# JasonQSY/Articulation3D

Hardware: AMD Instinct MI355X
Metric: frames/sec through PlaneRCNN detector at 480x640 (higher is better)
Workload: dtype f32 storage and accumulation; operands enter the matrix pipe with a 22-bit significand under ONE power-of-two block exponent per image (per ROI behind the poolers, per layer for filters): x*s = h + l in fp16, three fp16 MFMAs per k step (h.h + h.l + l.h). Elementwise law |y - y64| <= c (2^-22 sum|x|; 1 GPU; BASELINE configs[2]: full PlaneRCNN detector (ResNet50-FPN + RPN + ROIAlign + box/mask/plane/axis heads + depth head + NMS + mask paste + plane-offset LSQ + record pack), random-init weights with calibrated BN, synthetic 480x640 uint8 frames resident in HBM (arithmetic: see `dtype`)

## Files before the change

articulation3d_amd/_lib.py:

```python
from __future__ import annotations

import ctypes as C
import os

_PKG = os.path.dirname(os.path.abspath(__file__))
LIB_PATH = os.path.join(_PKG, "liba3d_hip.so")

ACT_NONE, ACT_RELU, ACT_LEAKY = 0, 1, 2

_ERR = {-1: "A3D_ERR_ARG", -2: "A3D_ERR_LAUNCH", -3: "A3D_ERR_UNSUPPORTED"}

fptr = C.c_void_p


class ConvDesc(C.Structure):
    _fields_ = [
        ("x", fptr), ("x2", fptr), ("w", fptr), ("scale", fptr), ("shift", fptr), ("res", fptr), ("y", fptr),
        ("workspace", fptr),
        ("B", C.c_int), ("H", C.c_int), ("W", C.c_int), ("Cin", C.c_int), ("Cin2", C.c_int),
        ("Ho", C.c_int), ("Wo", C.c_int), ("Cout", C.c_int),
        ("KH", C.c_int), ("KW", C.c_int), ("stride", C.c_int), ("pad", C.c_int),
        ("Kpad", C.c_int), ("ups", C.c_int), ("act", C.c_int), ("res_ups", C.c_int), ("pixshuf", C.c_int),
        ("stem", C.c_int), ("splitk", C.c_int),
        ("m_dev", fptr),
        ("tune", C.c_int), ("phase", C.c_int),
        ("w_wino", fptr),
        ("gate", fptr),
        ("precision", C.c_int),
        ("w_wino_x3", fptr),
        ("w_wino_cm", fptr),
        ("w_x3", fptr),
        ("in_amax", fptr),
        ("in_amax2", fptr),
        ("y_amax", fptr),
        ("w_scale", C.c_float),
        ("wino_m", fptr),
        ("io_bf16", C.c_int),
        ("x_h2", fptr),
        ("x2_h2", fptr),
        ("dot_w", fptr),
        ("dot_y", fptr),
        ("wino_t_off", C.c_int), ("wino_t_total", C.c_int),
        ("w_bf16", fptr),
    ]


class RpnDesc(C.Structure):
    _fields_ = [
        ("head", fptr * 5),
        ("Hf", C.c_int * 5), ("Wf", C.c_int * 5), ("stride", C.c_int * 5),
        ("cell_anchors", ((C.c_float * 4) * 3) * 5),
        ("B", C.c_int), ("L", C.c_int), ("A", C.c_int), ("CH", C.c_int),
        ("img_h", C.c_int), ("img_w", C.c_int),
        ("pre_topk", C.c_int), ("post_topk", C.c_int),
        ("nms_thresh", C.c_float), ("min_size", C.c_float),
        ("weights", C.c_float * 4),
        ("scale_clamp", C.c_float),
        ("workspace", fptr),
        ("out_boxes", fptr), ("out_scores", fptr), ("out_level", fptr), ("out_pos", fptr), ("out_count", fptr),
    ]


class BoxDetDesc(C.Structure):
    _fields_ = [
        ("pred", fptr), ("prop_boxes", fptr), ("prop_count", fptr),
        ("B", C.c_int), ("R", C.c_int), ("C", C.c_int), ("CH", C.c_int),
        ("img_h", C.c_int), ("img_w", C.c_int),
        ("score_thresh", C.c_float), ("nms_thresh", C.c_float),
        ("topk", C.c_int),
        ("weights", C.c_float * 4),
        ("scale_clamp", C.c_float),
        ("workspace", fptr),
        ("out_boxes", fptr), ("out_scores", fptr), ("out_classes", fptr), ("out_pos", fptr), ("out_count", fptr),
    ]


class RoiAlignDesc(C.Structure):
    _fields_ = [
        ("feat", fptr * 4),
        ("Hf", C.c_int * 4), ("Wf", C.c_int * 4),
        ("scale", C.c_float * 4),
        ("L", C.c_int), ("C", C.c_int),
        ("boxes", fptr), ("count", fptr), ("row_offset", fptr),
        ("B", C.c_int), ("R", C.c_int),
        ("P", C.c_int), ("sampling_ratio", C.c_int), ("aligned", C.c_int),
        ("out", fptr), ("out_level", fptr), ("order_ws", fptr),
        ("out_amax", fptr), ("level_amax", fptr * 4), ("window_count", fptr),
        ("out_h2", fptr),
        ("serial", C.c_int),
    ]


class PasteDesc(C.Structure):
    _fields_ = [
        ("boxes", fptr), ("scores", fptr), ("count", fptr), ("row_offset", fptr), ("mask_prob", fptr),
        ("normals", fptr), ("depth", fptr),
        ("B", C.c_int), ("R", C.c_int), ("MS", C.c_int), ("H", C.c_int), ("W", C.c_int),
        ("post_score_thresh", C.c_float), ("mask_thresh", C.c_float),
        ("focal", C.c_float), ("cx", C.c_float), ("cy", C.c_float), ("clip_boxes", C.c_int),
        ("masks", fptr), ("planes", fptr), ("area", fptr), ("keep", fptr), ("out_boxes", fptr),
    ]


class PackDesc(C.Structure):
    _fields_ = [
        ("boxes", fptr), ("scores", fptr), ("classes", fptr), ("count", fptr), ("row_offset", fptr), ("keep", fptr),
        ("planes", fptr), ("rot_axis", fptr), ("tran_axis", fptr), ("mask_prob", fptr),
        ("B", C.c_int), ("R", C.c_int), ("MS", C.c_int),
        ("records", fptr), ("rec_count", fptr),
    ]


class WgradDesc(C.Structure):
    _fields_ = [
        ("x", fptr), ("dy", fptr), ("scale", fptr), ("dw", fptr), ("workspace", fptr),
        ("B", C.c_int), ("H", C.c_int), ("W", C.c_int), ("Cin", C.c_int), ("Ho", C.c_int), ("Wo", C.c_int), ("Cout", C.c_int),
        ("KH", C.c_int), ("KW", C.c_int), ("stride", C.c_int), ("pad", C.c_int),
        ("splitk", C.c_int), ("accumulate", C.c_int), ("precision", C.c_int), ("io_bf16", C.c_int), ("defer_reduce", C.c_int),
        ("p_dev", fptr),
    ]
# ... 368 lines not shown
```

articulation3d_amd/csrc/conv_common.h:

```cpp
#pragma once
#include "conv_prims.h"
#include "../../include/a3d.h"

#define BK 32
#define LDK 36

template <int ACT>
__device__ __forceinline__ float a3d_act(float v) {
    if (ACT == A3D_ACT_RELU) return v <= 0.f ? 0.f : v;
    if (ACT == A3D_ACT_LEAKY) return v > 0.f ? v : 0.01f * v;
    return v;
}

__device__ __forceinline__ void a3d_stage_scale_shift(float *ss , const a3d_conv_desc &d, int n0, int BN, int tid) {
    if (tid < BN) {
        const int n = n0 + tid;
        const bool ok = n < d.Cout;
        ss[tid] = (d.scale && ok) ? d.scale[n] : 1.f;
        ss[BN + tid] = (d.shift && ok) ? d.shift[n] : 0.f;
    }
}
__device__ __forceinline__ f32x4 a3d_epilogue_math(const a3d_conv_desc &d, f32x4 v, const f32x4 s, const f32x4 sh, const bool has_res,
                                                    const f32x4 r) {
#pragma unroll
    for (int i = 0; i < 4; ++i) v[i] = __builtin_fmaf(v[i], s[i], sh[i]);
    if (has_res) v += r;
    if (d.act == A3D_ACT_RELU) {
#pragma unroll
        for (int i = 0; i < 4; ++i) v[i] = v[i] <= 0.f ? 0.f : v[i];
    } else if (d.act == A3D_ACT_LEAKY) {
#pragma unroll
        for (int i = 0; i < 4; ++i) v[i] = v[i] > 0.f ? v[i] : 0.01f * v[i];
    }
    return v;
}

__device__ __forceinline__ void out_rows(const a3d_conv_desc &d, int m, size_t &res_row, int &b, int &oh, int &ow) {
    res_row = (size_t)m;
    b = oh = ow = 0;
    if (d.res_ups || d.pixshuf || d.phase) {
        const int hw = d.Ho * d.Wo;
        b = m / hw;
        const int r = m - b * hw;
        oh = r / d.Wo;
        ow = r - oh * d.Wo;
        if (d.res_ups) res_row = ((size_t)b * (d.Ho >> 1) + (oh >> 1)) * (size_t)(d.Wo >> 1) + (ow >> 1);
    }
}

__device__ __forceinline__ void store_out(const a3d_conv_desc &d, f32x4 v, int m, int n, int b, int oh, int ow) {
    if (d.phase) {
        const int dy = (d.phase - 1) >> 1, dx = (d.phase - 1) & 1;
        const size_t row = ((size_t)b * (2 * d.Ho) + (2 * oh + dy)) * (size_t)(2 * d.Wo) + (2 * ow + dx);
        *reinterpret_cast<f32x4 *>(d.y + row * d.Cout + n) = v;
    } else if (d.pixshuf) {
        const int co_n = d.Cout >> 2;
        const int q = n / co_n, co = n - q * co_n;
        const int dy = q >> 1, dx = q & 1;
        const size_t row = ((size_t)b * (2 * d.Ho) + (2 * oh + dy)) * (size_t)(2 * d.Wo) + (2 * ow + dx);
        *reinterpret_cast<f32x4 *>(d.y + row * co_n + co) = v;
    } else {
        if (d.gate) {
            const f32x4 g = *reinterpret_cast<const f32x4 *>(d.gate + (size_t)m * d.Cout + n);
            for (int i = 0; i < 4; ++i) v[i] = g[i] > 0.f ? v[i] : 0.f;
        }
        *reinterpret_cast<f32x4 *>(d.y + (size_t)m * d.Cout + n) = v;
    }
}


__device__ __forceinline__ float a3d_pow2_scale(const float amax) {
    if (!(amax > 0.f) || !(amax < 3.0e38f)) return 1.f;
    return ldexpf(1.f, min(14 - ilogbf(amax), 126));
}
__device__ __forceinline__ float a3d_in_scale(const a3d_conv_desc &d, const int b) {
    float a = d.in_amax[b];
    if (d.in_amax2) a = fmaxf(a, d.in_amax2[b]);
    return a3d_pow2_scale(a);
}
void a3d_note_variant(const char *fmt, ...) __attribute__((format(printf, 1, 2)));

int a3d_conv_launch_v2(const a3d_conv_desc *d, hipStream_t s);
int a3d_conv_launch_xs_h2(const a3d_conv_desc *d, hipStream_t s);

#define A3D_SG_MAX_WAVES 1280
int a3d_conv_launch_sg_h2(const a3d_conv_desc *d, hipStream_t s);

int a3d_conv_launch_pw(const a3d_conv_desc *d, hipStream_t s, int force);

int a3d_conv_launch_bf16(const a3d_conv_desc *d, hipStream_t s);
int a3d_conv_launch_bf16w(const a3d_conv_desc *d, hipStream_t s);
int a3d_conv_launch_bf16xs(const a3d_conv_desc *d, hipStream_t s);
int a3d_conv_launch_bf16x3(const a3d_conv_desc *d, hipStream_t s);
int a3d_conv_launch_bf16x3_wide(const a3d_conv_desc *d, hipStream_t s);
int a3d_conv_launch_ph4p(const a3d_conv_desc *d, hipStream_t s);
int a3d_conv_launch_c3p(const a3d_conv_desc *d, hipStream_t s);
void a3d_launch_splitk_reduce(const a3d_conv_desc *d, int M, hipStream_t s);

int a3d_wino_eligible(const a3d_conv_desc *d);
size_t a3d_wino_workspace_bytes(const a3d_conv_desc *d);
int a3d_conv_launch_wino(const a3d_conv_desc *d, hipStream_t s);
int a3d_wino_fused_eligible(const a3d_conv_desc *d);
int a3d_conv_launch_wino_fused(const a3d_conv_desc *d, hipStream_t s);
```

articulation3d_amd/csrc/conv_gemm.hip:

```cpp
#include "conv_common.h"
#include <stdarg.h>
#include <stdio.h>

static int conv_check(const a3d_conv_desc *d) {
    if (!d || (!d->x && !d->x_h2) || !d->w || (!d->y && !d->dot_y)) return A3D_ERR_ARG;
    if ((d->dot_w || d->dot_y) && d->phase != 5) return A3D_ERR_ARG;
    if (d->x_h2 && d->precision != 3) return A3D_ERR_ARG;
    if (d->B <= 0 || d->Ho <= 0 || d->Wo <= 0 || d->Cout <= 0) return A3D_ERR_ARG;
    if ((d->Cout & 3) || (d->Kpad & 31) || d->splitk < 1) return A3D_ERR_ARG;
    if (d->stem) {
        if (d->KH != 7 || d->KW != 7 || d->stride != 2 || d->pad != 3 || d->Kpad != 224 || d->Cin2 || d->ups) return A3D_ERR_ARG;
    } else {
        if ((d->Cin & 31) || (d->Cin2 & 31) || (d->Cin2 && !d->x2 && !d->x2_h2)) return A3D_ERR_ARG;
        if (d->Kpad < d->KH * d->KW * (d->Cin + d->Cin2)) return A3D_ERR_ARG;
    }
    if (d->pixshuf && (d->Cout & 15)) return A3D_ERR_ARG;
    if (d->phase < 0 || d->phase > 5 || (d->phase == 5 && d->precision != 3 && d->precision != 2)) return A3D_ERR_ARG;
    if (d->gate && (d->pixshuf || d->phase)) return A3D_ERR_ARG;
    if (d->io_bf16 && d->precision != 1) return A3D_ERR_ARG;
    if (d->splitk > 1 && !d->workspace) return A3D_ERR_ARG;
    if ((size_t)d->B * d->H * d->W >= ((size_t)1 << 31)) return A3D_ERR_UNSUPPORTED;
    return A3D_OK;
}

static thread_local char g_last_variant[160] = "";
void a3d_note_variant(const char *fmt, ...) {
    va_list ap;
    va_start(ap, fmt);
    vsnprintf(g_last_variant, sizeof(g_last_variant), fmt, ap);
    va_end(ap);
}
extern "C" const char *a3d_last_conv_variant(void) { return g_last_variant; }

extern "C" size_t a3d_conv_workspace_bytes(const a3d_conv_desc *d) {
    if (!d) return 0;
    if (d->tune == 0 && a3d_wino_fused_eligible(d)) return 0;
    if ((d->tune == 0 || d->tune == 7 || d->tune == 8 || (d->tune >= 23 && d->tune <= 25) || d->tune >= 200) && a3d_wino_eligible(d)) return a3d_wino_workspace_bytes(d);
    if (d->splitk <= 1) return 0;
    return (size_t)d->splitk * d->B * d->Ho * d->Wo * d->Cout * sizeof(float);
}

extern "C" int a3d_conv2d_nhwc_f32(const a3d_conv_desc *d, void *stream) {
    const int rc = conv_check(d);
    if (rc != A3D_OK) return rc;
    hipStream_t s = (hipStream_t)stream;
    a3d_begin();
    if (d->precision == 1) return a3d_conv_launch_bf16(d, s);
    if (d->precision == 2) {
        if ((d->tune == 0 || d->tune == 8 || d->tune == 24 || d->tune == 25) && d->workspace && d->w_wino && d->w_wino_x3 && ((d->Cin + d->Cin2) & 31) == 0 && a3d_wino_eligible(d)) return a3d_conv_launch_wino(d, s);
        return a3d_conv_launch_bf16x3(d, s);
    }
    if (d->precision == 3 && d->x_h2) return a3d_conv_launch_bf16x3_wide(d, s);
    if (d->precision == 3) {
        if ((d->tune == 0 || d->tune == 23 || d->tune == 24) && d->workspace && d->w_wino && d->w_wino_x3 && ((d->Cin + d->Cin2) & 31) == 0 && a3d_wino_eligible(d))
            return a3d_conv_launch_wino(d, s);
        return a3d_conv_launch_bf16x3(d, s);
    }
    if (d->precision != 0) return A3D_ERR_ARG;
    if (d->tune == 0 && a3d_wino_fused_eligible(d)) return a3d_conv_launch_wino_fused(d, s);
    if ((d->tune == 0 || d->tune == 7 || d->tune >= 200) && d->workspace && a3d_wino_eligible(d)) return a3d_conv_launch_wino(d, s);
    if (d->tune == 0 || d->tune == 6) {
        const int r1 = a3d_conv_launch_pw(d, s, d->tune == 6);
        if (r1 != A3D_ERR_UNSUPPORTED) return r1;
    }
    if (d->tune == 1) return A3D_ERR_UNSUPPORTED;
    return a3d_conv_launch_v2(d, s);
}

extern "C" int a3d_version(void) { return 1; }
```

articulation3d_amd/csrc/conv_prims.h:

```cpp
#pragma once
#include "a3d_common.h"

typedef float f32x8 __attribute__((ext_vector_type(8)));
typedef __bf16 bf16x4 __attribute__((ext_vector_type(4)));
typedef __bf16 bf16x8 __attribute__((ext_vector_type(8)));
typedef _Float16 h16x4 __attribute__((ext_vector_type(4)));
typedef _Float16 h16x8 __attribute__((ext_vector_type(8)));

__device__ __forceinline__ __amdgpu_buffer_rsrc_t a3d_rsrc(const void *p, unsigned bytes) {
    return __builtin_amdgcn_make_buffer_rsrc(const_cast<void *>(p), 0, (int)bytes, 0x00020000);
}
__device__ __forceinline__ __amdgpu_buffer_rsrc_t a3d_rsrc_uniform(const void *p, unsigned bytes) {
    const unsigned long long v = reinterpret_cast<unsigned long long>(p);
    const unsigned lo = __builtin_amdgcn_readfirstlane((unsigned)v), hi = __builtin_amdgcn_readfirstlane((unsigned)(v >> 32));
    void *q = reinterpret_cast<void *>(((unsigned long long)hi << 32) | lo);
    return __builtin_amdgcn_make_buffer_rsrc(q, 0, (int)__builtin_amdgcn_readfirstlane(bytes), 0x00020000);
}
__device__ __forceinline__ f32x4 a3d_load4(__amdgpu_buffer_rsrc_t r, int voff, int soff) {
    return __builtin_bit_cast(f32x4, __builtin_amdgcn_raw_buffer_load_b128(r, voff, soff, 0));
}
__device__ __forceinline__ void a3d_dma16(__amdgpu_buffer_rsrc_t r, void *lds_dst, int voff, int soff) {
    __builtin_amdgcn_raw_ptr_buffer_load_lds(r, (__attribute__((address_space(3))) void *)lds_dst, 16, voff, soff, 0, 0);
}
template <int N>
__device__ __forceinline__ void a3d_wait_vm() {
    __asm__ volatile("s_waitcnt vmcnt(%0)" ::"n"(N) : "memory");
}

template <typename F, typename B>
__device__ __forceinline__ void a3d_split3(const F v, B &h, B &m, B &l) {
    h = __builtin_convertvector(v, B);
    const F r1 = v - __builtin_convertvector(h, F);
    m = __builtin_convertvector(r1, B);
    const F r2 = r1 - __builtin_convertvector(m, F);
    l = __builtin_convertvector(r2, B);
}
template <typename F, typename H>
__device__ __forceinline__ void a3d_split2h(const F v, const float s, H &h, H &l) {
    const F xs = v * s;
    h = __builtin_convertvector(xs, H);
    const F r = xs - __builtin_convertvector(h, F);
    l = __builtin_convertvector(r, H);
}

__device__ __forceinline__ void a3d_turn_put(float *T, const int row, const int quad, const f32x4 v) {
    *reinterpret_cast<f32x4 *>(T + row * 32 + ((quad ^ (row & 7)) << 2)) = v;
}
__device__ __forceinline__ f32x4 a3d_turn_get(const float *T, const int row, const int quad) {
    return *reinterpret_cast<const f32x4 *>(T + row * 32 + ((quad ^ (row & 7)) << 2));
}

__device__ __forceinline__ void a3d_note_amax(float *y_amax, const int b, float v, const bool valid) {
    if (!valid) v = 0.f;
    const unsigned long long live = __ballot(valid);
    if (!live) return;
    const int b0 = __shfl(b, __ffsll((long long)live) - 1, 64);
    const bool uniform = __all(!valid || b == b0);
    if (uniform) {
#pragma unroll
        for (int off = 32; off > 0; off >>= 1) v = fmaxf(v, __shfl_xor(v, off, 64));
        if ((threadIdx.x & 63) == 0 && v > y_amax[b0]) atomicMax(reinterpret_cast<int *>(y_amax + b0), __float_as_int(v));
    } else if (valid && v > y_amax[b]) {
        atomicMax(reinterpret_cast<int *>(y_amax + b), __float_as_int(v));
    }
}
__device__ __forceinline__ float a3d_max8(float v) {
    v = fmaxf(v, __shfl_xor(v, 1, 64));
    v = fmaxf(v, __shfl_xor(v, 2, 64));
    v = fmaxf(v, __shfl_xor(v, 4, 64));
    return v;
}
__device__ __forceinline__ void a3d_note_rows(float *y_amax, const float (&vm)[4], const bool one_image, const int mb, const int M, const int hwo,
                                              const int qr, const int qc) {
    if (!y_amax) return;
    if (one_image) {
        a3d_note_amax(y_amax, mb / hwo, fmaxf(fmaxf(vm[0], vm[1]), fmaxf(vm[2], vm[3])), true);
    } else {
#pragma unroll
        for (int j = 0; j < 4; ++j) {
            const int m = mb + qr + 8 * j;
            const float v = a3d_max8(vm[j]);
            a3d_note_amax(y_amax, m < M ? m / hwo : 0, v, m < M && qc == 0);
        }
    }
}
```

articulation3d_amd/csrc/conv_stem_pool.hip:

```cpp
#include "conv_common.h"
#include <limits.h>
#include <stdlib.h>

namespace {
typedef int i32x4 __attribute__((ext_vector_type(4)));

constexpr int SP_NKC = 14;
constexpr int SP_SP = 68;
template <int PH, int PW, int NW>
struct SpCfg {
    static constexpr int NT = 64 * NW;
    static constexpr int CH = 2 * PH + 1, CW = 2 * PW + 1, NQ = CH * CW;
    static constexpr int NBLK = NW;
    static constexpr int IH = 2 * CH + 5, IW = 2 * CW + 6, NPIX = IH * IW;
    static constexpr int PLANE = NPIX * 8;
    static constexpr int LI = (NPIX + NT - 1) / NT;
    static constexpr int PI = (PH * PW * 16 + NT - 1) / NT;
    static constexpr int LDS = 2 * PLANE + 32 * NBLK * SP_SP * 4 + 128 * 4;
    static_assert(NQ <= 32 * NBLK, "the blocks cover the conv pixels");
};

template <int PH, int PW, int NW>
__global__ __launch_bounds__(64 * NW, NW == 8 ? 1 : 2) void stem_pool_kernel(const a3d_conv_desc d, const int Hp, const int Wp, const int tiles_x, const int tiles_y, const int total) {
    using K = SpCfg<PH, PW, NW>;
// ... 136 lines not shown
                    f32x4 v = {acc[j][rg * 4 + 0], acc[j][rg * 4 + 1], acc[j][rg * 4 + 2], acc[j][rg * 4 + 3]};
                    v = (v * unx) * unw;
                    const f32x4 zero = {0.f, 0.f, 0.f, 0.f};
                    v = a3d_epilogue_math(d, v, *reinterpret_cast<const f32x4 *>(ss + n), *reinterpret_cast<const f32x4 *>(ss + 64 + n), false, zero);
                    *reinterpret_cast<f32x4 *>(stg + qq[j] * SP_SP + n) = v;
                }
        }
        __asm__ volatile("s_waitcnt lgkmcnt(0)" ::: "memory");
        __builtin_amdgcn_s_barrier();
        if (t + 1 < t_end) {
            const int bn = (t + 1) / tpi;
            if (bn != b_sx) {
                b_sx = bn;
                sx_p = a3d_in_scale(d, bn);
            }
            store_patch(sx_p);
        }
#ifdef A3D_ABLATIONS
        if (!(d.tune & 2))
#endif
#pragma unroll
        for (int it = 0; it < SP_PI; ++it) {
            if (pl_stg[it] < 0) continue;
            const int ppy = pl_pyx[it] >> 8, ppx = pl_pyx[it] & 255;
            const int py = py0 + ppy, px = px0 + ppx;
            if (py >= Hp || px >= Wp) continue;
            const float *sp = stg + pl_stg[it];
            f32x4 m = {-INFINITY, -INFINITY, -INFINITY, -INFINITY};
            if (relu) {
                i32x4 mi = {INT_MIN, INT_MIN, INT_MIN, INT_MIN};
#pragma unroll
                for (int dy = 0; dy < 3; ++dy) {
                    if ((unsigned)(cy0 + 2 * ppy + dy) >= (unsigned)d.Ho) continue;
#pragma unroll
                    for (int dx = 0; dx < 3; ++dx) {
                        if ((unsigned)(cx0 + 2 * ppx + dx) >= (unsigned)d.Wo) continue;
                        const i32x4 v = *reinterpret_cast<const i32x4 *>(sp + (dy * SP_CW + dx) * SP_SP) & 0x7FFFFFFF;
#pragma unroll
                        for (int k = 0; k < 4; ++k) mi[k] = max(mi[k], v[k]);
                    }
                }
                m = __builtin_bit_cast(f32x4, mi);
            } else {
#pragma unroll
                for (int dy = 0; dy < 3; ++dy) {
                    if ((unsigned)(cy0 + 2 * ppy + dy) >= (unsigned)d.Ho) continue;
#pragma unroll
                    for (int dx = 0; dx < 3; ++dx) {
                        if ((unsigned)(cx0 + 2 * ppx + dx) >= (unsigned)d.Wo) continue;
                        const f32x4 v = *reinterpret_cast<const f32x4 *>(sp + (dy * SP_CW + dx) * SP_SP);
#pragma unroll
                        for (int k = 0; k < 4; ++k) m[k] = (v[k] > m[k] || v[k] != v[k]) ? v[k] : m[k];
                    }
                }
            }
#ifdef A3D_ABLATIONS
            if (!(d.tune & 4))
#endif
            *reinterpret_cast<f32x4 *>(d.y + (((size_t)b * Hp + py) * Wp + px) * 64 + pl_c4[it]) = m;
            vmax = fmaxf(vmax, a3d_absmax4(m));
        }
        load_patch(t + 2 < t_end ? t + 2 : total);
    }
    if (b_cur >= 0 && d.y_amax) a3d_note_amax(d.y_amax, b_cur, vmax, true);
}
template <int PH, int PW, int NW>
int sp_launch(const a3d_conv_desc *d, hipStream_t s, const int Hp, const int Wp, const int slots) {
    using K = SpCfg<PH, PW, NW>;
    const int tiles_y = (Hp + PH - 1) / PH, tiles_x = (Wp + PW - 1) / PW;
    const long total = (long)d->B * tiles_x * tiles_y;
    if (total >= (1l << 30)) return A3D_ERR_UNSUPPORTED;
    static a3d_attr_once attr;
    if (attr.needed()) {
        if (hipFuncSetAttribute((const void *)stem_pool_kernel<PH, PW, NW>, hipFuncAttributeMaxDynamicSharedMemorySize, K::LDS) != hipSuccess) return A3D_ERR_LAUNCH;
        attr.mark();
    }
    const int grid = (int)(total < slots ? total : slots);
    hipLaunchKernelGGL((stem_pool_kernel<PH, PW, NW>), dim3(grid), dim3(K::NT), K::LDS, s, *d, Hp, Wp, tiles_x, tiles_y, (int)total);
    return a3d_check_launch();
}
}

extern "C" int a3d_stem_conv_pool(const a3d_conv_desc *d, void *stream) {
    if (!d || !d->x || !d->w_x3 || !d->y || !d->in_amax || !(d->w_scale > 0.f)) return A3D_ERR_ARG;
    if (!d->stem || d->precision != 3 || d->Cout != 64 || d->KH != 7 || d->KW != 7 || d->stride != 2 || d->pad != 3 || d->Kpad != 224) return A3D_ERR_UNSUPPORTED;
    if (d->Ho != (d->H + 6 - 7) / 2 + 1 || d->Wo != (d->W + 6 - 7) / 2 + 1 || d->x2 || d->res || d->gate || d->ups || d->phase || d->pixshuf || d->splitk != 1 || d->m_dev)
        return A3D_ERR_UNSUPPORTED;
    if ((size_t)d->B * d->H * d->W * 16 >= ((size_t)1 << 31)) return A3D_ERR_UNSUPPORTED;
    const int Hp = (d->Ho - 1) / 2 + 1, Wp = (d->Wo - 1) / 2 + 1;
    a3d_begin();
    int cus = 0, dev = 0;
    if (hipGetDevice(&dev) != hipSuccess || hipDeviceGetAttribute(&cus, hipDeviceAttributeMultiprocessorCount, dev) != hipSuccess || cus <= 0) cus = 256;
    const int form = (int)a3d_dev_knob("A3D_STEM_TILE", 0);
    a3d_note_variant("stem_pool_kernel");
    if (form == 2) return sp_launch<3, 8, 4>(d, (hipStream_t)stream, Hp, Wp, 2 * cus);
    return sp_launch<6, 9, 8>(d, (hipStream_t)stream, Hp, Wp, cus);
}
```

articulation3d_amd/csrc/conv_wino.hip:

```cpp
#include "conv_common.h"
#include <stdlib.h>

typedef unsigned int u32x4 __attribute__((ext_vector_type(4)));

__global__ __launch_bounds__(256) void wino_input_kernel(const float *__restrict__ x, const float *__restrict__ x2,
                                                         float *__restrict__ V, int B, int H, int W, int Cin, int Cin2,
                                                         int ups, int Ty, int Tx) {
    const int C = Cin + Cin2, C4 = C >> 2;
    const int Hl = ups ? 2 * H : H, Wl = ups ? 2 * W : W;
    const size_t T = (size_t)B * Ty * Tx;
    const size_t total = T * C4;
    for (size_t i = (size_t)blockIdx.x * blockDim.x + threadIdx.x; i < total; i += (size_t)gridDim.x * blockDim.x) {
        const int c = (int)(i % C4) * 4;
        const size_t t = i / C4;
        const int tx = (int)(t % Tx);
        const size_t r = t / Tx;
        const int ty = (int)(r % Ty);
        const int b = (int)(r / Ty);
        const bool second = c >= Cin;
        const float *src = second ? x2 : x;
        const int cs = second ? Cin2 : Cin, cc = second ? c - Cin : c;
        f32x4 d[4][4];
#pragma unroll
        for (int p = 0; p < 4; ++p) {
            const int ly = 2 * ty - 1 + p;
#pragma unroll
            for (int q = 0; q < 4; ++q) {
                const int lx = 2 * tx - 1 + q;
                f32x4 v = {0.f, 0.f, 0.f, 0.f};
                if ((unsigned)ly < (unsigned)Hl && (unsigned)lx < (unsigned)Wl) {
                    const int sy = ups ? ly >> 1 : ly, sx = ups ? lx >> 1 : lx;
                    v = *reinterpret_cast<const f32x4 *>(src + (((size_t)b * H + sy) * W + sx) * cs + cc);
                }
                d[p][q] = v;
            }
        }
        f32x4 m[4][4];
#pragma unroll
        for (int q = 0; q < 4; ++q) {
            m[0][q] = d[0][q] - d[2][q];
            m[1][q] = d[1][q] + d[2][q];
            m[2][q] = d[2][q] - d[1][q];
            m[3][q] = d[1][q] - d[3][q];
        }
#pragma unroll
        for (int u = 0; u < 4; ++u) {
            const f32x4 v0 = m[u][0] - m[u][2], v1 = m[u][1] + m[u][2], v2 = m[u][2] - m[u][1], v3 = m[u][1] - m[u][3];
            float *o = V + ((size_t)(u * 4) * T + t) * C + c;
            *reinterpret_cast<f32x4 *>(o) = v0;
            *reinterpret_cast<f32x4 *>(o + T * C) = v1;
            *reinterpret_cast<f32x4 *>(o + 2 * T * C) = v2;
            *reinterpret_cast<f32x4 *>(o + 3 * T * C) = v3;
        }
    }
}

typedef unsigned int wi_u32x2 __attribute__((ext_vector_type(2)));
typedef unsigned int wi_u32x4 __attribute__((ext_vector_type(4)));
__global__ __launch_bounds__(256) void wino_input_h2_kernel(const float *__restrict__ x, const float *__restrict__ x2, unsigned char *__restrict__ Vs,
                                                            const float *__restrict__ in_amax, const float *__restrict__ in_amax2, int B, int H, int W,
                                                            int Cin, int Cin2, int ups, int Ty, int Tx, int t_off, int t_total) {
    const int C = Cin + Cin2;
    const int Hl = ups ? 2 * H : H, Wl = ups ? 2 * W : W;
    const size_t T = (size_t)B * Ty * Tx;
    const size_t tile = (size_t)t_total * 64;
    const int KC = C >> 5;
    const size_t witems = ((T + 7) / 8) * KC;
    const int lane = threadIdx.x & 63;
    for (size_t w = (size_t)blockIdx.x * (blockDim.x >> 6) + (threadIdx.x >> 6); w < witems; w += (size_t)gridDim.x * (blockDim.x >> 6)) {
        const int kcw = (int)(w % KC);
        const size_t t = (w / KC) * 8 + (lane >> 3);
        if (t >= T) continue;
        const int c = kcw * 32 + (lane & 7) * 4;
        const int tx = (int)(t % Tx);
        const size_t r = t / Tx;
        const int ty = (int)(r % Ty);
        const int b = (int)(r / Ty);
        const bool second = c >= Cin;
        const float *src = second ? x2 : x;
        const int cs = second ? Cin2 : Cin, cc = second ? c - Cin : c;
        float am = in_amax[b];
        if (in_amax2) am = fmaxf(am, in_amax2[b]);
        const float sv = 0.25f * a3d_pow2_scale(am);
        f32x4 d[4][4];
#pragma unroll
        for (int p = 0; p < 4; ++p) {
            const int ly = 2 * ty - 1 + p;
#pragma unroll
            for (int q = 0; q < 4; ++q) {
                const int lx = 2 * tx - 1 + q;
                f32x4 v = {0.f, 0.f, 0.f, 0.f};
                if ((unsigned)ly < (unsigned)Hl && (unsigned)lx < (unsigned)Wl) {
                    const int sy = ups ? ly >> 1 : ly, sx = ups ? lx >> 1 : lx;
                    v = *reinterpret_cast<const f32x4 *>(src + (((size_t)b * H + sy) * W + sx) * cs + cc);
                }
                d[p][q] = v;
            }
        }
        f32x4 m[4][4];
#pragma unroll
        for (int q = 0; q < 4; ++q) {
            m[0][q] = d[0][q] - d[2][q];
            m[1][q] = d[1][q] + d[2][q];
            m[2][q] = d[2][q] - d[1][q];
            m[3][q] = d[1][q] - d[3][q];
        }
        const int kc = c >> 5;
        unsigned char *oh = Vs + (size_t)kc * 2 * tile + ((size_t)t_off + t) * 64 + (c & 31) * 2;
        const size_t pstride = (size_t)KC * 2 * tile;
#pragma unroll
        for (int u = 0; u < 4; ++u) {
            const f32x4 vv[4] = {m[u][0] - m[u][2], m[u][1] + m[u][2], m[u][2] - m[u][1], m[u][1] - m[u][3]};
#pragma unroll
            for (int v = 0; v < 4; ++v) {
                h16x4 h, l;
                a3d_split2h(vv[v], sv, h, l);
                *reinterpret_cast<h16x4 *>(oh) = h;
                *reinterpret_cast<h16x4 *>(oh + tile) = l;
                oh += pstride;
            }
        }
    }
}

struct WinoArgs {
    const float *V;
    const float *U;
    const float *scale, *shift;
    const float *gate;
    float *y;
    int T, C, Cout, B, Hl, Wl, Ty, Tx, act;
    const __bf16 *U3;
    float *y_amax;
    const float *in_amax, *in_amax2;
    float w_scale;
    float *M;
    int abl;
    int Toff, Ttot;
    struct Levels {
        int n;
        int t0[6];
        int Ty[5], Tx[5], Hl[5], Wl[5];
        float *y[5];
        const float *in_amax[5];
        float *y_amax[5];
    } lv;
};
__device__ __forceinline__ void wino_level_of(const WinoArgs::Levels &L, const int t, int &l, int &tl) {
    l = 0;
#pragma unroll
    for (int k = 1; k < 5; ++k) l = (k < L.n && t >= L.t0[k]) ? k : l;
    int base = L.t0[0];
#pragma unroll
    for (int k = 1; k < 5; ++k) base = l == k ? L.t0[k] : base;
    tl = t - base;
}
template <typename V>
__device__ __forceinline__ V wino_level_sel(const V (&arr)[5], const int l) {
    V v = arr[0];
#pragma unroll
    for (int k = 1; k < 5; ++k) v = l == k ? arr[k] : v;
    return v;
}

__device__ __forceinline__ float wino_v_scale(const WinoArgs &a, const int b) {
    float m = a.in_amax[b];
    if (a.in_amax2) m = fmaxf(m, a.in_amax2[b]);
    return 0.25f * a3d_pow2_scale(m);
}

template <int TN, int BKT>
__global__ __launch_bounds__(256, TN == 1 ? 3 : 1) void wino_gemm_kernel(const WinoArgs a, const int ntiles, const int nblk) {
    constexpr int BM = 64, BN = 2 * TN * 32;
    constexpr int LK = BKT + 4, TPR = BKT / 4, RPP = 256 / TPR;
    constexpr int XR = (BM + RPP - 1) / RPP, WR = BN / RPP;
    constexpr int BUF = (BM + BN) * LK;
    static_assert(BN % RPP == 0 && (BM % RPP == 0 || BM < RPP), "loader pass must tile the operand rows");
    __shared__ __attribute__((aligned(16))) float lds[2 * BUF];
    __shared__ __attribute__((aligned(16))) float ss[2 * BN];

    const int tid = threadIdx.x, lane = tid & 63, wave = tid >> 6;
    const int wm = wave >> 1, wn = wave & 1;
    const int logical = a3d_xcd_remap(blockIdx.x, nblk);
    const int mt = logical / ntiles, nt = logical - mt * ntiles;
    const int t0 = mt * BM, n0 = nt * BN;
    const int lr = tid / TPR, lc = (tid % TPR) * 4;
    const size_t vplane = (size_t)a.T * a.C, uplane = (size_t)a.Cout * a.C;
    const unsigned vbytes = (unsigned)(vplane * 4), ubytes = (unsigned)(uplane * 4);
    const int KC = a.C / BKT;
    const int NIT = 16 * KC;

    int xoff[XR], woff[WR];
#pragma unroll
    for (int i = 0; i < XR; ++i) {
        const int rrow = lr + RPP * i;
        const int t = t0 + rrow;
        xoff[i] = (rrow < BM && t < a.T) ? (t * a.C + lc) * 4 : -1;
    }
#pragma unroll
    for (int i = 0; i < WR; ++i) {
        const int n = n0 + lr + RPP * i;
        woff[i] = n < a.Cout ? (n * a.C + lc) * 4 : -1;
    }
    f32x4 xsA[XR], wsA[WR], xsB[XR], wsB[WR];
    int ld_f = 0, ld_kc = 0;
    auto load_chunk = [&](f32x4 (&xs)[XR], f32x4 (&ws)[WR]) {
        const int f = min(ld_f, 15);
        const __amdgpu_buffer_rsrc_t rv = a3d_rsrc(a.V + (size_t)f * vplane, vbytes);
        const __amdgpu_buffer_rsrc_t ru = a3d_rsrc(a.U + (size_t)f * uplane, ubytes);
        const int soff = ld_kc * BKT * 4;
#pragma unroll
        for (int i = 0; i < XR; ++i) xs[i] = a3d_load4(rv, xoff[i], soff);
#pragma unroll
        for (int i = 0; i < WR; ++i) ws[i] = a3d_load4(ru, woff[i], soff);
        if (++ld_kc == KC) {
            ld_kc = 0;
            ++ld_f;
        }
    };
    auto store_chunk = [&](int buf, const f32x4 (&xs)[XR], const f32x4 (&ws)[WR]) {
        float *X = lds + buf * BUF;
        float *Wt = X + BM * LK;
#pragma unroll
        for (int i = 0; i < XR; ++i)
            if (BM >= RPP || lr < BM) *reinterpret_cast<f32x4 *>(X + (lr + RPP * i) * LK + lc) = xs[i];
#pragma unroll
        for (int i = 0; i < WR; ++i) *reinterpret_cast<f32x4 *>(Wt + (lr + RPP * i) * LK + lc) = ws[i];
    };

    f32x16 mf[TN];
    f32x16 yy[4][TN];
#pragma unroll
    for (int n = 0; n < TN; ++n) {
#pragma unroll
        for (int r = 0; r < 16; ++r) {
            mf[n][r] = 0.f;
            yy[0][n][r] = yy[1][n][r] = yy[2][n][r] = yy[3][n][r] = 0.f;
        }
    }

    if (tid < BN) {
        const int n = n0 + tid;
        ss[tid] = (a.scale && n < a.Cout) ? a.scale[n] : 1.f;
        ss[BN + tid] = (a.shift && n < a.Cout) ? a.shift[n] : 0.f;
    }
    load_chunk(xsA, wsA);
    store_chunk(0, xsA, wsA);
    load_chunk(xsB, wsB);
    load_chunk(xsA, wsA);
    __syncthreads();
// ... 753 lines not shown
        rdB(F0, 0, 0, p);
    }
    X3W_FENCE

    int cf = 0, ckc = 0;
    for (int it = 0; it < nit; it += 2) {
        step0(0, F0, F1, xsB);
        __asm__ volatile("s_waitcnt vmcnt(2)" ::: "memory");
        __syncthreads();
        step1(0, F1, F0, xsB);
        if constexpr (!PS) {
            if (++ckc == KC) {
                ckc = 0;
                fold(mf, cf++);
            }
        }
        X3W_FENCE
        step0(1, F0, F1, xsA);
        __asm__ volatile("s_waitcnt vmcnt(2)" ::: "memory");
        __syncthreads();
        step1(1, F1, F0, xsA);
        if constexpr (!PS) {
            if (++ckc == KC) {
                ckc = 0;
                fold(mf, cf++);
            }
        }
        X3W_FENCE
    }
    }
#undef X3W_MIX
#undef X3W_TERM
#undef X3W_MFMA
#undef X3W_FENCE

    static_assert(NP * PLX * 2 >= WM * 4096, "WM 4 KiB tiles per V area");
    float *Tt = reinterpret_cast<float *>(lds + (wave / WM) * BUF) + (wave % WM) * 1024;
    const int tb = t0 + wm * 32;
    const int pr = lane & 31, ph = lane >> 5, qr = lane >> 3, qc = lane & 7;
    if constexpr (PS) {
#pragma unroll
        for (int ni = 0; ni < TN; ++ni) {
#pragma unroll
            for (int rg = 0; rg < 4; ++rg) {
                const f32x4 v = {mf[ni][rg * 4 + 0], mf[ni][rg * 4 + 1], mf[ni][rg * 4 + 2], mf[ni][rg * 4 + 3]};
                *reinterpret_cast<f32x4 *>(Tt + pr * 32 + (((rg * 2 + ph) ^ (pr & 7)) << 2)) = v;
            }
            const int n = n0 + wn * 64 + ni * 32 + qc * 4;
#pragma unroll
            for (int j = 0; j < 4; ++j) {
                const int q = qr + 8 * j;
                const f32x4 v = *reinterpret_cast<const f32x4 *>(Tt + q * 32 + ((qc ^ (q & 7)) << 2));
                const int t = tb + q;
                if (t < a.T && n < a.Cout) *reinterpret_cast<f32x4 *>(a.M + ((size_t)pf * a.T + t) * a.Cout + n) = v;
            }
        }
        return;
    }
#ifdef A3D_ABLATIONS
    if (a.abl & 64) {
        float sacc = 0.f;
#pragma unroll
        for (int ij = 0; ij < 4; ++ij)
#pragma unroll
            for (int ni = 0; ni < TN; ++ni)
#pragma unroll
                for (int r = 0; r < 16; ++r) sacc += yy[ij][ni][r];
        if (sacc == 12345.678f) a.y[tid] = sacc;
        return;
    }
#endif
    const int tyx = a.Ty * a.Tx;
    float unx = 1.f;
    const float unw = F16 ? 1.f / a.w_scale : 1.f;
    int jb[4], jy[4], jx[4];
    int jH[4], jW[4];
    float *jyp[4], *jya[4];
    if constexpr (ML) {
        {
            int l, tl;
            wino_level_of(a.lv, min(tb + pr, a.T - 1), l, tl);
            const int b = tl / (wino_level_sel(a.lv.Ty, l) * wino_level_sel(a.lv.Tx, l));
            if (tb + pr < a.T) {
                float m = wino_level_sel(a.lv.in_amax, l)[b];
                if (a.in_amax2) m = fmaxf(m, a.in_amax2[b]);
                unx = 1.f / (0.25f * a3d_pow2_scale(m));
            }
        }
#pragma unroll
        for (int j = 0; j < 4; ++j) {
            const int t = tb + qr + 8 * j;
            int l, tl;
            wino_level_of(a.lv, min(t, a.T - 1), l, tl);
            const int Tx = wino_level_sel(a.lv.Tx, l), Ty = wino_level_sel(a.lv.Ty, l);
            const int r = tl / Tx;
            jx[j] = 2 * (tl - r * Tx);
            jy[j] = 2 * (r % Ty);
            jb[j] = t < a.T ? r / Ty : -1;
            jH[j] = wino_level_sel(a.lv.Hl, l);
            jW[j] = wino_level_sel(a.lv.Wl, l);
            jyp[j] = wino_level_sel(a.lv.y, l);
            jya[j] = wino_level_sel(a.lv.y_amax, l);
        }
    } else {
    if (F16 && tb + pr < a.T) unx = 1.f / wino_v_scale(a, (tb + pr) / tyx);
#pragma unroll
    for (int j = 0; j < 4; ++j) {
        const int t = tb + qr + 8 * j;
        const int r = t / a.Tx;
        jx[j] = 2 * (t - r * a.Tx);
        jy[j] = 2 * (r % a.Ty);
        jb[j] = t < a.T ? r / a.Ty : -1;
        jH[j] = a.Hl;
        jW[j] = a.Wl;
        jyp[j] = a.y;
        jya[j] = a.y_amax;
    }
    }
    float vmax[4] = {0.f, 0.f, 0.f, 0.f};
#pragma unroll
    for (int ij = 0; ij < 4; ++ij) {
#pragma unroll
        for (int ni = 0; ni < TN; ++ni) {
#pragma unroll
            for (int rg = 0; rg < 4; ++rg) {
                f32x4 v = {yy[ij][ni][rg * 4 + 0], yy[ij][ni][rg * 4 + 1], yy[ij][ni][rg * 4 + 2], yy[ij][ni][rg * 4 + 3]};
                if constexpr (F16) v = (v * unx) * unw;
                *reinterpret_cast<f32x4 *>(Tt + pr * 32 + (((rg * 2 + ph) ^ (pr & 7)) << 2)) = v;
            }
            const int nl = wn * 64 + ni * 32 + qc * 4;
            const int n = n0 + nl;
            const f32x4 sc = *reinterpret_cast<const f32x4 *>(ss + nl), sh = *reinterpret_cast<const f32x4 *>(ss + BN + nl);
            f32x4 tv[4];
#pragma unroll
            for (int j = 0; j < 4; ++j) {
                const int q = qr + 8 * j;
                tv[j] = *reinterpret_cast<const f32x4 *>(Tt + q * 32 + ((qc ^ (q & 7)) << 2));
            }
#pragma unroll
            for (int j = 0; j < 4; ++j) {
                const int oy = jy[j] + (ij >> 1), ox = jx[j] + (ij & 1);
                if (jb[j] < 0 || oy >= jH[j] || ox >= jW[j] || n >= a.Cout) continue;
                const size_t ooff = (((size_t)jb[j] * jH[j] + oy) * jW[j] + ox) * a.Cout + n;
                f32x4 v = tv[j];
#pragma unroll
                for (int k = 0; k < 4; ++k) v[k] = __builtin_fmaf(v[k], sc[k], sh[k]);
                if (a.act == A3D_ACT_RELU) {
                    for (int k = 0; k < 4; ++k) v[k] = v[k] <= 0.f ? 0.f : v[k];
                } else if (a.act == A3D_ACT_LEAKY) {
                    for (int k = 0; k < 4; ++k) v[k] = v[k] > 0.f ? v[k] : 0.01f * v[k];
                }
                if (a.gate) {
                    const f32x4 g = *reinterpret_cast<const f32x4 *>(a.gate + ooff);
                    for (int k = 0; k < 4; ++k) v[k] = g[k] > 0.f ? v[k] : 0.f;
                }
                vmax[j] = fmaxf(vmax[j], a3d_absmax4(v));
                *reinterpret_cast<f32x4 *>(jyp[j] + ooff) = v;
            }
        }
    }
    if constexpr (ML) {
        int l0, tl0, l1, tl1;
        wino_level_of(a.lv, min(tb, a.T - 1), l0, tl0);
        wino_level_of(a.lv, min(tb + 31, a.T - 1), l1, tl1);
        const int tyx0 = wino_level_sel(a.lv.Ty, l0) * wino_level_sel(a.lv.Tx, l0);
        float *ya0 = wino_level_sel(a.lv.y_amax, l0);
        if (tb < a.T && l0 == l1 && tl0 / tyx0 == tl1 / tyx0) {
            if (ya0) a3d_note_amax(ya0, tl0 / tyx0, fmaxf(fmaxf(vmax[0], vmax[1]), fmaxf(vmax[2], vmax[3])), true);
        } else {
#pragma unroll
            for (int j = 0; j < 4; ++j) {
                const float v = a3d_max8(vmax[j]);
                if (jb[j] >= 0 && qc == 0 && jya[j] && v > jya[j][jb[j]]) atomicMax(reinterpret_cast<int *>(jya[j] + jb[j]), __float_as_int(v));
            }
        }
        return;
    }
    if (a.y_amax) {
        const int tl = min(tb + 31, a.T - 1);
        if (tb < a.T && tb / tyx == tl / tyx) {
            a3d_note_amax(a.y_amax, tb / tyx, fmaxf(fmaxf(vmax[0], vmax[1]), fmaxf(vmax[2], vmax[3])), true);
        } else {
#pragma unroll
            for (int j = 0; j < 4; ++j) a3d_note_amax(a.y_amax, max(jb[j], 0), a3d_max8(vmax[j]), jb[j] >= 0 && qc == 0);
        }
    }
}
__global__ __launch_bounds__(256) void wino_fold_kernel(const WinoArgs a) {
    const int C4 = a.Cout >> 2;
    const size_t idx = (size_t)blockIdx.x * 256 + threadIdx.x;
    const bool ok = idx < (size_t)a.T * C4;
    const int t = ok ? (int)(idx / C4) : 0;
    const int n = ok ? (int)(idx - (size_t)t * C4) * 4 : 0;
    const int tyx = a.Ty * a.Tx;
    const int bimg = t / tyx;
    float vmax = 0.f;
    if (ok) {
        f32x4 yy[4];
#pragma unroll
        for (int ij = 0; ij < 4; ++ij) yy[ij] = f32x4{0.f, 0.f, 0.f, 0.f};
#pragma unroll
        for (int f = 0; f < 16; ++f) {
            const f32x4 x = *reinterpret_cast<const f32x4 *>(a.M + ((size_t)f * a.T + t) * a.Cout + n);
            const int u = f >> 2, v = f & 3;
            const float au0 = (u < 3) ? 1.f : 0.f, au1 = (u == 0) ? 0.f : ((u == 1) ? 1.f : -1.f);
            const float av0 = (v < 3) ? 1.f : 0.f, av1 = (v == 0) ? 0.f : ((v == 1) ? 1.f : -1.f);
            const float c00 = au0 * av0, c01 = au0 * av1, c10 = au1 * av0, c11 = au1 * av1;
#pragma unroll
            for (int k = 0; k < 4; ++k) {
                yy[0][k] = __builtin_fmaf(c00, x[k], yy[0][k]);
                yy[1][k] = __builtin_fmaf(c01, x[k], yy[1][k]);
                yy[2][k] = __builtin_fmaf(c10, x[k], yy[2][k]);
                yy[3][k] = __builtin_fmaf(c11, x[k], yy[3][k]);
            }
        }
        const float unx = 1.f / wino_v_scale(a, bimg), unw = 1.f / a.w_scale;
        const int r = t / a.Tx;
        const int ox0 = 2 * (t - r * a.Tx), oy0 = 2 * (r % a.Ty);
        const f32x4 sc = a.scale ? *reinterpret_cast<const f32x4 *>(a.scale + n) : f32x4{1.f, 1.f, 1.f, 1.f};
        const f32x4 sh = a.shift ? *reinterpret_cast<const f32x4 *>(a.shift + n) : f32x4{0.f, 0.f, 0.f, 0.f};
#pragma unroll
        for (int ij = 0; ij < 4; ++ij) {
            const int oy = oy0 + (ij >> 1), ox = ox0 + (ij & 1);
            if (oy >= a.Hl || ox >= a.Wl) continue;
            const size_t ooff = (((size_t)bimg * a.Hl + oy) * a.Wl + ox) * a.Cout + n;
            f32x4 v = (yy[ij] * unx) * unw;
#pragma unroll
            for (int k = 0; k < 4; ++k) v[k] = __builtin_fmaf(v[k], sc[k], sh[k]);
            if (a.act == A3D_ACT_RELU) {
                for (int k = 0; k < 4; ++k) v[k] = v[k] <= 0.f ? 0.f : v[k];
            } else if (a.act == A3D_ACT_LEAKY) {
                for (int k = 0; k < 4; ++k) v[k] = v[k] > 0.f ? v[k] : 0.01f * v[k];
            }
            if (a.gate) {
                const f32x4 g = *reinterpret_cast<const f32x4 *>(a.gate + ooff);
                for (int k = 0; k < 4; ++k) v[k] = g[k] > 0.f ? v[k] : 0.f;
            }
            vmax = fmaxf(vmax, a3d_absmax4(v));
            *reinterpret_cast<f32x4 *>(a.y + ooff) = v;
        }
    }
    if (a.y_amax) a3d_note_amax(a.y_amax, bimg, vmax, ok);
}
__global__ __launch_bounds__(256) void split_bf16x3_kernel(const float *__restrict__ src, __bf16 *__restrict__ dst, int rows, int cols, int chunk, size_t total) {
    const size_t i = ((size_t)blockIdx.x * 256 + threadIdx.x) * 4;
    if (i >= total) return;
    const size_t per = (size_t)rows * cols;
    const size_t o = i / per, r = i - o * per;
    const int n = (int)(r / cols), c = (int)(r - (size_t)n * cols);
    bf16x4 h, m, l;
    a3d_split3(*reinterpret_cast<const f32x4 *>(src + i), h, m, l);
    __bf16 *d = dst + o * 3 * per + ((size_t)(c / chunk) * 3 * rows + n) * chunk + (c % chunk);
    *reinterpret_cast<bf16x4 *>(d) = h;
    *reinterpret_cast<bf16x4 *>(d + (size_t)rows * chunk) = m;
    *reinterpret_cast<bf16x4 *>(d + (size_t)rows * chunk * 2) = l;
}

extern "C" int a3d_split_bf16x3_chunk(const float *src, void *dst, int outer, int rows, int cols, int chunk, void *stream) {
    if (!src || !dst || outer <= 0 || rows <= 0 || cols <= 0 || (chunk != 16 && chunk != 32) || cols % chunk) return A3D_ERR_ARG;
    a3d_begin();
    const size_t total = (size_t)outer * rows * cols;
    hipLaunchKernelGGL(split_bf16x3_kernel, dim3((unsigned)((total / 4 + 255) / 256)), dim3(256), 0, (hipStream_t)stream, src, (__bf16 *)dst, rows, cols, chunk,
                       total);
    return a3d_check_launch();
}

__global__ __launch_bounds__(256) void split_f16x2_kernel(const float *__restrict__ src, _Float16 *__restrict__ dst, int rows, int cols, int chunk, float scale,
                                                          size_t total) {
    const size_t i = ((size_t)blockIdx.x * 256 + threadIdx.x) * 4;
    if (i >= total) return;
    const size_t per = (size_t)rows * cols;
    const size_t o = i / per, r = i - o * per;
    const int n = (int)(r / cols), c = (int)(r - (size_t)n * cols);
    h16x4 h, l;
    a3d_split2h(*reinterpret_cast<const f32x4 *>(src + i), scale, h, l);
    _Float16 *d = dst + o * 2 * per + ((size_t)(c / chunk) * 2 * rows + n) * chunk + (c % chunk);
    *reinterpret_cast<h16x4 *>(d) = h;
    *reinterpret_cast<h16x4 *>(d + (size_t)rows * chunk) = l;
}

extern "C" int a3d_split_f16x2_chunk(const float *src, void *dst, int outer, int rows, int cols, int chunk, float scale, void *stream) {
    if (!src || !dst || outer <= 0 || rows <= 0 || cols <= 0 || (chunk != 16 && chunk != 32) || cols % chunk || !(scale > 0.f)) return A3D_ERR_ARG;
    a3d_begin();
    const size_t total = (size_t)outer * rows * cols;
    hipLaunchKernelGGL(split_f16x2_kernel, dim3((unsigned)((total / 4 + 255) / 256)), dim3(256), 0, (hipStream_t)stream, src, (_Float16 *)dst, rows, cols, chunk,
                       scale, total);
    return a3d_check_launch();
}

extern "C" int a3d_split_bf16x3(const float *src, void *dst, int outer, int rows, int cols, void *stream) {
    return a3d_split_bf16x3_chunk(src, dst, outer, rows, cols, 32, stream);
}

int a3d_wino_eligible(const a3d_conv_desc *d) {
    if (!d->w_wino) return 0;
    if (d->KH != 3 || d->KW != 3 || d->stride != 1 || d->pad != 1) return 0;
    if (d->res || d->pixshuf || d->stem || d->splitk != 1 || d->m_dev) return 0;
    if (((d->Cin + d->Cin2) & 15) || (d->Cin & 3) || (d->Cin2 & 3) || (d->Cout & 3)) return 0;
    const int Hl = d->ups ? 2 * d->H : d->H, Wl = d->ups ? 2 * d->W : d->W;
    const size_t T = (size_t)d->B * ((Hl + 1) / 2) * ((Wl + 1) / 2);
    const size_t C = (size_t)d->Cin + d->Cin2;
    if (T * C * 4 >= ((size_t)1 << 32) || (size_t)d->Cout * C * 4 >= ((size_t)1 << 32)) return 0;
    return 1;
}

size_t a3d_wino_workspace_bytes(const a3d_conv_desc *d) {
    const int Hl = d->ups ? 2 * d->H : d->H, Wl = d->ups ? 2 * d->W : d->W;
    size_t T = (size_t)d->B * ((Hl + 1) / 2) * ((Wl + 1) / 2);
    if (d->precision == 3 && d->wino_t_total > 0) T = (size_t)d->wino_t_total;
    return 16 * T * ((size_t)d->Cin + d->Cin2) * sizeof(float);
}

extern "C" size_t a3d_wino_m_bytes(const a3d_conv_desc *d) {
    const long ps_max = a3d_dev_knob("A3D_WINO_PS_BLOCKS", 48);
    if (!d || d->precision != 3 || !a3d_wino_eligible(d)) return 0;
    const int C = d->Cin + d->Cin2;
    if ((C & 63) || ((d->Cout + 63) / 64) % 2 != 0) return 0;
    const int Hl = d->ups ? 2 * d->H : d->H, Wl = d->ups ? 2 * d->W : d->W;
    const size_t T = (size_t)d->B * ((Hl + 1) / 2) * ((Wl + 1) / 2);
    const long blocks4 = (long)((T + 127) / 128) * ((d->Cout + X3W_BN - 1) / X3W_BN);
    if (blocks4 > ps_max) return 0;
    return 16 * T * (size_t)d->Cout * sizeof(float);
}

static int wino_launch_input(const a3d_conv_desc *d, hipStream_t s) {
    const int Hl = d->ups ? 2 * d->H : d->H, Wl = d->ups ? 2 * d->W : d->W;
    const int Ty = (Hl + 1) / 2, Tx = (Wl + 1) / 2;
    const int C = d->Cin + d->Cin2;
    const size_t T = (size_t)d->B * Ty * Tx;
    const size_t total = T * (C / 4);
    size_t blocks = (total + 255) / 256;
    if (blocks > 16384) blocks = 16384;
    if (d->precision == 3) {
        if ((C & 31) || !d->in_amax) return A3D_ERR_ARG;
        if (d->wino_t_total && (d->wino_t_off < 0 || (size_t)d->wino_t_off + T > (size_t)d->wino_t_total)) return A3D_ERR_ARG;
        if ((size_t)(d->wino_t_total ? d->wino_t_total : T) * C * 4 >= ((size_t)1 << 32)) return A3D_ERR_UNSUPPORTED;
        hipLaunchKernelGGL(wino_input_h2_kernel, dim3((int)blocks), dim3(256), 0, s, d->x, d->x2, reinterpret_cast<unsigned char *>(d->workspace), d->in_amax,
                           d->in_amax2, d->B, d->H, d->W, d->Cin, d->Cin2, d->ups, Ty, Tx, d->wino_t_total ? d->wino_t_off : 0, d->wino_t_total ? d->wino_t_total : (int)T);
        return A3D_OK;
    }
    hipLaunchKernelGGL(wino_input_kernel, dim3((int)blocks), dim3(256), 0, s, d->x, d->x2, d->workspace, d->B, d->H, d->W,
                       d->Cin, d->Cin2, d->ups, Ty, Tx);
    return A3D_OK;
}

static int wino_launch_gemm(const a3d_conv_desc *d, hipStream_t s) {
    const int Hl = d->ups ? 2 * d->H : d->H, Wl = d->ups ? 2 * d->W : d->W;
    const int Ty = (Hl + 1) / 2, Tx = (Wl + 1) / 2;
    const size_t T = (size_t)d->B * Ty * Tx;
    WinoArgs a;
    a.V = d->workspace;
    a.U = d->w_wino;
    a.scale = d->scale;
    a.shift = d->shift;
    a.gate = d->gate;
    a.y = d->y;
    a.T = (int)T;
    a.C = d->Cin + d->Cin2;
    a.Cout = d->Cout;
    a.B = d->B;
    a.Hl = Hl;
    a.Wl = Wl;
    a.Ty = Ty;
    a.Tx = Tx;
    a.act = d->act;
    const int mtiles = (int)((T + 63) / 64);
    a.U3 = nullptr;
    a.y_amax = d->y_amax;
    a.in_amax = d->in_amax;
    a.in_amax2 = d->in_amax2;
    a.w_scale = d->w_scale;
    a.M = nullptr;
    a.abl = (int)a3d_dev_knob("A3D_WINO_ABL", 0);
    a.Toff = 0;
    a.Ttot = (int)T;
    a.lv.n = 1;
    for (int k = 0; k < 5; ++k) {
        a.lv.t0[k] = k == 0 ? 0 : (int)T;
        a.lv.Ty[k] = Ty;
        a.lv.Tx[k] = Tx;
        a.lv.Hl[k] = Hl;
        a.lv.Wl[k] = Wl;
        a.lv.y[k] = d->y;
        a.lv.in_amax[k] = d->in_amax;
        a.lv.y_amax[k] = d->y_amax;
    }
    a.lv.t0[5] = (int)T;
    if (d->wino_t_total) {
        if (d->precision != 3 || d->wino_t_off < 0 || (size_t)d->wino_t_off + T > (size_t)d->wino_t_total) return A3D_ERR_ARG;
        a.Toff = d->wino_t_off;
        a.Ttot = d->wino_t_total;
    }
    if (d->precision == 3) {
        if (!d->w_wino_x3 || (a.C & 31) || !d->in_amax || !(d->w_scale > 0.f) || ((d->Cout + 63) / 64) % 2 != 0 ||
            (size_t)16 * d->Cout * a.C * 4 >= ((size_t)1 << 32))
            return A3D_ERR_ARG;
        a.U3 = reinterpret_cast<const __bf16 *>(d->w_wino_x3);
        const int nt = (d->Cout + X3W_BN - 1) / X3W_BN;
        const int wmx = d->tune == 24 ? 2 : 4;
        static a3d_attr_once attr3;
        if (attr3.needed()) {
            if (hipFuncSetAttribute((const void *)wino_gemm_x3w_kernel<2, true>, hipFuncAttributeMaxDynamicSharedMemorySize, x3w_lds_bytes(2, 2)) != hipSuccess ||
                hipFuncSetAttribute((const void *)wino_gemm_x3w_kernel<4, true>, hipFuncAttributeMaxDynamicSharedMemorySize, x3w_lds_bytes(4, 2)) != hipSuccess ||
                hipFuncSetAttribute((const void *)wino_gemm_x3w_kernel<4, true, false, 1>, hipFuncAttributeMaxDynamicSharedMemorySize, x3w_lds_bytes(4, 2)) != hipSuccess ||
                hipFuncSetAttribute((const void *)wino_gemm_x3w_kernel<2, true, true>, hipFuncAttributeMaxDynamicSharedMemorySize, x3w_lds_bytes(2, 2)) != hipSuccess)
                return A3D_ERR_LAUNCH;
            attr3.mark();
        }
        if (d->wino_m && a3d_wino_m_bytes(d)) {
            a.M = d->wino_m;
            a3d_note_variant("wino_gemm_h2w_kernel<2> planes + wino_fold_kernel");
            hipLaunchKernelGGL((wino_gemm_x3w_kernel<2, true, true>), dim3(mtiles * nt, 16), dim3(256), x3w_lds_bytes(2, 2), s, a, nt, mtiles * nt);
            const size_t threads = T * (size_t)(d->Cout / 4);
            hipLaunchKernelGGL(wino_fold_kernel, dim3((unsigned)((threads + 255) / 256)), dim3(256), 0, s, a);
            return A3D_OK;
        }
        a3d_note_variant("wino_gemm_h2w_kernel<%d>", wmx);
        if (wmx == 4) {
            const int m4 = (int)((T + 127) / 128);
            if (d->tune == 23) hipLaunchKernelGGL((wino_gemm_x3w_kernel<4, true>), dim3(m4 * nt), dim3(512), x3w_lds_bytes(4, 2), s, a, nt, m4 * nt);
            else hipLaunchKernelGGL((wino_gemm_x3w_kernel<4, true, false, 1>), dim3(m4 * nt), dim3(512), x3w_lds_bytes(4, 2), s, a, nt, m4 * nt);
        } else {
            hipLaunchKernelGGL((wino_gemm_x3w_kernel<2, true>), dim3(mtiles * nt), dim3(256), x3w_lds_bytes(2, 2), s, a, nt, mtiles * nt);
        }
        return A3D_OK;
    }
    if (d->precision == 2) {
        if (!d->w_wino_x3 || (a.C & 31)) return A3D_ERR_ARG;
        a.U3 = reinterpret_cast<const __bf16 *>(d->w_wino_x3);
        const int wm_force = d->tune == 24 ? 2 : (d->tune == 25 ? 4 : 0);
        const int ntw = (d->Cout + X3W_BN - 1) / X3W_BN;
        const long blocks_w = (long)((T + 127) / 128) * ntw, blocks_n = (long)mtiles * ((d->Cout + 63) / 64);
        const long rounds_w = (blocks_w + 255) / 256, rounds_n = ((blocks_n + 255) / 256 + 2) / 3;
        const bool wide = d->tune != 8 && ((d->Cout + 63) / 64) % 2 == 0 && (size_t)16 * d->Cout * a.C * 6 < ((size_t)1 << 32) &&
                          (wm_force || 100 * rounds_w <= 86 * rounds_n);
        if (wide) {
            const int nt = ntw;
            const int wmx = wm_force ? wm_force : 4;
            static a3d_attr_once attr_set;
            if (attr_set.needed()) {
                if (hipFuncSetAttribute((const void *)wino_gemm_x3w_kernel<2>, hipFuncAttributeMaxDynamicSharedMemorySize, x3w_lds_bytes(2, 3)) != hipSuccess ||
                    hipFuncSetAttribute((const void *)wino_gemm_x3w_kernel<4>, hipFuncAttributeMaxDynamicSharedMemorySize, x3w_lds_bytes(4, 3)) != hipSuccess)
                    return A3D_ERR_LAUNCH;
                attr_set.mark();
            }
            a3d_note_variant("wino_gemm_x3w_kernel<%d>", wmx);
            if (wmx == 4) {
                const int m4 = (int)((T + 127) / 128);
                hipLaunchKernelGGL((wino_gemm_x3w_kernel<4>), dim3(m4 * nt), dim3(512), x3w_lds_bytes(4, 3), s, a, nt, m4 * nt);
            } else {
                hipLaunchKernelGGL((wino_gemm_x3w_kernel<2>), dim3(mtiles * nt), dim3(256), x3w_lds_bytes(2, 3), s, a, nt, mtiles * nt);
            }
            return A3D_OK;
        }
        const int nt = (d->Cout + 63) / 64;
        a3d_note_variant("wino_gemm_x3_kernel");
        hipLaunchKernelGGL(wino_gemm_x3_kernel, dim3(mtiles * nt), dim3(256), 0, s, a, nt, mtiles * nt);
        return A3D_OK;
    }
    int tn = 1, bk32 = 1;
    if (d->tune >= 200) {
        tn = (d->tune - 200) / 10 + 1;
        bk32 = (d->tune - 200) % 10;
    }
    const int bn = tn * 64;
    const int ntiles = (d->Cout + bn - 1) / bn;
    const dim3 grid(mtiles * ntiles);
    a3d_note_variant("wino_gemm_kernel<%d,%d>", tn, bk32 ? 32 : 16);
    if (tn == 1 && !bk32) hipLaunchKernelGGL((wino_gemm_kernel<1, 16>), grid, dim3(256), 0, s, a, ntiles, mtiles * ntiles);
    else if (tn == 1) hipLaunchKernelGGL((wino_gemm_kernel<1, 32>), grid, dim3(256), 0, s, a, ntiles, mtiles * ntiles);
    else if (!bk32) hipLaunchKernelGGL((wino_gemm_kernel<2, 16>), grid, dim3(256), 0, s, a, ntiles, mtiles * ntiles);
    else hipLaunchKernelGGL((wino_gemm_kernel<2, 32>), grid, dim3(256), 0, s, a, ntiles, mtiles * ntiles);
    return A3D_OK;
}

int a3d_conv_launch_wino(const a3d_conv_desc *d, hipStream_t s) {
    if (!a3d_wino_eligible(d) || !d->workspace) return A3D_ERR_UNSUPPORTED;
    int r = wino_launch_input(d, s);
    if (r != A3D_OK) return r;
    r = wino_launch_gemm(d, s);
    if (r != A3D_OK) return r;
    return a3d_check_launch();
}

extern "C" int a3d_wino_input_transform(const a3d_conv_desc *d, void *stream) {
    if (!d || !d->x || !a3d_wino_eligible(d) || !d->workspace) return A3D_ERR_ARG;
    a3d_begin();
    const int r = wino_launch_input(d, (hipStream_t)stream);
    if (r != A3D_OK) return r;
    return a3d_check_launch();
}

extern "C" int a3d_wino_gemm_levels(const a3d_conv_desc *lv, int n, void *stream) {
    if (!lv || n < 1 || n > 5) return A3D_ERR_ARG;
    const a3d_conv_desc *d0 = lv;
    if (d0->precision != 3 || !a3d_wino_eligible(d0) || !d0->workspace || !d0->w_wino_x3 || !(d0->w_scale > 0.f) || d0->wino_t_total <= 0) return A3D_ERR_ARG;
    const int C = d0->Cin + d0->Cin2;
    if ((C & 31) || ((d0->Cout + 63) / 64) % 2 != 0 || (size_t)16 * d0->Cout * C * 4 >= ((size_t)1 << 32)) return A3D_ERR_ARG;
    WinoArgs a;
    a.V = d0->workspace;
    a.U = d0->w_wino;
    a.U3 = reinterpret_cast<const __bf16 *>(d0->w_wino_x3);
    a.scale = d0->scale;
    a.shift = d0->shift;
    a.gate = nullptr;
    a.y = nullptr;
    a.y_amax = nullptr;
    a.in_amax = nullptr;
    a.in_amax2 = nullptr;
    a.w_scale = d0->w_scale;
    a.M = nullptr;
    a.abl = 0;
    a.C = C;
    a.Cout = d0->Cout;
    a.act = d0->act;
    a.B = d0->B;
    a.Hl = a.Wl = a.Ty = a.Tx = 1;
    a.Toff = 0;
    a.Ttot = a.T = d0->wino_t_total;
    a.lv.n = n;
    size_t t = 0;
    for (int k = 0; k < 5; ++k) {
        const a3d_conv_desc *d = lv + (k < n ? k : n - 1);
        if (k < n) {
            if (d->precision != 3 || !a3d_wino_eligible(d) || d->workspace != d0->workspace || d->w_wino_x3 != d0->w_wino_x3 || d->Cout != d0->Cout ||
                d->Cin + d->Cin2 != C || d->Cin2 || d->x2 || d->ups || d->gate || d->act != d0->act || d->scale != d0->scale || d->shift != d0->shift ||
                d->w_scale != d0->w_scale || d->wino_t_total != d0->wino_t_total || (size_t)d->wino_t_off != t || !d->in_amax || !d->y)
                return A3D_ERR_ARG;
        }
        const int Ty = (d->H + 1) / 2, Tx = (d->W + 1) / 2;
        a.lv.t0[k] = (int)t;
        a.lv.Ty[k] = Ty;
        a.lv.Tx[k] = Tx;
        a.lv.Hl[k] = d->H;
        a.lv.Wl[k] = d->W;
        a.lv.y[k] = d->y;
        a.lv.in_amax[k] = d->in_amax;
        a.lv.y_amax[k] = d->y_amax;
        if (k < n) t += (size_t)d->B * Ty * Tx;
    }
    a.lv.t0[5] = (int)t;
    if (t != (size_t)d0->wino_t_total || t * C * 4 >= ((size_t)1 << 32)) return A3D_ERR_ARG;
    a3d_begin();
    static a3d_attr_once attr_ml;
    if (attr_ml.needed()) {
        if (hipFuncSetAttribute((const void *)wino_gemm_x3w_kernel<4, true, false, 1>, hipFuncAttributeMaxDynamicSharedMemorySize, x3w_lds_bytes(4, 2)) != hipSuccess)
            return A3D_ERR_LAUNCH;
        attr_ml.mark();
    }
    const int nt = (a.Cout + X3W_BN - 1) / X3W_BN, m4 = (int)((t + 127) / 128);
    a3d_note_variant("wino_gemm_h2w_kernel<4> levels%d", n);
    hipLaunchKernelGGL((wino_gemm_x3w_kernel<4, true, false, 1>), dim3(m4 * nt), dim3(512), x3w_lds_bytes(4, 2), (hipStream_t)stream, a, nt, m4 * nt);
    return a3d_check_launch();
}

extern "C" int a3d_wino_gemm(const a3d_conv_desc *d, void *stream) {
    if (!d || !d->y || !a3d_wino_eligible(d) || !d->workspace) return A3D_ERR_ARG;
    a3d_begin();
    const int r = wino_launch_gemm(d, (hipStream_t)stream);
    if (r != A3D_OK) return r;
    return a3d_check_launch();
}
```

articulation3d_amd/csrc/conv_xs_b2b.hip:

```cpp
#include "conv_common.h"

namespace {

constexpr int BB_NST = 7;
constexpr int BB_D = BB_NST - 1;
constexpr int BB_STAGE = 8192;
constexpr int bb_lds_bytes(int bn, int n2) { return BB_NST * BB_STAGE + 4 * 4096 + 2 * 2 * bn * 4 + 2 * n2 * 4; }

struct B2bArgs {
    const void *w2;
    const float *scale2;
    const float *shift2;
    float *z;
    float *z_amax;
    int Cout2, act2;
};

template <int KC, int NG, int KS, int N2T, bool PREF>
__global__ __launch_bounds__(256, 2) void conv_xs_b2b_kernel(const a3d_conv_desc d, const B2bArgs e, const int M) {
    static_assert(NG * KS == 4 && KC % KS == 0 && N2T % 2 == 0, "ring stage = 8 KiB; the second layer's tiles go in pairs");
    constexpr int BN = 32 * NG;
    constexpr int SPT = KC / KS;
    constexpr int R = 4 * NG;
    constexpr int TP = N2T / 2;
// ... 191 lines not shown
                    yb[1] = __builtin_shufflevector(m0_, m1_, 0, 1, 2, 3, 4, 5, 6, 7);
                    yb[2] = __builtin_shufflevector(l0, l1, 0, 1, 2, 3, 4, 5, 6, 7);
                }
#pragma unroll
                for (int tp = 0; tp < TP; ++tp) {
                    const unsigned char *st = enter(SPT + g * G2G + ci * TP + tp);
                    bf16x8 fa[3][2];
#pragma unroll
                    for (int p = 0; p < 3; ++p)
#pragma unroll
                        for (int tl = 0; tl < 2; ++tl) fa[p][tl] = *reinterpret_cast<const bf16x8 *>(st + (p * 2 + tl) * 1024);
#define BB_TERM(PA, PB)                                                                                                          \
    _Pragma("unroll") for (int tl = 0; tl < 2; ++tl) z[tp * 2 + tl] = __builtin_amdgcn_mfma_f32_32x32x16_bf16(fa[PA][tl], yb[PB], z[tp * 2 + tl], 0, 0, 0);
                    BB_TERM(0, 0)
                    BB_TERM(0, 1)
                    BB_TERM(1, 0)
                    BB_TERM(1, 1)
                    BB_TERM(2, 0)
                    BB_TERM(0, 2)
#undef BB_TERM
                }
            }
        }
    };
    if constexpr (PREF) {
        for (int ns = 0; ns < nsteps; ns += 2) {
            nstep(ns, rvA, rvB);
            nstep(ns + 1, rvB, rvA);
        }
    } else {
        for (int ns = 0; ns < nsteps; ++ns) nstep(ns, rvA, rvA);
    }

    a3d_conv_desc d2 = d;
    d2.act = e.act2;
    float zmax[4] = {0.f, 0.f, 0.f, 0.f};
#pragma unroll
    for (int t = 0; t < N2T; ++t) {
#pragma unroll
        for (int rg = 0; rg < 4; ++rg) {
            const f32x4 v = {z[t][rg * 4 + 0], z[t][rg * 4 + 1], z[t][rg * 4 + 2], z[t][rg * 4 + 3]};
            a3d_turn_put(T, pr, rg * 2 + ph, v);
        }
        const int nl = t * 32 + qc * 4;
        f32x4 tv[4];
#pragma unroll
        for (int j = 0; j < 4; ++j) {
            const int qq = qr + 8 * j;
            tv[j] = a3d_turn_get(T, qq, qc);
        }
#pragma unroll
        for (int j = 0; j < 4; ++j) {
            const int m = m0 + qr + 8 * j;
            if (m >= M) continue;
            const f32x4 zero = {0.f, 0.f, 0.f, 0.f};
            const f32x4 v = a3d_epilogue_math(d2, tv[j], *reinterpret_cast<const f32x4 *>(ss2 + nl), *reinterpret_cast<const f32x4 *>(ss2 + Cout2 + nl), false, zero);
            zmax[j] = fmaxf(zmax[j], a3d_absmax4(v));
            *reinterpret_cast<f32x4 *>(e.z + (size_t)m * Cout2 + nl) = v;
        }
    }
    a3d_note_rows(d.y_amax, vmax, one_image, m0, M, hwo, qr, qc);
    a3d_note_rows(e.z_amax, zmax, one_image, m0, M, hwo, qr, qc);
    a3d_wait_vm<0>();
}
template <int KC, int NG, int KS, int N2T, bool PREF>
int launch_b2b(const a3d_conv_desc *d, const B2bArgs &e, hipStream_t s) {
    constexpr int BN = 32 * NG;
    const int M = d->B * d->Ho * d->Wo;
    const int mtiles = (M + 127) / 128;
    constexpr int lds = bb_lds_bytes(BN, 32 * N2T);
    static a3d_attr_once attr;
    if (attr.needed()) {
        if (hipFuncSetAttribute((const void *)conv_xs_b2b_kernel<KC, NG, KS, N2T, PREF>, hipFuncAttributeMaxDynamicSharedMemorySize, lds) != hipSuccess) return A3D_ERR_LAUNCH;
        attr.mark();
    }
    a3d_note_variant("conv_h2xs_b2b_kernel<%d,%d>", 16 * KC, 32 * N2T);
    hipLaunchKernelGGL((conv_xs_b2b_kernel<KC, NG, KS, N2T, PREF>), dim3(mtiles), dim3(256), lds, s, *d, e, M);
    return a3d_check_launch();
}
}

extern "C" int a3d_conv_b2b(const a3d_conv_desc *d1, const a3d_conv_desc *d2, void *stream) {
    if (!d1 || !d2 || !d1->x || !d1->y || !d2->y) return A3D_ERR_ARG;
    const a3d_conv_desc *d = d1;
    if (d->precision != 3 || !d->w_x3 || !d->in_amax || d->in_amax2 || !(d->w_scale > 0.f) || !d->res) return A3D_ERR_UNSUPPORTED;
    if (d->KH != 1 || d->KW != 1 || d->stride != 1 || d->pad != 0 || d->Kpad != d->Cin) return A3D_ERR_UNSUPPORTED;
    if (d->stem || d->ups || d->phase || d->pixshuf || d->gate || d->x2 || d->Cin2 || d->splitk != 1 || d->m_dev || d->res_ups || d->io_bf16) return A3D_ERR_UNSUPPORTED;
    if (d2->precision != 2 || !d2->w_x3 || d2->KH != 1 || d2->KW != 1 || d2->stride != 1 || d2->pad != 0 || d2->Kpad != d2->Cin) return A3D_ERR_UNSUPPORTED;
    if (d2->stem || d2->ups || d2->phase || d2->pixshuf || d2->gate || d2->x2 || d2->Cin2 || d2->splitk != 1 || d2->m_dev || d2->res || d2->io_bf16) return A3D_ERR_UNSUPPORTED;
    if (d2->Cin != d->Cout || d2->B != d->B || d2->H != d->Ho || d2->W != d->Wo || d2->Ho != d->Ho || d2->Wo != d->Wo) return A3D_ERR_ARG;
    if (d2->x && d2->x != d->y) return A3D_ERR_ARG;
    if (d->Cout % 128) return A3D_ERR_UNSUPPORTED;
    const size_t M = (size_t)d->B * d->Ho * d->Wo;
    if (M * d->Cout * 4 >= ((size_t)1 << 31) || M * d->Cin * 4 >= ((size_t)1 << 31) || (size_t)d->Cout * d->Cin * 4 >= ((size_t)1 << 31)) return A3D_ERR_UNSUPPORTED;
    B2bArgs e;
    e.w2 = d2->w_x3;
    e.scale2 = d2->scale;
    e.shift2 = d2->shift;
    e.z = d2->y;
    e.z_amax = d2->y_amax;
    e.Cout2 = d2->Cout;
    e.act2 = d2->act;
    a3d_begin();
    if (d->Cin == 64 && d2->Cout == 64) return launch_b2b<4, 2, 2, 2, true>(d, e, (hipStream_t)stream);
    if (d->Cin == 128 && d2->Cout == 128) return launch_b2b<8, 2, 2, 4, false>(d, e, (hipStream_t)stream);
    return A3D_ERR_UNSUPPORTED;
}
```

articulation3d_amd/modeling/backbone.py:

```python
from __future__ import annotations

from typing import Dict

import torch
from torch import nn

from .. import ops
from ..streams import SMALL_BATCH, run_branches
from ..registry import BACKBONE_REGISTRY
from ..structures import ShapeSpec
from .layers import ACT_NONE, ACT_RELU, Conv2d, FrozenBatchNorm2d, c2_msra_fill, c2_xavier_fill, to_nchw_view


class BasicStem(nn.Module):
    def __init__(self, in_channels=3, out_channels=64):
        super().__init__()
        self.conv1 = Conv2d(in_channels, out_channels, 7, stride=2, padding=3, bias=False,
                            norm=FrozenBatchNorm2d(out_channels), act=ACT_RELU)
        c2_msra_fill(self.conv1.weight)

    def forward(self, x4):
        from .layers import _CalibrationState

        if not _CalibrationState.active and not self.training:
            y = ops.stem_pool(x4, self.conv1.packed())
            if y is not None:
                return y
        return ops.maxpool3x3s2(self.conv1(x4))


class BottleneckBlock(nn.Module):

    def __init__(self, in_channels, out_channels, bottleneck_channels, stride):
        super().__init__()
        self.shortcut = None
        if in_channels != out_channels:
            self.shortcut = Conv2d(in_channels, out_channels, 1, stride=stride, bias=False,
                                   norm=FrozenBatchNorm2d(out_channels))
        self.conv1 = Conv2d(in_channels, bottleneck_channels, 1, stride=stride, bias=False,
                            norm=FrozenBatchNorm2d(bottleneck_channels), act=ACT_RELU)
        self.conv2 = Conv2d(bottleneck_channels, bottleneck_channels, 3, stride=1, padding=1, bias=False,
                            norm=FrozenBatchNorm2d(bottleneck_channels), act=ACT_RELU)
        self.conv3 = Conv2d(bottleneck_channels, out_channels, 1, bias=False, norm=FrozenBatchNorm2d(out_channels),
                            act=ACT_RELU)
        for layer in (self.conv1, self.conv2, self.conv3, self.shortcut):
            if layer is not None:
                c2_msra_fill(layer.weight)

    def forward(self, x):
        sc = self.shortcut(x) if self.shortcut is not None else x
        y = self.conv2(self.conv1(x))
        return self.conv3(y, res=sc)

    def forward_pair(self, x, a=None, nxt=None, frozen=False):
        from .layers import _CalibrationState

        sc = self.shortcut(x) if self.shortcut is not None else x
        b = self.conv2(self.conv1(x) if a is None else a)
        if nxt is not None and not _CalibrationState.active and (frozen or not self.training):
            pair = ops.conv2d_b2b(b, self.conv3.packed(), sc, nxt.conv1.packed())
            if pair is not None:
                return pair
        return self.conv3(b, res=sc), None


class ResNet(nn.Module):
    def __init__(self, cfg):
        super().__init__()
        r = cfg.MODEL.RESNETS
        assert r.DEPTH == 50 and r.NORM == "FrozenBN" and r.STRIDE_IN_1X1 and r.NUM_GROUPS == 1 and r.RES5_DILATION == 1, \
            "only the ResNet-50 / FrozenBN / stride-in-1x1 backbone of the reference config is implemented"
        self.stem = BasicStem(3, r.STEM_OUT_CHANNELS)
        in_c, out_c, mid = r.STEM_OUT_CHANNELS, r.RES2_OUT_CHANNELS, r.NUM_GROUPS * r.WIDTH_PER_GROUP
        self._out_features = list(r.OUT_FEATURES)
        self._out_feature_channels, self._out_feature_strides = {}, {}
        stride_total = 4
        for name, nblk in (("res2", 3), ("res3", 4), ("res4", 6), ("res5", 3)):
            first_stride = 1 if name == "res2" else 2
            blocks = []
            for i in range(nblk):
                blocks.append(BottleneckBlock(in_c, out_c, mid, first_stride if i == 0 else 1))
                in_c = out_c
            for prev, blk in zip(blocks, blocks[1:]):
                blk.conv1.b2b_second = (prev.conv3.in_channels, blk.conv1.out_channels) in ops.B2B_PAIRS
            self.add_module(name, nn.Sequential(*blocks))
            stride_total *= first_stride
            self._out_feature_channels[name], self._out_feature_strides[name] = out_c, stride_total
            out_c, mid = out_c * 2, mid * 2

    def forward_stage(self, name: str, x, frozen: bool = False):
        blocks = list(getattr(self, name))
        a = None
        for i, blk in enumerate(blocks):
            x, a = blk.forward_pair(x, a, blocks[i + 1] if i + 1 < len(blocks) else None, frozen=frozen)
        return x

    def forward(self, x4) -> Dict[str, torch.Tensor]:
        x = self.stem(x4)
        outs = {}
        for name in ("res2", "res3", "res4", "res5"):
            x = outs[name] = self.forward_stage(name, x)
        return outs

    def output_shape(self):
        return {n: ShapeSpec(channels=self._out_feature_channels[n], stride=self._out_feature_strides[n]) for n in self._out_features}


class FPN(nn.Module):

    def __init__(self, cfg):
        super().__init__()
        f = cfg.MODEL.FPN
        assert f.NORM == "" and f.FUSE_TYPE == "sum", "reference config: FPN.NORM '' / FUSE_TYPE sum"
        self.bottom_up = ResNet(cfg)
        self.in_features = list(f.IN_FEATURES)
        shapes = self.bottom_up.output_shape()
        oc = f.OUT_CHANNELS
        self._levels = []
        for name in self.in_features:
            stage = int(name[3:])
            lat = Conv2d(shapes[name].channels, oc, 1, bias=True)
            out = Conv2d(oc, oc, 3, padding=1, bias=True)
            c2_xavier_fill(lat.weight, lat.bias)
            c2_xavier_fill(out.weight, out.bias)
            self.add_module(f"fpn_lateral{stage}", lat)
# ... 44 lines not shown
```

articulation3d_amd/modeling/layers.py:

```python
from __future__ import annotations

import math
from typing import Optional

import torch
from torch import nn

from .. import ops
from ..ops import ACT_LEAKY, ACT_NONE, ACT_RELU


def c2_msra_fill(weight: torch.Tensor, bias: Optional[torch.Tensor] = None):
    nn.init.kaiming_normal_(weight, mode="fan_out", nonlinearity="relu")
    if bias is not None:
        nn.init.constant_(bias, 0)


def c2_xavier_fill(weight: torch.Tensor, bias: Optional[torch.Tensor] = None):
    nn.init.kaiming_uniform_(weight, a=1)
    if bias is not None:
        nn.init.constant_(bias, 0)


def to_nhwc(t: torch.Tensor) -> torch.Tensor:
    return t.permute(0, 2, 3, 1).contiguous()


def to_nchw_view(t: torch.Tensor) -> torch.Tensor:
    return t.permute(0, 3, 1, 2)


class _CalibrationState:

    active = False


def _calibrate_norm(norm, y_raw: torch.Tensor, eps_floor: float = 1e-6):
    flat = y_raw.reshape(-1, y_raw.shape[-1])[:, : norm.running_mean.numel()]
    norm.running_mean.copy_(flat.mean(0))
    norm.running_var.copy_(flat.var(0, unbiased=False).clamp_min(eps_floor))


def _publish():
    if torch.cuda.is_available():
        ops.publish()


class _Packable(nn.Module):

    pin_precision = None
    b2b_second = False
    _a3d_name = ""

    def __init__(self):
        super().__init__()
        self._pack_cache = None
        self._pack_key = None
        self._key_src = None

    def __setattr__(self, name, value):
        if name not in ("_pack_cache", "_pack_key", "_key_src"):
            self.__dict__["_key_src"] = None
        super().__setattr__(name, value)

    def _apply(self, fn, recurse=True):
        self.__dict__["_key_src"] = None
        return super()._apply(fn, recurse)

    @staticmethod
    def _shape_of(mods):
        n, kids = 0, []
        for m in mods:
            n += len(m._parameters) + len(m._buffers)
            kids += [id(c) for c in m._modules.values()]
        return n, tuple(kids)

    def _key(self):
        cached = self.__dict__.get("_key_src")
        if cached is not None:
            src, mods, shape = cached
            if shape != self._shape_of(mods):
                cached = None
        if cached is None:
            src, mods = [], list(self.modules())
            for m in mods:
                src += [(m._parameters, k) for k in m._parameters] + [(m._buffers, k) for k in m._buffers]
            shape = self._shape_of(mods)
            self.__dict__["_key_src"] = (src, mods, shape)
        out = []
        for d, k in src:
            t = d.get(k)
            if t is not None:
                out.append((t.data_ptr(), t._version, t.device))
        return tuple(out)

    def packed(self) -> ops.PackedConv:
        key = self._key()
        if self._pack_cache is None or key != self._pack_key:
            self._pack_cache = self._pack()
            self._pack_key = key
            _publish()
        pin = self.pin_precision
        if pin is None and self.b2b_second and ops.B2B_FUSED:
            pin = 2
        self._pack_cache.pin_precision, self._pack_cache.name = pin, self._a3d_name
        return self._pack_cache

    def _pack(self):
        raise NotImplementedError


class FrozenBatchNorm2d(nn.Module):

    def __init__(self, num_features, eps=1e-5):
        super().__init__()
        self.num_features = num_features
        self.eps = eps
        self.register_buffer("weight", torch.ones(num_features))
        self.register_buffer("bias", torch.zeros(num_features))
        self.register_buffer("running_mean", torch.zeros(num_features))
        self.register_buffer("running_var", torch.ones(num_features) - eps)


class Conv2d(_Packable):

    def __init__(self, in_channels, out_channels, kernel_size, stride=1, padding=0, bias=True, norm=None, act=ACT_NONE):
        super().__init__()
        self.in_channels, self.out_channels = in_channels, out_channels
        self.kernel_size, self.stride, self.padding, self.act = kernel_size, stride, padding, act
        self.weight = nn.Parameter(torch.empty(out_channels, in_channels, kernel_size, kernel_size))
        self.bias = nn.Parameter(torch.zeros(out_channels)) if bias else None
        self.norm = norm
        nn.init.kaiming_uniform_(self.weight, a=math.sqrt(5))

    def _pack(self):
        bn = None
        if self.norm is not None:
            n = self.norm
            bn = (n.weight, n.bias, n.running_mean, n.running_var, n.eps)
        if self.in_channels == 3 and self.kernel_size == 7:
            return ops.pack_stem(self.weight, bn, device=self.weight.device)
        return ops.pack_conv(self.weight, self.bias, bn, self.stride, self.padding, self.act, device=self.weight.device)

    def forward(self, x, **kw):
        if _CalibrationState.active and self.norm is not None:
            stem = self.in_channels == 3 and self.kernel_size == 7
            ident = (torch.ones_like(self.norm.weight), torch.zeros_like(self.norm.bias), torch.zeros_like(self.norm.running_mean),
                     torch.ones_like(self.norm.running_var) - self.norm.eps, self.norm.eps)
            raw = ops.pack_stem(self.weight, ident, device=self.weight.device) if stem else \
                ops.pack_conv(self.weight, self.bias, ident, self.stride, self.padding, ACT_NONE, device=self.weight.device)
            _calibrate_norm(self.norm, ops.conv2d(x, raw, act=ACT_NONE, **{k: v for k, v in kw.items() if k in ("x2", "ups")}))
        return ops.conv2d(x, self.packed(), **kw)


class BNConv2d(_Packable):

    def __init__(self, conv: nn.Conv2d, bn: nn.BatchNorm2d, act: int):
        super().__init__()
        self.conv, self.bn, self.act = conv, bn, act

    def _key(self):
        ts = list(self.conv.parameters()) + list(self.bn.parameters()) + list(self.bn.buffers())
        return tuple((t.data_ptr(), t._version, str(t.device)) for t in ts)

    def _pack(self):
        bn = (self.bn.weight, self.bn.bias, self.bn.running_mean, self.bn.running_var, self.bn.eps)
        return ops.pack_conv(self.conv.weight, self.conv.bias, bn, 1, 1, self.act, device=self.conv.weight.device)

    def forward(self, x, **kw):
        if _CalibrationState.active:
            raw = ops.pack_conv(self.conv.weight, self.conv.bias, None, 1, 1, ACT_NONE, device=self.conv.weight.device)
            _calibrate_norm(self.bn, ops.conv2d(x, raw, **kw))
        if kw.get("ups"):
            return ops.conv2d_ups(x, self.packed_phases(), x2=kw.get("x2"))
        return ops.conv2d(x, self.packed(), **kw)

    def packed_phases(self):
        key = self._key()
        if getattr(self, "_phase_cache", None) is None or key != self._phase_key:
            bn = (self.bn.weight, self.bn.bias, self.bn.running_mean, self.bn.running_var, self.bn.eps)
            self._phase_cache = ops.pack_conv_ups_phases(self.conv.weight, self.conv.bias, bn, self.act, device=self.conv.weight.device)
            self._phase_key = key
            _publish()
        for q in self._phase_cache:
            q.pin_precision, q.name = self.pin_precision, self._a3d_name
        return self._phase_cache


# ... 17 lines not shown
```

articulation3d_amd/modeling/mask_head.py:

```python
from __future__ import annotations

import torch
from torch import nn

from .. import ops
from ..registry import ROI_MASK_HEAD_REGISTRY
from ..structures import ShapeSpec
from .layers import ACT_RELU, Conv2d, _Packable, c2_msra_fill


class ConvTranspose2x2(_Packable):
    def __init__(self, cin, cout):
        super().__init__()
        self.weight = nn.Parameter(torch.empty(cin, cout, 2, 2))
        self.bias = nn.Parameter(torch.zeros(cout))

    def _pack(self):
        return ops.pack_deconv2x2(self.weight, self.bias, ACT_RELU, device=self.weight.device)

    def forward(self, x, **kw):
        return ops.conv2d(x, self.packed(), **kw)


@ROI_MASK_HEAD_REGISTRY.register()
class MaskRCNNConvUpsampleHead(nn.Module):
    def __init__(self, cfg, input_shape: ShapeSpec):
        super().__init__()
        m = cfg.MODEL.ROI_MASK_HEAD
        assert m.NORM == "" and m.CLS_AGNOSTIC_MASK, "reference config: no norm, class-agnostic mask"
        cin, dim = input_shape.channels, m.CONV_DIM
        self.conv_norm_relus = []
        for k in range(m.NUM_CONV):
            conv = Conv2d(cin if k == 0 else dim, dim, 3, padding=1, act=ACT_RELU)
            c2_msra_fill(conv.weight, conv.bias)
            self.add_module(f"mask_fcn{k + 1}", conv)
            self.conv_norm_relus.append(conv)
        self.deconv = ConvTranspose2x2(dim if m.NUM_CONV > 0 else cin, dim)
        c2_msra_fill(self.deconv.weight, self.deconv.bias)
        self.predictor = Conv2d(dim, 1, 1)
        nn.init.normal_(self.predictor.weight, std=0.001)
        nn.init.constant_(self.predictor.bias, 0)

    def forward_rows(self, x):
        rows = x.shape[0]
        for conv in self.conv_norm_relus:
            x = conv(x, wino=True)
        x = self.deconv(x)
        S = x.shape[1]
        w = self.predictor.weight.reshape(1, -1).contiguous()
        p = ops.linear_small(x.view(rows * S * S, x.shape[3]), w, self.predictor.bias, sigmoid=True)
        return p.view(rows, S, S)


def build_mask_head(cfg, input_shape):
    return ROI_MASK_HEAD_REGISTRY.get(cfg.MODEL.ROI_MASK_HEAD.NAME)(cfg, input_shape)
```

articulation3d_amd/modeling/meta_arch.py:

```python
from __future__ import annotations

import importlib
import os
from dataclasses import dataclass
from typing import List, Optional

import torch
from torch import nn

from .. import ops
from ..registry import META_ARCH_REGISTRY
from ..streams import SMALL_BATCH
from ..structures import Boxes, ImageList, Instances
from .backbone import build_backbone
from .depth_head import build_depth_head
from .layers import to_nchw_view
from .postprocessing import detector_postprocess
from .roi_heads.roi_heads import BatchedDetections, build_roi_heads
from .rpn import build_proposal_generator

__all__ = ["PlaneRCNN", "BatchedOutput", "build_model"]

POST_SCORE_THRESH = 0.1
STAGE3_TRAINABLE = "roi_heads.mask_head"
STAGE3_FROZEN_HEADS = ("roi_heads.plane_head", "roi_heads.axis_head", "depth_head")
STAGE4_TRAINABLE = "roi_heads.plane_head"
STAGE4_FROZEN_HEADS = ("roi_heads.mask_head", "roi_heads.axis_head", "depth_head")
STAGE5_TRAINABLE = "depth_head"
STAGE5_FROZEN_HEADS = ("roi_heads.mask_head", "roi_heads.plane_head", "roi_heads.axis_head")
STAGE_TRAINER = {1: ("..training", "DetectorTrainer"), 2: ("..training_axis", "AxisTrainer"), 3: ("..training_mask", "MaskTrainer"),
                 4: ("..training_plane", "PlaneTrainer"), 5: ("..training_depth", "DepthTrainer")}


@dataclass
class BatchedOutput:
    image_size: tuple
    det: BatchedDetections
    depth: Optional[torch.Tensor]
    keep: torch.Tensor
    boxes: torch.Tensor
    planes: torch.Tensor
    area: torch.Tensor
    masks: Optional[torch.Tensor]
    records: torch.Tensor
    rec_count: torch.Tensor
    proposals: Optional[tuple] = None


@META_ARCH_REGISTRY.register()
class PlaneRCNN(nn.Module):
    def __init__(self, cfg):
        super().__init__()
        self.device = torch.device(cfg.MODEL.DEVICE)
        self.backbone = build_backbone(cfg)
        self.proposal_generator = build_proposal_generator(cfg, self.backbone.output_shape())
        self.roi_heads = build_roi_heads(cfg, self.backbone.output_shape())
        self.mask_threshold = cfg.MODEL.ROI_MASK_HEAD.MASK_THRESHOLD
        self.nms = cfg.MODEL.ROI_MASK_HEAD.NMS
        self.depth_head_on = cfg.MODEL.DEPTH_ON
        self.refine_on = cfg.MODEL.REFINE_ON
        self.axis_on = cfg.MODEL.AXIS_ON
        if self.depth_head_on:
            self.depth_head = build_depth_head(cfg)
        assert not self.refine_on, "REFINE_ON is false in every reference config (refine head out of scope)"
        self.vis_period = cfg.VIS_PERIOD
        self.input_format = cfg.INPUT.FORMAT
        assert len(cfg.MODEL.PIXEL_MEAN) == len(cfg.MODEL.PIXEL_STD) == 3
        self.pixel_mean = tuple(float(v) for v in cfg.MODEL.PIXEL_MEAN)
        self.pixel_std = tuple(float(v) for v in cfg.MODEL.PIXEL_STD)
        self._eval_gt_box = cfg.TEST.EVAL_GT_BOX
        self.to(self.device)
        self._freeze = cfg.MODEL.FREEZE
        for layers in self._freeze:
            final = self
            for l in layers.split("."):
                final = getattr(final, l)
            for params in final.parameters():
                params.requires_grad = False

    @torch.no_grad()
    def inference_batched(self, frames: torch.Tensor, want_masks: bool = False, given_boxes=None, source_rgb: bool = False,
                          resize_to=(480, 640)) -> BatchedOutput:
        assert not self.training
        if frames.is_cuda and ops.DEFAULT_PRECISION == 3:
            ops.amax_reserve(frames.shape[0] * (512 + 8 * int(self.proposal_generator.post_nms_topk[False])), frames.device)
        if source_rgb:
            assert frames.dtype == torch.uint8 and self.input_format == "BGR"
            B = frames.shape[0]
            H, W = int(resize_to[0]), int(resize_to[1])
            x4 = ops.preprocess_resize_u8(frames.contiguous(), self.pixel_mean, self.pixel_std, (H, W), swap_rb=True)
        elif frames.dtype == torch.uint8:
            B, H, W, _ = frames.shape
            x4 = ops.preprocess_u8hwc(frames.contiguous(), self.pixel_mean, self.pixel_std)
        else:
            B, _, H, W = frames.shape
            x4 = ops.preprocess_f32chw(frames.contiguous().float(), self.pixel_mean, self.pixel_std)
        assert H % self.backbone.size_divisibility == 0 and W % self.backbone.size_divisibility == 0, \
            "batched path expects frames already a multiple of 32 (the reference feeds 480x640)"
        hw = (H, W)
        feats = self.backbone.forward_nhwc(x4)
        share = [f for f in feats.values() if f.is_cuda] if (self.depth_head_on and given_boxes is None and B > SMALL_BATCH) else []
        with ops.share_wino_input(share):
            return self._detect_on_features(feats, frames, B, hw, want_masks, given_boxes)

    @torch.no_grad()
    def inference_graphed(self, frames: torch.Tensor, want_masks: bool = False) -> BatchedOutput:
        assert not self.training and frames.is_cuda
        rh = self.roi_heads
        B = frames.shape[0]
        R = rh.box_predictor.test_topk_per_image
        if B * R > rh.FIXED_ROWS_CAP:
            return self.inference_batched(frames, want_masks=want_masks)
        key = (tuple(frames.shape), frames.dtype, bool(want_masks), ops.DEFAULT_PRECISION, tuple(self.pinned_layers()))
        cache = self.__dict__.setdefault("_graphs", {})
        ent = cache.get(key)
        if ent is None:
            saved = rh.fixed_rows
            rh.fixed_rows = True
            try:
                static_in = frames.clone()
                for _ in range(2):
                    self.inference_batched(static_in, want_masks=want_masks)
                torch.cuda.synchronize()
                g = torch.cuda.CUDAGraph()
                ops._amax_arena.pop(static_in.device, None)
                with torch.cuda.graph(g):
                    out = self.inference_batched(static_in, want_masks=want_masks)
                ops._amax_arena.pop(static_in.device, None)
            finally:
                rh.fixed_rows = saved
            ent = cache[key] = (g, static_in, out)
        g, static_in, out = ent
        static_in.copy_(frames)
        g.replay()
        return out

    def _packables(self):
        from .layers import _Packable

        seen = {}
        for name, m in self.named_modules():
            if isinstance(m, _Packable):
                seen[id(m)] = (name, m)
        dh = getattr(self, "depth_head", None)
        if dh is not None:
            for kind in ("conv", "deconv"):
                for i, m in enumerate(getattr(dh, "_pk_" + kind, []), 1):
                    seen.setdefault(id(m), (f"depth_head.{kind}{i}", m))
        return list(seen.values())

    @torch.no_grad()
    def audit_precision(self, frames: torch.Tensor, pin: bool = True, source_rgb: bool = False, resize_to=(480, 640)):
        assert not self.training
        for name, m in self._packables():
            m._a3d_name = name
        audit = ops.PrecisionAudit(pin=pin)
        if ops.DEFAULT_PRECISION != 3:
            return audit
        with audit:
            self.inference_batched(frames, source_rgb=source_rgb, resize_to=resize_to)
            torch.cuda.synchronize()
        if pin:
            names = {r["layer"] for r in audit.pinned()}
            for name, m in self._packables():
                if name in names:
                    m.pin_precision = 2
        return audit

# ... 244 lines not shown
```

articulation3d_amd/modeling/roi_heads/axis_head.py:

```python
from __future__ import annotations

import numpy as np
import torch
from torch import nn

from ... import ops
from ...registry import ROI_AXIS_HEAD_REGISTRY
from ...structures import ShapeSpec
from ..layers import ACT_RELU, Conv2d, Linear, c2_msra_fill, c2_xavier_fill, to_nhwc
from .plane_head import head_fc


@ROI_AXIS_HEAD_REGISTRY.register()
class PlaneRCNNConvFCHead(nn.Module):
    def __init__(self, cfg, input_shape: ShapeSpec):
        super().__init__()
        h = cfg.MODEL.ROI_AXIS_HEAD
        assert h.NORM == "", "reference config: ROI_AXIS_HEAD.NORM ''"
        self._output_size = (input_shape.channels, input_shape.height, input_shape.width)
        self.smooth_l1_beta = h.SMOOTH_L1_BETA
        self.conv_norm_relus_R, self.conv_norm_relus_T = [], []
        for k in range(h.NUM_CONV):
            for t, lst in (("R", self.conv_norm_relus_R), ("T", self.conv_norm_relus_T)):
                conv = Conv2d(self._output_size[0], h.CONV_DIM, 3, padding=1, act=ACT_RELU)
                self.add_module(f"axis_{t}_conv{k + 1}", conv)
                lst.append(conv)
            self._output_size = (h.CONV_DIM, self._output_size[1], self._output_size[2])
        self.fcs_R, self.fcs_T = [], []
        for k in range(h.NUM_FC):
            chw = self._output_size if isinstance(self._output_size, tuple) else None
            for t, lst in (("R", self.fcs_R), ("T", self.fcs_T)):
                fc = Linear(int(np.prod(self._output_size)), h.FC_DIM, chw=chw, act=ACT_RELU)
                self.add_module(f"axis_{t}_fc{k + 1}", fc)
                lst.append(fc)
            self._output_size = h.FC_DIM
        self.rotation = Linear(h.FC_DIM, 2)
        self.offset = Linear(h.FC_DIM, 1)
        self.translation = Linear(h.FC_DIM, 2)
        for layer in self.conv_norm_relus_R + self.conv_norm_relus_T:
            c2_msra_fill(layer.weight, layer.bias)
        for layer in self.fcs_R + self.fcs_T:
            c2_xavier_fill(layer.weight, layer.bias)
        self._loss_weight = h.LOSS_WEIGHT
        self.keep_raw, self.raw = False, None

    @property
    def output_size(self):
        return self._output_size

    def _tower(self, x, convs, fcs):
        for layer in convs:
            x = layer(x, wino=True)
        x = ops.keep_amax(x.reshape(x.shape[0], -1), x)
        for fc in fcs:
            x = head_fc(x, fc)
        return x

    def forward_rows(self, x):
        xr = self._tower(x, self.conv_norm_relus_R, self.fcs_R)
        w = torch.cat((self.rotation.weight, self.offset.weight), 0).contiguous()
        b = torch.cat((self.rotation.bias, self.offset.bias), 0).contiguous()
        rot = ops.linear_small(xr, w, b, norm_n=2)
        xt = self._tower(x, self.conv_norm_relus_T, self.fcs_T)
        tran = ops.linear_small(xt, self.translation.weight, self.translation.bias, norm_n=2)
        if self.keep_raw:
            self.raw = (ops.linear_small(xr, w, b, norm_n=0), ops.linear_small(xt, self.translation.weight, self.translation.bias, norm_n=0))
        return rot, tran

    def forward(self, x, instances):
        if self.training:
            raise NotImplementedError("axis loss (training) is outside the inference hot path (SURVEY.md 8f-1)")
        if x.shape[0]:
            rot, tran = self.forward_rows(to_nhwc(x))
        else:
            rot, tran = x.new_zeros((0, 3)), x.new_zeros((0, 2))
        arti_inference(rot, tran, instances)
        return instances


def arti_inference(pred_rot_axis, pred_tran_axis, pred_instances):
    n = [len(i) for i in pred_instances]
    for r_axis, t_axis, instances in zip(pred_rot_axis.split(n, dim=0), pred_tran_axis.split(n, dim=0), pred_instances):
        instances.pred_rot_axis = r_axis
        instances.pred_tran_axis = t_axis


def build_axis_head(cfg, input_shape):
    return ROI_AXIS_HEAD_REGISTRY.get(cfg.MODEL.ROI_AXIS_HEAD.NAME)(cfg, input_shape)
```

articulation3d_amd/modeling/roi_heads/plane_head.py:

```python
from __future__ import annotations

import numpy as np
import torch
from torch import nn

from ... import ops
from ...registry import ROI_PLANE_HEAD_REGISTRY
from ...structures import ShapeSpec
from ..layers import ACT_RELU, Conv2d, Linear, c2_msra_fill, c2_xavier_fill, to_nhwc


def head_fc(x_rows: torch.Tensor, fc: Linear) -> torch.Tensor:
    M, K = x_rows.shape
    p = fc.packed()
    return ops.linear(x_rows, p, splitk=ops.choose_splitk(M, p.cols, K))


@ROI_PLANE_HEAD_REGISTRY.register()
class PlaneRCNNConvFCHead(nn.Module):
    def __init__(self, cfg, input_shape: ShapeSpec):
        super().__init__()
        h = cfg.MODEL.ROI_PLANE_HEAD
        assert h.NORM == "", "reference config: ROI_PLANE_HEAD.NORM ''"
        self._plane_normal_only = h.NORMAL_ONLY
        self._output_size = (input_shape.channels, input_shape.height, input_shape.width)
        self.conv_norm_relus = []
        for k in range(h.NUM_CONV):
            conv = Conv2d(self._output_size[0], h.CONV_DIM, 3, padding=1, act=ACT_RELU)
            self.add_module(f"plane_conv{k + 1}", conv)
            self.conv_norm_relus.append(conv)
            self._output_size = (h.CONV_DIM, self._output_size[1], self._output_size[2])
        self.fcs = []
        for k in range(h.NUM_FC):
            chw = self._output_size if isinstance(self._output_size, tuple) else None
            fc = Linear(int(np.prod(self._output_size)), h.FC_DIM, chw=chw, act=ACT_RELU)
            self.add_module(f"plane_fc{k + 1}", fc)
            self.fcs.append(fc)
            self._output_size = h.FC_DIM
        self.param_pred = Linear(h.FC_DIM, h.PARAM_DIM)
        for layer in self.conv_norm_relus:
            c2_msra_fill(layer.weight, layer.bias)
        for layer in self.fcs:
            c2_xavier_fill(layer.weight, layer.bias)
        self._loss_weight = h.LOSS_WEIGHT
        self.keep_raw, self.raw = False, None

    @property
    def output_size(self):
        return self._output_size

    def forward_rows(self, x):
        for layer in self.conv_norm_relus:
            x = layer(x, wino=True)
        x = ops.keep_amax(x.reshape(x.shape[0], -1), x)
        for fc in self.fcs:
            x = head_fc(x, fc)
        n = self.param_pred.out_features
        if self.keep_raw:
            self.raw = ops.linear_small(x, self.param_pred.weight, self.param_pred.bias, norm_n=0)
        return ops.linear_small(x, self.param_pred.weight, self.param_pred.bias,
                                norm_n=n if self._plane_normal_only else 0)

    def forward(self, x, instances):
        if self.training:
            raise NotImplementedError("the module-level call has no autograd path: the plane head trains through training_plane.PlaneTrainer "
                                      "(configs/step3_planehead.yaml; PlaneRCNN.trainer())")
        planes = self.forward_rows(to_nhwc(x)) if x.shape[0] else x.new_zeros((0, self.param_pred.out_features))
        plane_rcnn_inference(planes, instances)
        return instances


def plane_rcnn_inference(plane_pred, pred_instances):
    num_boxes_per_image = [len(i) for i in pred_instances]
    for plane, instances in zip(plane_pred.split(num_boxes_per_image, dim=0), pred_instances):
        instances.pred_plane = plane


def build_plane_head(cfg, input_shape):
    return ROI_PLANE_HEAD_REGISTRY.get(cfg.MODEL.ROI_PLANE_HEAD.NAME)(cfg, input_shape)
```

articulation3d_amd/ops.py:

```python
from __future__ import annotations

import ctypes as C
import math
import os
from dataclasses import dataclass
from typing import List, Optional, Sequence, Tuple

import torch

from . import _lib
from ._lib import ACT_LEAKY, ACT_NONE, ACT_RELU

GROUP_CAP = 1024
fptr_t = C.c_void_p

CONV_TIMING: Optional[list] = None

DEFAULT_PRECISION = int(os.environ.get("A3D_PRECISION", "3"))


def last_conv_variant() -> str:
    return _lib.lib().a3d_last_conv_variant().decode()


_raw_stream, _raw_device = getattr(torch._C, "_cuda_getCurrentRawStream", None), getattr(torch._C, "_cuda_getDevice", None)


def _stream() -> int:
    if _raw_stream is not None and _raw_device is not None:
        return _raw_stream(_raw_device())
    return torch.cuda.current_stream().cuda_stream


def _p(t: Optional[torch.Tensor]) -> Optional[int]:
    return None if t is None else t.data_ptr()


def _req(t: torch.Tensor, dtype=torch.float32) -> torch.Tensor:
    if not t.is_cuda:
        raise RuntimeError("articulation3d_amd ops need CUDA/HIP tensors (there is no CPU fallback)")
    if t.dtype != dtype or not t.is_contiguous():
        raise RuntimeError(f"expected contiguous {dtype} tensor, got {t.dtype} contiguous={t.is_contiguous()}")
    return t


@dataclass
class PackedConv:
    w: torch.Tensor
    scale: Optional[torch.Tensor]
    shift: Optional[torch.Tensor]
    KH: int
    KW: int
    stride: int
    pad: int
    Cin: int
    cols: int
    Kpad: int
    act: int = ACT_NONE
    pixshuf: bool = False
    stem: bool = False
    w_wino: Optional[torch.Tensor] = None
    w_wino_x3: Optional[torch.Tensor] = None
    w_wino_cm: Optional[torch.Tensor] = None
    phase: int = 0
    presplit: bool = False
    w_x3: Optional[torch.Tensor] = None
    w_wino_h2: Optional[torch.Tensor] = None
    w_h2: Optional[torch.Tensor] = None
    w_b16: Optional[torch.Tensor] = None
    pin_precision: Optional[int] = None
    name: str = ""

    @property
    def out_channels(self) -> int:
        return self.cols // 4 if self.pixshuf else self.cols


def _pad_rows(t: torch.Tensor, mult: int = 4) -> torch.Tensor:
    n = t.shape[0]
    n_pad = (n + mult - 1) // mult * mult
    if n_pad == n:
        return t
    out = t.new_zeros((n_pad,) + tuple(t.shape[1:]))
    out[:n] = t
    return out


def fold_bn(weight, bias, mean, var, eps, conv_bias=None):
    scale = weight * torch.rsqrt(var + eps)
    shift = bias - mean * scale
    if conv_bias is not None:
        shift = shift + conv_bias * scale
    return scale, shift


def pack_conv(weight: torch.Tensor, bias=None, bn=None, stride=1, pad=0, act=ACT_NONE, device="cuda") -> PackedConv:
    Cout, Cin, KH, KW = weight.shape
    if Cin % 32:
        raise ValueError("generic conv path needs Cin % 32 == 0")
    w = weight.detach().float().permute(0, 2, 3, 1).reshape(Cout, KH * KW * Cin)
    scale = shift = None
    if bn is not None:
        scale, shift = fold_bn(*[t.detach().float() for t in bn[:4]], bn[4], None if bias is None else bias.detach().float())
    elif bias is not None:
        shift = bias.detach().float()
    w = _pad_rows(w)
    cols = w.shape[0]
    if scale is not None:
        scale = _pad_rows(scale)
    if shift is not None:
        shift = _pad_rows(shift)
    dev = lambda t: None if t is None else t.contiguous().to(device)
    pk = PackedConv(dev(w), dev(scale), dev(shift), KH, KW, stride, pad, Cin, cols, KH * KW * Cin, act, presplit=True)
    if KH == 3 and KW == 3 and stride == 1 and pad == 1 and Cin % 16 == 0:
        U = winograd_weights(_pad_rows(weight.detach().float()))
        pk.w_wino = dev(U)
        pk.w_wino_cm = dev(winograd_weights_chunk_major(U))
    return pk


def pack_conv_ups_phases(weight: torch.Tensor, bias=None, bn=None, act=ACT_NONE, device="cuda") -> List[PackedConv]:
    Cout, Cin, KH, KW = weight.shape
    assert KH == 3 and KW == 3 and Cin % 32 == 0
    w = weight.detach().double()
    groups = {0: ((0,), (1, 2)), 1: ((0, 1), (2,))}
    scale = shift = None
    if bn is not None:
        scale, shift = fold_bn(*[t.detach().float() for t in bn[:4]], bn[4], None if bias is None else bias.detach().float())
    elif bias is not None:
        shift = bias.detach().float()
    dev = lambda t: None if t is None else t.contiguous().to(device)
    scale_d, shift_d = dev(None if scale is None else _pad_rows(scale)), dev(None if shift is None else _pad_rows(shift))
    out = []
    for dy in (0, 1):
        for dx in (0, 1):
            wp = w.new_zeros(Cout, Cin, 2, 2)
            for a, khs in enumerate(groups[dy]):
                for b, kws in enumerate(groups[dx]):
                    for kh in khs:
                        for kw in kws:
                            wp[:, :, a, b] += w[:, :, kh, kw]
            wk = _pad_rows(wp.float().permute(0, 2, 3, 1).reshape(Cout, 4 * Cin))
            out.append(PackedConv(dev(wk), scale_d, shift_d, 2, 2, 1, 0, Cin, wk.shape[0], 4 * Cin, act, phase=1 + dy * 2 + dx, presplit=True))
    common = _pow2_scale_host(max(float(q.w.abs().max()) for q in out))
    for q in out:
        q._w_scale = common
    return out


def pack_conv_ups_fused(phases: Sequence[PackedConv]) -> Optional[PackedConv]:
    p0 = phases[0]
    Cout, CinT = p0.cols, p0.Cin
    if Cout % 32 or CinT % 32 or any(q.cols != Cout or q.Cin != CinT or q.phase != i + 1 for i, q in enumerate(phases)):
        return None
    dev = p0.w.device
    w = torch.zeros((4 * Cout, 3, 3, CinT), device=dev, dtype=torch.float32)
    co = torch.arange(Cout, device=dev)
    for ph, q in enumerate(phases):
        dy, dx = ph >> 1, ph & 1
        col = (co // 32) * 128 + 32 * ph + (co % 32)
        w[col, dy:dy + 2, dx:dx + 2, :] = q.w[:Cout].view(Cout, 2, 2, CinT)
    col_of = torch.empty(4 * Cout, dtype=torch.int64, device=dev)
    j = torch.arange(4 * Cout, device=dev)
    col_of = (j // 128) * 32 + (j % 32)
    scale = None if p0.scale is None else p0.scale[col_of].contiguous()
    shift = None if p0.shift is None else p0.shift[col_of].contiguous()
    return PackedConv(w.reshape(4 * Cout, 9 * CinT).contiguous(), scale, shift, 3, 3, 1, 1, CinT, 4 * Cout, 9 * CinT, p0.act, phase=5, presplit=True)


_WINO_G = ((1.0, 0.0, 0.0), (0.5, 0.5, 0.5), (0.5, -0.5, 0.5), (0.0, 0.0, 1.0))


def winograd_weights(weight: torch.Tensor) -> torch.Tensor:
    G = torch.tensor(_WINO_G, dtype=torch.float64, device=weight.device)
    U = torch.einsum("up,ncpq,vq->uvnc", G, weight.double(), G)
    return U.reshape(16, weight.shape[0], weight.shape[1]).float().contiguous()


def winograd_weights_chunk_major(U: torch.Tensor) -> torch.Tensor:
    f, n, c = U.shape
    nt = (n + 63) // 64
    Up = U.new_zeros((f, nt * 64, c))
    Up[:, :n] = U
    v = Up.view(f, nt, 64, c // 8, 2, 4)
    return v.permute(3, 0, 1, 4, 2, 5).contiguous()


def pack_stem(weight: torch.Tensor, bn, device="cuda") -> PackedConv:
    Cout = weight.shape[0]
    w = weight.new_zeros(Cout, 7, 8, 4)
    w[:, :, :7, :3] = weight.detach().float().permute(0, 2, 3, 1)
    scale, shift = fold_bn(*[t.detach().float() for t in bn[:4]], bn[4])
    return PackedConv(w.reshape(Cout, 224).contiguous().to(device), scale.contiguous().to(device),
                      shift.contiguous().to(device), 7, 7, 2, 3, 4, Cout, 224, ACT_RELU, stem=True, presplit=True)


def pack_linear(weight: torch.Tensor, bias=None, chw: Optional[Tuple[int, int, int]] = None, act=ACT_NONE,
                device="cuda") -> PackedConv:
    N, K = weight.shape
    w = weight.detach().float()
    if chw is not None:
        c, h, ww = chw
        w = w.view(N, c, h, ww).permute(0, 2, 3, 1).reshape(N, K)
    if K % 32:
        raise ValueError("K % 32 != 0")
    w = _pad_rows(w)
    shift = None if bias is None else _pad_rows(bias.detach().float())
    dev = lambda t: None if t is None else t.contiguous().to(device)
    return PackedConv(dev(w), None, dev(shift), 1, 1, 1, 0, K, w.shape[0], K, act, presplit=True)


def pack_deconv2x2(weight: torch.Tensor, bias, act=ACT_RELU, device="cuda") -> PackedConv:
    Cin, Cout = weight.shape[:2]
    w = weight.detach().float().permute(2, 3, 1, 0).reshape(4 * Cout, Cin)
    shift = bias.detach().float().repeat(4)
    return PackedConv(w.contiguous().to(device), None, shift.contiguous().to(device), 1, 1, 1, 0, Cin, 4 * Cout, Cin,
                      act, pixshuf=True, presplit=True)


def pack_fused_rows(weights: Sequence[torch.Tensor], biases: Sequence[torch.Tensor], device="cuda") -> PackedConv:
    w = torch.cat([x.detach().float().reshape(x.shape[0], -1) for x in weights], 0)
    b = torch.cat([x.detach().float() for x in biases], 0)
    K = w.shape[1]
    w = _pad_rows(w)
    b = _pad_rows(b)
    return PackedConv(w.contiguous().to(device), None, b.contiguous().to(device), 1, 1, 1, 0, K, w.shape[0], K, ACT_NONE, presplit=True)


WINO_PLANE_SPLIT = os.environ.get("A3D_WINO_PLANE_SPLIT", "1") != "0"
_AMAX_CHUNK = 1 << 18
AMAX_MISSES: Optional[list] = None
_amax_arena: dict = {}


def amax_reserve(n: int, device) -> None:
    a = _amax_arena.get(device)
    if a is None or a[1] + n > a[0].numel():
        _amax_arena[device] = [torch.zeros(max(_AMAX_CHUNK, n), device=device, dtype=torch.float32), 0]


def publish() -> None:
    torch.cuda.current_stream().synchronize()


def amax_slot(n: int, device) -> torch.Tensor:
    a = _amax_arena.get(device)
    if a is None or a[1] + n > a[0].numel():
        amax_reserve(n, device)
        a = _amax_arena[device]
        publish()
    t = a[0][a[1]:a[1] + n]
    a[1] += (n + 3) // 4 * 4
    return t


def amax_of(x: torch.Tensor) -> torch.Tensor:
    a = getattr(x, "_a3d_amax", None)
    if a is not None and a.numel() == x.shape[0] and a.device == x.device:
        return a
    if AMAX_MISSES is not None:
        AMAX_MISSES.append(tuple(x.shape))
    a = amax_slot(x.shape[0], x.device)
    _lib.check(_lib.lib().a3d_absmax_rows(x.data_ptr(), a.data_ptr(), x.shape[0], x.numel() // x.shape[0], _stream()), "a3d_absmax_rows")
    x._a3d_amax = a
    return a


def keep_amax(new: torch.Tensor, old: torch.Tensor) -> torch.Tensor:
    a = getattr(old, "_a3d_amax", None)
    if a is not None and new.shape[0] == old.shape[0]:
        new._a3d_amax = a
    return new


def _const_amax(t: torch.Tensor, bound: float) -> None:
    if DEFAULT_PRECISION == 3:
        t._a3d_amax = torch.full((t.shape[0],), float(bound), device=t.device, dtype=torch.float32)


def _pow2_scale_host(amax: float) -> float:
    return 1.0 if not (amax > 0.0) else 2.0 ** (14 - math.frexp(amax)[1] + 1)


def filter_scale(p: PackedConv, wino: bool = False) -> float:
    name = "_u_scale" if wino else "_w_scale"
    s = getattr(p, name, None)
    if s is None:
        s = _pow2_scale_host(float((p.w_wino if wino else p.w).abs().max()))
        setattr(p, name, s)
    return s


def weight_planes(p: PackedConv, kind: str) -> int:
    wino = kind.startswith("w_wino")
    src = p.w_wino if wino else p.w
    t = getattr(p, kind)
    if t is not None and t.device == src.device:
        return t.data_ptr()
    h2 = kind.endswith("h2")
    n, rows, k, c = (16, src.shape[1], src.shape[2], 32) if wino else (1, src.shape[0], p.Kpad, 16)
    t = torch.empty(((16,) if wino else ()) + (k // c, 2 if h2 else 3, rows, c), device=src.device, dtype=torch.float16 if h2 else torch.bfloat16)
    L = _lib.lib()
    if h2:
        _lib.check(L.a3d_split_f16x2_chunk(src.data_ptr(), t.data_ptr(), n, rows, k, c, filter_scale(p, wino), _stream()), "a3d_split_f16x2_chunk")
    elif wino:
        _lib.check(L.a3d_split_bf16x3(src.data_ptr(), t.data_ptr(), 16, rows, k, _stream()), "a3d_split_bf16x3")
    else:
        _lib.check(L.a3d_split_bf16x3_chunk(src.data_ptr(), t.data_ptr(), 1, rows, k, 16, _stream()), "a3d_split_bf16x3_chunk")
    setattr(p, kind, t)
    publish()
    return t.data_ptr()


def _conv_desc(p: PackedConv, B: int, H: int, W: int, Cin: int, Cin2: int, Ho: int, Wo: int, act: Optional[int] = None,
               res_ups: bool = False) -> "_lib.ConvDesc":
    d = _lib.ConvDesc()
    d.w, d.scale, d.shift = _p(p.w), _p(p.scale), _p(p.shift)
    d.B, d.H, d.W, d.Cin, d.Cin2 = B, H, W, Cin, Cin2
    d.Ho, d.Wo, d.Cout = Ho, Wo, p.cols
    d.KH, d.KW, d.stride, d.pad = p.KH, p.KW, p.stride, p.pad
    d.Kpad, d.act = p.Kpad, p.act if act is None else act
    d.res_ups, d.pixshuf, d.stem, d.phase, d.splitk = int(res_ups), int(p.pixshuf), int(p.stem), int(p.phase), 1
    return d


def _y_amax(out: torch.Tensor) -> int:
    ya = getattr(out, "_a3d_amax", None)
    if ya is None or ya.numel() != out.shape[0]:
        ya = out._a3d_amax = amax_slot(out.shape[0], out.device)
    return ya.data_ptr()


def _image_blocks(B: int, nb: int, *ts):
    for s in range(0, B, nb):
        e = min(s + nb, B)
        yield s, e, [t if t is None or e - s == B else keep_amax(t[s:e], _amax_rows(t, s, e)) for t in ts]


CONV_TIMING_ONLY: Optional[frozenset] = None
_TIMED_VARIANTS: dict = {}
_ERR_UNSUPPORTED = -3


def _launch(fn, *args, precision: Optional[int] = None, rec=None, unsupported: bool = False) -> bool:
    global _LAST_PRECISION
    if precision is not None:
        _LAST_PRECISION = precision
    timed = CONV_TIMING is not None and rec is not None
    if timed:
        label, fl, shape, ex, pipe, key = rec()
        if CONV_TIMING_ONLY is not None:
            known = label if label is not None else _TIMED_VARIANTS.get(key)
            timed = known is None or known in CONV_TIMING_ONLY
        if timed:
            e0, e1 = (torch.cuda.Event(enable_timing=True) for _ in range(2))
            e0.record()
    rc = fn(*args, _stream())
    if rc:
        if unsupported and rc == _ERR_UNSUPPORTED:
            return False
        _lib.check(rc, fn.__name__)
    if timed:
        e1.record()
        if label is None:
            label = _TIMED_VARIANTS[key] = last_conv_variant()
        CONV_TIMING.append((label, fl, e0, e1, shape, ex, pipe, _stream()))
    return True


_WINO_SHARE: Optional[dict] = None
WINO_SHARE_ENABLED = os.environ.get("A3D_WINO_SHARE", "1") != "0"


class share_wino_input:

    def __init__(self, tensors: Sequence[torch.Tensor]):
        self.map = {t.data_ptr(): [t, None] for t in tensors} if WINO_SHARE_ENABLED else {}

    def __enter__(self):
        global _WINO_SHARE
        self.prev, _WINO_SHARE = _WINO_SHARE, self.map
        return self

    def __exit__(self, *exc):
        global _WINO_SHARE
        _WINO_SHARE = self.prev
        self.map = {}
        return False


_ADDR_LIMIT = (1 << 32) - 1
WINO_LEVELS = os.environ.get("A3D_WINO_LEVELS", "1") != "0"


def conv2d_levels(xs: Sequence[torch.Tensor], p: PackedConv) -> list:
    xs = list(xs)
    ok = (WINO_LEVELS and DEFAULT_PRECISION == 3 and AUDIT is None and 2 <= len(xs) <= 5 and p.w_wino is not None
          and p.pin_precision != 2 and p.KH == 3 and p.stride == 1 and p.pad == 1 and not (p.stem or p.phase or p.pixshuf)
          and all(x.is_cuda and x.dtype == torch.float32 and x.shape[0] == xs[0].shape[0] and x.shape[3] == p.Cin for x in xs)
          and p.Cin % 32 == 0 and p.Cin >= 256 and -(-p.cols // 64) % 2 == 0)
    if ok and _WINO_SHARE is not None:
        ok = all((_WINO_SHARE.get(x.data_ptr()) or [None, None])[1] is None for x in xs)
    tiles = [x.shape[0] * ((x.shape[1] + 1) // 2) * ((x.shape[2] + 1) // 2) for x in xs]
    total = sum(tiles)
    if not ok or total * p.Cin * 4 > _ADDR_LIMIT:
        return [conv2d(x, p) for x in xs]
    dev = xs[0].device
    w_h2, u_scale = weight_planes(p, "w_wino_h2"), filter_scale(p, wino=True)
    ws = torch.empty(16 * total * p.Cin, device=dev, dtype=torch.float32)
    descs = (_lib.ConvDesc * len(xs))()
    outs, off = [], 0
    shape = lambda: f"{xs[0].shape[0]}x[{'+'.join(str(x.shape[1]) + 'x' + str(x.shape[2]) for x in xs)}]x{p.Cin}->{p.cols} k3 s1"
    for k, x in enumerate(xs):
        _req(x)
        B, H, W, Cin = x.shape
        out = torch.empty((B, H, W, p.cols), device=dev, dtype=torch.float32)
        descs[k] = _conv_desc(p, B, H, W, Cin, 0, H, W)
        d = descs[k]
        d.x, d.y, d.precision = _p(x), _p(out), 3
        d.w_wino, d.w_wino_x3, d.w_scale = p.w_wino.data_ptr(), w_h2, u_scale
        d.in_amax = amax_of(x).data_ptr()
        d.y_amax = _y_amax(out)
        d.workspace = ws.data_ptr()
        d.wino_t_off, d.wino_t_total = off, total
        _launch(_lib.lib().a3d_wino_input_transform, C.byref(d), precision=3, rec=lambda: ("wino_input_kernel", 0.0, shape(), 0.0, "none", None))
        if _WINO_SHARE is not None:
            ent = _WINO_SHARE.get(x.data_ptr())
            if ent is not None and ent[0].shape == x.shape:
                ent[1:] = [ws, 3, (off, total)]
        off += tiles[k]
        outs.append(out)

    def rec():
        px = sum(x.shape[0] * x.shape[1] * x.shape[2] for x in xs)
        return "wino_gemm_h2w_kernel<4>", 2.0 * px * p.cols * 9 * p.Cin, shape(), 2.0 * total * 16 * p.cols * p.Cin, "f16x3", None

    _launch(_lib.lib().a3d_wino_gemm_levels, descs, len(xs), precision=3, rec=rec)
    return outs


def conv2d(x: torch.Tensor, p: PackedConv, *, x2: Optional[torch.Tensor] = None, res: Optional[torch.Tensor] = None,
           res_ups: bool = False, ups: bool = False, act: Optional[int] = None, splitk: int = 1,
           m_dev: Optional[torch.Tensor] = None, out: Optional[torch.Tensor] = None, tune: int = 0,
           wino: Optional[bool] = None, gate: Optional[torch.Tensor] = None, precision=None, out_dtype=None, dot=None) -> torch.Tensor:
    if AUDIT is not None and not AUDIT.busy and precision is None and x.dtype == torch.float32 and out_dtype is None and not p.phase:
        return AUDIT.conv2d(x, p, x2=x2, res=res, res_ups=res_ups, ups=ups, act=act, splitk=splitk, m_dev=m_dev, out=out, tune=tune, wino=wino, gate=gate)
    if x.dtype == torch.float16:
        if splitk != 1 or m_dev is not None or gate is not None or tune or out_dtype is not None or ups or dot is not None or wino or precision not in (None, 3):
            raise RuntimeError("pre-split (float16) activations run the dual-DMA fp16x2 kernel only: splitk, m_dev, gate, tune, out_dtype, ups, dot, "
                               "wino and any precision other than 3 are not available with them")
        return _conv2d_presplit(x, p, x2=x2, res=res, res_ups=res_ups, act=act, out=out)
    if out_dtype is not None or x.dtype == torch.bfloat16 or (res is not None and res.dtype == torch.bfloat16) or (gate is not None and gate.dtype == torch.bfloat16):
        return _conv2d_bf16_storage(x, p, res=res, res_ups=res_ups, act=act, out=out, gate=gate, precision=precision, out_dtype=out_dtype, tune=tune)
    _req(x)
    B = x.shape[0]
    if B > 1:
        Hl_, Wl_ = (2 * x.shape[1], 2 * x.shape[2]) if ups else (x.shape[1], x.shape[2])
        Ho_ = x.shape[1] if p.phase else (Hl_ + 2 * p.pad - p.KH) // p.stride + 1
        Wo_ = x.shape[2] if p.phase else (Wl_ + 2 * p.pad - p.KW) // p.stride + 1
        per_in = x.shape[1] * x.shape[2] * max(x.shape[3], 0 if x2 is None else x2.shape[3]) * 4
        per_out = Ho_ * Wo_ * p.cols * 4 * (4 if 0 < p.phase < 5 else 1) * max(1, int(splitk))
        if dot is not None:
            per_out = 9 * 4 * Ho_ * Wo_ * 4
        per_v = ((Hl_ + 1) // 2) * ((Wl_ + 1) // 2) * (x.shape[3] + (0 if x2 is None else x2.shape[3])) * 4 if p.w_wino is not None else 0
        per = max(per_in, per_out, per_v, 1)
        if B * per > _ADDR_LIMIT:
            if dot is not None:
                raise RuntimeError("tap-product epilogue (dot): the batch must fit one launch")
            return _conv2d_blocks(x, p, max(1, _ADDR_LIMIT // per), (Ho_, Wo_), x2=x2, res=res, res_ups=res_ups, ups=ups, act=act, splitk=splitk,
                                  m_dev=m_dev, out=out, tune=tune, wino=wino, gate=gate, precision=precision)
    return _conv2d_launch(x, p, x2=x2, res=res, res_ups=res_ups, ups=ups, act=act, splitk=splitk, m_dev=m_dev, out=out, tune=tune,
                          wino=wino, gate=gate, precision=precision, dot=dot)


def _conv2d_blocks(x, p, nb, hw_out, *, x2, res, out, gate, m_dev, **kw):
    B = x.shape[0]
    Ho, Wo = hw_out
    if out is None:
        shape = (B, 2 * Ho, 2 * Wo, p.cols // 4) if p.pixshuf else (B, Ho, Wo, p.cols)
        out = torch.empty(shape, device=x.device, dtype=torch.float32)
    recorded = []
    for s, e, (xb, x2b, rb, gb) in _image_blocks(B, nb, x, x2, res, gate):
        md = None if m_dev is None else (m_dev.reshape(1) - s).clamp(0, e - s).to(torch.int32)
        o = out[s:e]
        ya = getattr(out, "_a3d_amax", None)
        if ya is not None and ya.numel() == B:
            o._a3d_amax = ya[s:e]
        _conv2d_launch(xb, p, x2=x2b, res=rb, out=o, gate=gb, m_dev=md, **kw)
        recorded.append(getattr(o, "_a3d_amax", None))
    if getattr(out, "_a3d_amax", None) is None and all(r is not None for r in recorded):
        out._a3d_amax = torch.cat(recorded)
    return out


BF16_SPLITK = os.environ.get("A3D_BF16_SPLITK", "1") != "0"
BF16_SPLITK_AUTO = False
_BF16_SK_CFG = tuple(int(v) for v in os.environ.get("A3D_BF16_SPLITK_CFG", "128,256,12,24,8").split(","))


def _bf16_splitk(M: int, cols: int, Kpad: int) -> int:
    tiles = -(-M // 128) * -(-cols // 64)
    nk = Kpad // 32
    maxtiles, target, per, minnk, cap = _BF16_SK_CFG
    if not BF16_SPLITK or tiles > maxtiles or nk < minnk:
        return 1
    return int(max(1, min(cap, nk // per, target // tiles)))


_BF16_DESC_CACHE: dict = {}


def _conv2d_bf16_storage(x, p: PackedConv, *, res, res_ups, act, out, gate, precision, out_dtype, tune=0) -> torch.Tensor:
    if precision != 1:
        raise RuntimeError("bf16-stored tensors belong to the bf16 arithmetic (precision=1): the fp32-grade modes keep fp32 tensors")
    ok = lambda t: t is None or (t.is_cuda and t.is_contiguous() and t.dtype in (torch.float32, torch.bfloat16))
    if not (ok(x) and ok(res) and ok(gate) and ok(out)):
        raise RuntimeError("expected contiguous fp32 / bf16 CUDA tensors")
    B, H, W, Cin = x.shape
    assert Cin == p.Cin and not (p.stem or p.pixshuf or p.phase), "plain layers only"
    Ho = (H + 2 * p.pad - p.KH) // p.stride + 1
    Wo = (W + 2 * p.pad - p.KW) // p.stride + 1
    if out is None:
        out = torch.empty((B, Ho, Wo, p.cols), device=x.device, dtype=out_dtype or torch.float32)
    if B * max(H * W * Cin, Ho * Wo * p.cols) * 4 > _ADDR_LIMIT:
        raise RuntimeError("tensor past the 32-bit addressing limit of one launch: split the batch")
    if gate is not None:
        assert tuple(gate.shape) == tuple(out.shape), (gate.shape, out.shape)
    act_eff = p.act if act is None else act
    key = (p.w.data_ptr(), _p(p.scale), _p(p.shift), _p(p.w_b16), p.KH, p.KW, p.stride, p.pad, p.Kpad, p.cols, act_eff, B, H, W, Cin,
           x.dtype, out.dtype, None if res is None else res.dtype, None if gate is None else gate.dtype, bool(res_ups), int(tune), BF16_SPLITK_AUTO, BF16_SPLITK)
    proto = _BF16_DESC_CACHE.get(key)
    if proto is None:
        d = _conv_desc(p, B, H, W, Cin, 0, Ho, Wo, act=act_eff, res_ups=res_ups)
        d.precision = 1
        b16 = lambda t: t is not None and t.dtype == torch.bfloat16
        d.io_bf16 = (1 if b16(x) else 0) | (2 if b16(out) else 0) | (4 if b16(res) else 0) | (8 if b16(gate) else 0)
        d.tune = int(tune)
        if p.w_b16 is not None:
            d.w_bf16 = p.w_b16.data_ptr()
        sk = 1 if (res_ups or not BF16_SPLITK_AUTO) else _bf16_splitk(B * Ho * Wo, p.cols, p.Kpad)
        d.splitk = sk
        if len(_BF16_DESC_CACHE) > 4096:
            _BF16_DESC_CACHE.clear()
        proto = _BF16_DESC_CACHE[key] = (bytes(d), sk)
    d = _lib.ConvDesc.from_buffer_copy(proto[0])
    sk = proto[1]
    d.x, d.y = x.data_ptr(), out.data_ptr()
    if res is not None:
        d.res = res.data_ptr()
    if gate is not None:
        d.gate = gate.data_ptr()
    if sk > 1:
        ws = torch.empty(sk * B * Ho * Wo * p.cols, device=x.device, dtype=torch.float32)
        d.workspace = ws.data_ptr()

    def rec():
        fl = 2.0 * B * Ho * Wo * p.cols * p.KH * p.KW * p.Cin
        return None, fl, f"{B}x{H}x{W}x{Cin}->{p.cols} k{p.KH} s{p.stride} io{int(d.io_bf16)}", fl, "bf16", key

    _launch(_lib.lib().a3d_conv2d_nhwc_f32, C.byref(d), precision=1, rec=rec)
    return out


def presplit_f16x2(x: torch.Tensor, x2: Optional[torch.Tensor] = None):
    _req(x)
    B, n = x.shape[0], x.numel() // x.shape[0]
    ax, ax2 = amax_of(x), (None if x2 is None else amax_of(_req(x2)))
    outs = []
    for t in ((x,) if x2 is None else (x, x2)):
        nt = t.numel() // B
        o = torch.empty(tuple(t.shape[:-1]) + (t.shape[-1] // 16, 2, 16), device=t.device, dtype=torch.float16)
        _lib.check(_lib.lib().a3d_presplit_f16x2(t.data_ptr(), o.data_ptr(), ax.data_ptr(), _p(ax2), B, nt, _stream()), "a3d_presplit_f16x2")
        o._a3d_amax = ax if x2 is None else torch.maximum(ax, ax2)
        outs.append(o)
    return outs[0] if x2 is None else tuple(outs)


def _conv2d_presplit(x, p: PackedConv, *, x2=None, res=None, res_ups=False, act=None, out=None) -> torch.Tensor:
    if DEFAULT_PRECISION != 3:
        raise RuntimeError("pre-split activations belong to the fp16x2 arithmetic (A3D_PRECISION=3)")
    ok = lambda t: t.is_cuda and t.is_contiguous() and t.dtype == torch.float16 and t.dim() == 6 and t.shape[4:] == (2, 16)
    if not ok(x) or (x2 is not None and not ok(x2)):
        raise RuntimeError("expected contiguous pre-split fp16 tensors [B, H, W, C/16, 2, 16]")
    B, H, W = x.shape[:3]
    Cin = x.shape[3] * 16
    Cin2 = 0 if x2 is None else x2.shape[3] * 16
    assert Cin + Cin2 == p.Cin and not (p.stem or p.pixshuf or p.phase) and p.presplit and p.Kpad == p.KH * p.KW * p.Cin, "plain direct layers only"
    Ho = (H + 2 * p.pad - p.KH) // p.stride + 1
    Wo = (W + 2 * p.pad - p.KW) // p.stride + 1
    if out is None:
        out = torch.empty((B, Ho, Wo, p.cols), device=x.device, dtype=torch.float32)
    per_image = max(H * W * max(Cin, Cin2), Ho * Wo * p.cols) * 4
    if B * per_image > _ADDR_LIMIT:
        ya = out._a3d_amax = amax_slot(B, x.device)
        for s, e, (xb, x2b, rb) in _image_blocks(B, max(1, _ADDR_LIMIT // per_image), x, x2, res):
            o = out[s:e]
            o._a3d_amax = ya[s:e]
            _conv2d_presplit(xb, p, x2=x2b, res=rb, res_ups=res_ups, act=act, out=o)
        return out
    a = getattr(x, "_a3d_amax", None)
    if a is None or a.numel() != B:
        raise RuntimeError("a pre-split tensor carries the per-image maxima it was scaled by (_a3d_amax)")
    d = _conv_desc(p, B, H, W, Cin, Cin2, Ho, Wo, act=act, res_ups=res_ups)
    d.x_h2, d.x2_h2, d.res, d.y = x.data_ptr(), _p(x2), _p(res), out.data_ptr()
    d.precision = 3
    d.tune = int(os.environ.get("A3D_XD_TUNE", "0"))
    d.in_amax = a.data_ptr()
    d.w_scale, d.w_x3 = filter_scale(p), weight_planes(p, "w_h2")
    d.y_amax = _y_amax(out)

    def rec():
        fl = 2.0 * B * Ho * Wo * p.cols * p.KH * p.KW * p.Cin
        return None, fl, f"{B}x{H}x{W}x{Cin + Cin2}->{p.cols} k{p.KH} s{p.stride} presplit", fl, "f16x3", (id(p), B, H, W, Cin, Cin2, "presplit")

    _launch(_lib.lib().a3d_conv2d_nhwc_f32, C.byref(d), precision=3, rec=rec)
    return out


class _amax_rows:

    def __init__(self, t, s, e):
        a = getattr(t, "_a3d_amax", None)
        self._a3d_amax = None if a is None or a.numel() != t.shape[0] else a[s:e]
        self.shape = (e - s,)


def _check_res(res: torch.Tensor, B: int, Ho: int, Wo: int, cols: int, res_ups: bool) -> None:
    _req(res)
    want = (B, Ho >> 1, Wo >> 1, cols) if res_ups else (B, Ho, Wo, cols)
    if tuple(res.shape) != want or (res_ups and (Ho % 2 or Wo % 2)):
        raise ValueError(f"residual of shape {tuple(res.shape)} for an output grid [{B}, {Ho}, {Wo}, {cols}]{' (res_ups)' if res_ups else ''}: expected {want}")


_PIPE = {0: "f32", 1: "bf16", 2: "bf16x6", 3: "f16x3"}


def _arithmetic(p: PackedConv, default: int, wino_tune: int, precision, Cin: int, Cin2: int, *, ups: bool, splitk: int, tune: int, wino,
                x2: bool, res: bool, gate: bool, m_dev: bool) -> Tuple[int, bool, int]:
    wino_ok = (p.w_wino is not None and not res and splitk == 1 and not m_dev and (tune in (0, 7, 8, 23, 24, 25) or tune >= 200) and not ups
               and (wino if wino is not None else True))
    if precision is None or precision == "bf16x3":
        mode = default if precision is None else 2
        if mode == 3 and p.pin_precision == 2:
            mode = 2
        plain = not (p.stem or ups or p.phase or p.pixshuf or x2 or splitk != 1 or m_dev) and p.Kpad == p.KH * p.KW * p.Cin
        if mode == 1:
            precision = 1 if plain and p.Cin % 32 == 0 else 0
        elif mode in (2, 3):
            x3_ok = p.stem and not ups and splitk == 1 and not m_dev and not x2 and not res
            x3_ok = x3_ok or (not (p.stem or ups or m_dev) and p.Kpad == p.KH * p.KW * p.Cin
                     and not (p.pixshuf and (res or gate))
                     and (splitk == 1 or (p.presplit and p.Kpad >= 4096 and p.cols >= 192 and -(-p.cols // 256) * 256 <= p.cols + p.cols // 4
                                          and not p.phase and not gate and not p.pixshuf))
                     and (not x2 or Cin2 == Cin) and Cin % 16 == 0 and not (p.phase and res))
            precision = 2 if tune == 0 and ((x3_ok and not wino_ok) or (wino_ok and (Cin + Cin2) % 32 == 0)) else 0
            if precision == 2 and mode == 3:
                precision = 3
        else:
            precision = 0
    use_wino = wino_ok and (precision == 0 or (precision in (2, 3) and tune in (0, 8, 23, 24, 25) and (Cin + Cin2) % 32 == 0))
    if use_wino and precision == 3 and (-(-p.cols // 64) % 2 or (Cin + Cin2 < 256 and wino is None)):
        use_wino = False
    if use_wino and precision == 3 and tune == 0 and wino_tune:
        tune = wino_tune
    return int(precision), use_wino, int(tune)


def _conv2d_launch(x: torch.Tensor, p: PackedConv, *, x2: Optional[torch.Tensor] = None, res: Optional[torch.Tensor] = None,
                   res_ups: bool = False, ups: bool = False, act: Optional[int] = None, splitk: int = 1,
                   m_dev: Optional[torch.Tensor] = None, out: Optional[torch.Tensor] = None, tune: int = 0,
                   wino: Optional[bool] = None, gate: Optional[torch.Tensor] = None, precision=None, dot=None) -> torch.Tensor:
    _req(x)
    plan_key = None
    if (LAUNCH_PLANS and CONV_TIMING is None and x2 is None and m_dev is None and out is None and gate is None and dot is None and not ups and splitk == 1
            and tune == 0 and wino is None and precision is None and act is None and not (p.phase or p.pixshuf or p.stem) and p.presplit
            and (_WINO_SHARE is None or x.data_ptr() not in _WINO_SHARE)):
        plan_key = (DEFAULT_PRECISION, WINO_TUNE, p.pin_precision, x.shape, None if res is None else tuple(res.shape), bool(res_ups),
                    WINO_PLANE_SPLIT, BF16_SPLITK_AUTO, BF16_SPLITK, x.device, p.w.data_ptr())
        plans = p.__dict__.get("_plans")
        plan = plans.get(plan_key) if plans else None
        if plan is not None:
            proto, oshape, need_in, need_y, ws_n, m_n, prec = plan
            out = torch.empty(oshape, device=x.device, dtype=torch.float32)
            d = _lib.ConvDesc.from_buffer_copy(proto)
            d.x, d.y = x.data_ptr(), out.data_ptr()
            if res is not None:
                _check_res(res, oshape[0], d.Ho, d.Wo, d.Cout, res_ups)
                d.res = res.data_ptr()
            if need_in:
                d.in_amax = amax_of(x).data_ptr()
            if need_y:
                ya = out._a3d_amax = amax_slot(oshape[0], x.device)
                d.y_amax = ya.data_ptr()
            if ws_n:
                ws = torch.empty(ws_n, device=x.device, dtype=torch.float32)
                d.workspace = ws.data_ptr()
            if m_n:
                wino_m = torch.empty(m_n, device=x.device, dtype=torch.float32)
                d.wino_m = wino_m.data_ptr()
            _launch(_lib.lib().a3d_conv2d_nhwc_f32, C.byref(d), precision=prec)
            return out
    B, H, W, Cin = x.shape
    Cin2 = 0
    if x2 is not None:
        _req(x2)
        Cin2 = x2.shape[3]
        assert x2.shape[:3] == x.shape[:3]
    if not p.stem:
        assert Cin + Cin2 == p.Cin, (Cin, Cin2, p.Cin)
    Hl, Wl = (2 * H, 2 * W) if ups else (H, W)
    Ho = (Hl + 2 * p.pad - p.KH) // p.stride + 1
    Wo = (Wl + 2 * p.pad - p.KW) // p.stride + 1
    if p.phase:
        assert not ups and out is not None, "phase convs run on the source grid and fill a shared [B,2H,2W,C] output"
        Ho, Wo = H, W
        if p.phase == 5:
            assert precision in (2, 3) and (dot is not None or tuple(out.shape) == (B, 2 * H, 2 * W, p.cols // 4)), "the fused four-phase form belongs to the split-operand arithmetics"
    if res is not None:
        _check_res(res, B, Ho, Wo, p.cols, res_ups)
    if out is None:
        shape = (B, 2 * Ho, 2 * Wo, p.cols // 4) if p.pixshuf else (B, Ho, Wo, p.cols)
        out = torch.empty(shape, device=x.device, dtype=torch.float32)
    d = _conv_desc(p, B, H, W, Cin, Cin2, Ho, Wo, act=act, res_ups=res_ups)
    d.x, d.x2, d.res, d.y = _p(x), _p(x2), _p(res), _p(out)
    d.ups, d.splitk, d.m_dev = int(ups), int(splitk), _p(m_dev)
    if gate is not None:
        assert tuple(_req(gate).shape) == tuple(out.shape), (gate.shape, out.shape)
        d.gate = gate.data_ptr()
    if dot is not None:
        assert p.phase == 5 and precision == 3
        d.dot_w, d.dot_y = _req(dot[0]).data_ptr(), _req(dot[1]).data_ptr()
        d.y = None
    precision, use_wino, tune = _arithmetic(p, DEFAULT_PRECISION, WINO_TUNE, precision, Cin, Cin2, ups=ups, splitk=splitk, tune=tune, wino=wino,
                                            x2=x2 is not None, res=res is not None, gate=gate is not None, m_dev=m_dev is not None)
    d.precision, d.tune = precision, tune
    if precision == 1 and p.w_b16 is not None:
        d.w_bf16 = p.w_b16.data_ptr()
    if (precision == 1 and splitk == 1 and BF16_SPLITK_AUTO and not (p.stem or ups or p.phase or p.pixshuf or x2 is not None or m_dev is not None or res_ups)
            and p.Kpad == p.KH * p.KW * p.Cin and p.Cin % 32 == 0):
        splitk = _bf16_splitk(B * Ho * Wo, p.cols, p.Kpad)
        d.splitk = splitk
    if precision == 3:
        d.in_amax = amax_of(x).data_ptr()
        if x2 is not None:
            d.in_amax2 = amax_of(x2).data_ptr()
        d.w_scale = filter_scale(p)
    if precision in (2, 3) and (DEFAULT_PRECISION == 3 or precision == 3) and not p.pixshuf:
        d.y_amax = _y_amax(out)
    if use_wino:
        d.w_wino = p.w_wino.data_ptr()
        if p.w_wino_cm is not None and precision == 0 and tune == 0:
            d.w_wino_cm = p.w_wino_cm.data_ptr()
        if precision == 3:
            d.w_scale = filter_scale(p, wino=True)
            d.w_wino_x3 = weight_planes(p, "w_wino_h2")
        elif precision == 2:
            d.w_wino_x3 = weight_planes(p, "w_wino_x3")
    elif precision == 3 and p.presplit and p.Kpad % 16 == 0:
        d.w_x3 = weight_planes(p, "w_h2")
    elif (precision == 2 and p.presplit and p.cols >= 192 and p.Kpad % 16 == 0 and (p.Kpad >= 4096 or tune == 9 or p.phase == 5)
            and not (p.stem or p.pixshuf)):
        d.w_x3 = weight_planes(p, "w_x3")
    ws = None
    fused_wino = False
    shared = None
    nbytes = mbytes = 0
    if use_wino or splitk > 1:
        if use_wino and _WINO_SHARE is not None and x2 is None:
            shared = _WINO_SHARE.get(x.data_ptr())
            if shared is not None and (shared[0].shape != x.shape or tune not in (0, 23, 24)):
                shared = None
            if shared is not None and shared[1] is not None and len(shared) > 2 and shared[2] != precision:
                shared = None
        if shared is not None:
            d.w_wino_cm = None
            if len(shared) > 3 and shared[1] is not None:
                d.wino_t_off, d.wino_t_total = shared[3]
        nbytes = _lib.lib().a3d_conv_workspace_bytes(C.byref(d))
        fused_wino = use_wino and nbytes == 0
        if shared is not None and shared[1] is not None:
            ws = shared[1]
            assert ws.numel() * 4 == nbytes
            d.workspace = ws.data_ptr()
        elif nbytes:
            ws = torch.empty(nbytes // 4, device=x.device, dtype=torch.float32)
            d.workspace = ws.data_ptr()
        if use_wino and precision == 3 and WINO_PLANE_SPLIT:
            mbytes = _lib.lib().a3d_wino_m_bytes(C.byref(d))
            if mbytes:
                wino_m = torch.empty(mbytes // 4, device=x.device, dtype=torch.float32)
                d.wino_m = wino_m.data_ptr()
    have_v = False
    if shared is not None:
        have_v, shared[1] = shared[1] is not None, ws
        if len(shared) > 2:
            shared[2] = precision
        else:
            shared.append(precision)

    def rec(label=None):
        k_real = 147 if p.stem else p.KH * p.KW * p.Cin
        shape = f"{B}x{H}x{W}x{Cin + Cin2}->{p.cols} k{p.KH} s{p.stride}{' ups' if ups else ''}{' sk%d' % splitk if splitk > 1 else ''}"
        if label is not None:
            return label, 0.0, shape, 0.0, "none", None
        fl = 2.0 * B * Ho * Wo * p.cols * (9 * p.Cin if p.phase else k_real)
        if use_wino:
            ex = 2.0 * B * ((Ho + 1) // 2) * ((Wo + 1) // 2) * 16 * p.cols * p.Cin
        else:
            ex = 2.0 * B * Ho * Wo * p.cols * (4 * p.Cin if p.phase == 5 else k_real)
        return None, fl, shape, ex, _PIPE[precision], (id(p), B, H, W, bool(ups), int(splitk), precision, tune, res is not None, x2 is not None, shared is not None)

    L = _lib.lib()
    if use_wino and not fused_wino and (shared is not None or CONV_TIMING is not None):
        if not have_v:
            _launch(L.a3d_wino_input_transform, C.byref(d), precision=precision, rec=lambda: rec("wino_input_kernel"))
        _launch(L.a3d_wino_gemm, C.byref(d), precision=precision, rec=rec)
        return out
    _launch(L.a3d_conv2d_nhwc_f32, C.byref(d), precision=precision, rec=rec)
    if plan_key is not None:
        if p.__dict__.get("_plans") is None or len(p._plans) > 64:
            p._plans = {}
        p._plans[plan_key] = (bytes(d), tuple(out.shape), bool(d.in_amax), bool(d.y_amax), nbytes // 4 if ws is not None else 0,
                              mbytes // 4 if d.wino_m else 0, precision)
    return out


LAUNCH_PLANS = os.environ.get("A3D_LAUNCH_PLANS", "1") != "0"
B2B_FUSED = os.environ.get("A3D_B2B", "1") != "0"
B2B_MIN_PIXELS = 128 * 512
B2B_PAIRS = ((64, 64),)


def conv2d_b2b(x: torch.Tensor, p1: PackedConv, res: torch.Tensor, p2: PackedConv):
    if not B2B_FUSED or DEFAULT_PRECISION != 3 or AUDIT is not None or not x.is_cuda or x.dtype != torch.float32:
        return None
    B, H, W, Cin = x.shape
    M = B * H * W
    if (p1.KH, p1.KW, p1.stride, p1.pad, p2.KH, p2.KW, p2.stride, p2.pad) != (1, 1, 1, 0, 1, 1, 1, 0) or p1.pin_precision == 2:
        return None
    if (Cin, p2.cols) not in B2B_PAIRS or p1.Cin != Cin or p2.Cin != p1.cols or p1.cols % 64 or not (p1.presplit and p2.presplit):
        return None
    if p1.Kpad != Cin or p2.Kpad != p2.Cin or p1.pixshuf or p2.pixshuf or p1.phase or p2.phase or p1.stem or p2.stem:
        return None
    if M < B2B_MIN_PIXELS or M * p1.cols * 4 >= (1 << 31) or res is None or tuple(res.shape) != (B, H, W, p1.cols):
        return None
    _req(x)
    _req(res)
    y = torch.empty((B, H, W, p1.cols), device=x.device, dtype=torch.float32)
    z = torch.empty((B, H, W, p2.cols), device=x.device, dtype=torch.float32)
    d1, d2 = _conv_desc(p1, B, H, W, Cin, 0, H, W), _conv_desc(p2, B, H, W, p2.Cin, 0, H, W)
    d1.x, d1.res, d1.y, d1.y_amax = x.data_ptr(), res.data_ptr(), y.data_ptr(), _y_amax(y)
    d2.x, d2.y, d2.y_amax = y.data_ptr(), z.data_ptr(), _y_amax(z)
    d1.precision, d2.precision = 3, 2
    d1.in_amax = amax_of(x).data_ptr()
    d1.w_scale = filter_scale(p1)
    d1.w_x3, d2.w_x3 = weight_planes(p1, "w_h2"), weight_planes(p2, "w_x3")

    def rec():
        fl, ex = 2.0 * M * (p1.cols * Cin + p2.cols * p2.Cin), 2.0 * M * (p1.cols * Cin + 2 * p2.cols * p2.Cin)
        return None, fl, f"{B}x{H}x{W}x{Cin}->{p1.cols}->{p2.cols} k1 b2b", ex, "f16x3", (id(p1), id(p2), B, H, W)

    if not _launch(_lib.lib().a3d_conv_b2b, C.byref(d1), C.byref(d2), precision=3, rec=rec, unsupported=True):
        return None
    return y, z


WINO_TUNE = int(os.environ.get("A3D_WINO_TUNE", "0"))
UPS_FUSED = os.environ.get("A3D_UPS_FUSED", "1") != "0"


def conv2d_ups(x: torch.Tensor, phases: Sequence[PackedConv], *, x2: Optional[torch.Tensor] = None, fused: Optional[bool] = None, tune: int = 0) -> torch.Tensor:
    B, H, W, _ = x.shape
    if AUDIT is not None and not AUDIT.busy and fused is None:
        return AUDIT.conv2d_ups(x, phases, x2)
    out = torch.empty((B, 2 * H, 2 * W, phases[0].cols), device=x.device, dtype=torch.float32)
    pinned = phases[0].pin_precision == 2
    if fused is None:
        fused = UPS_FUSED and DEFAULT_PRECISION in (2, 3)
    if fused:
        pf = getattr(phases[0], "_fused", None)
        if pf is None:
            pf = pack_conv_ups_fused(phases)
            phases[0]._fused = pf if pf is not None else False
        if pf:
            pf.name = getattr(phases[0], "name", "")
        b3 = pinned or DEFAULT_PRECISION == 2
        if pf and b3 and (pf.cols < 192 or pf.cols * pf.Kpad * 6 >= 2 ** 31):
            pf = None
        if pf:
            return conv2d(x, pf, x2=x2, out=out, precision=2 if b3 else 3, tune=tune)
    for p in phases:
        conv2d(x, p, x2=x2, out=out)
    return out


DEPTH_PRED_FUSED = os.environ.get("A3D_DEPTH_PRED_FUSED", "1") != "0"


def conv2d_ups_to1(x: torch.Tensor, phases: Sequence[PackedConv], w9: torch.Tensor, bias: float, *, x2: Optional[torch.Tensor] = None) -> Optional[torch.Tensor]:
    pinned = phases[0].pin_precision == 2
    if not (DEPTH_PRED_FUSED and UPS_FUSED and DEFAULT_PRECISION == 3 and not pinned and AUDIT is None and phases[0].cols == 64):
        return None
    B, H, W, C = x.shape
    pf = getattr(phases[0], "_fused", None)
    if pf is None:
        pf = pack_conv_ups_fused(phases)
        phases[0]._fused = pf if pf is not None else False
    if not pf:
        return None
    per_image = max(9 * 4 * H * W * 4, H * W * C * 4, 0 if x2 is None else x2.shape[1] * x2.shape[2] * x2.shape[3] * 4)
    y = torch.empty((B, 2 * H, 2 * W), device=x.device, dtype=torch.float32)
    w9 = w9.reshape(9, 64)
    for b0, b1, (xb, x2b) in _image_blocks(B, max(1, _ADDR_LIMIT // per_image), x, x2):
        g = torch.empty((b1 - b0, 9, 2 * H, 2 * W), device=x.device, dtype=torch.float32)
        conv2d(xb, pf, x2=x2b, out=g, precision=3, dot=(w9, g))
        _lib.check(_lib.lib().a3d_tapsum9(g.data_ptr(), float(bias), y[b0:b1].data_ptr(), b1 - b0, 2 * H, 2 * W, _stream()), "a3d_tapsum9")
    return y


_LAST_PRECISION = -1
AUDIT = None


class PrecisionAudit:

    def __init__(self, pin: bool = True, slack: float = 1.25):
        self.pin, self.slack, self.busy = pin, slack, False
        self.rows = []

    def __enter__(self):
        global AUDIT
        self._prev, AUDIT = AUDIT, self
        return self

    def __exit__(self, *exc):
        global AUDIT
        AUDIT = self._prev
# ... 59 lines not shown
            S = torch.empty_like(y)
            for p in phases:
                conv2d(x, p, x2=x2, out=out2, precision="bf16x3")
                conv2d(x.abs(), self._abs_pack(p), x2=None if x2 is None else x2.abs(), out=S, precision="bf16x3")
            row = self._judge(phases[0], variant, tuple(x.shape) + ("ups",), y, out2, S, 4 * phases[0].Cin, False)
            if row["pinned"]:
                for p in phases:
                    p.pin_precision = 2
            return y
        finally:
            self.busy = False

    def pinned(self):
        return [r for r in self.rows if r["pinned"]]


def linear(x: torch.Tensor, p: PackedConv, *, act: Optional[int] = None, splitk: int = 1,
           m_dev: Optional[torch.Tensor] = None, precision=None) -> torch.Tensor:
    if x.dtype == torch.float16:
        M = x.shape[0]
        y = conv2d(x, p, act=act, splitk=splitk, m_dev=m_dev, precision=precision)
        return keep_amax(y.view(M, p.cols), y)
    M, K = x.shape
    y = conv2d(keep_amax(x.view(M, 1, 1, K), x), p, act=act, splitk=splitk, m_dev=m_dev, precision=precision)
    return keep_amax(y.view(M, p.cols), y)


def choose_splitk(M: int, cols: int, K: int) -> int:
    return 32 if K >= 16384 else 1


def _f3(v):
    return (C.c_float * 3)(*[float(t) for t in v])


def preprocess_u8hwc(frames: torch.Tensor, mean, std) -> torch.Tensor:
    _req(frames, torch.uint8)
    B, H, W, _ = frames.shape
    out = torch.empty((B, H, W, 4), device=frames.device, dtype=torch.float32)
    _lib.check(_lib.lib().a3d_preprocess_u8hwc(frames.data_ptr(), out.data_ptr(), B, H, W, _f3(mean), _f3(std), _stream()),
               "a3d_preprocess_u8hwc")
    _const_amax(out, max(max(abs(0.0 - m), abs(255.0 - m)) / sd for m, sd in zip(mean, std)))
    return out


def preprocess_resize_u8(frames: torch.Tensor, mean, std, out_hw=(480, 640), swap_rb: bool = True, want_u8: bool = False):
    _req(frames, torch.uint8)
    B, Hs, Ws, _ = frames.shape
    Hd, Wd = int(out_hw[0]), int(out_hw[1])
    out = torch.empty((B, Hd, Wd, 4), device=frames.device, dtype=torch.float32)
    u8 = torch.empty((B, Hd, Wd, 3), device=frames.device, dtype=torch.uint8) if want_u8 else None
    _lib.check(_lib.lib().a3d_preprocess_resize_u8(frames.data_ptr(), out.data_ptr(), _p(u8), B, Hs, Ws, Hd, Wd, int(bool(swap_rb)),
                                                   _f3(mean), _f3(std), _stream()), "a3d_preprocess_resize_u8")
    _const_amax(out, max(max(abs(0.0 - m), abs(255.0 - m)) / sd for m, sd in zip(mean, std)))
    return (out, u8) if want_u8 else out


def preprocess_f32chw(images: torch.Tensor, mean, std) -> torch.Tensor:
    _req(images)
    B, _, H, W = images.shape
    out = torch.empty((B, H, W, 4), device=images.device, dtype=torch.float32)
    _lib.check(_lib.lib().a3d_preprocess_f32chw(images.data_ptr(), out.data_ptr(), B, H, W, _f3(mean), _f3(std), _stream()),
               "a3d_preprocess_f32chw")
    return out


STEM_POOL_FUSED = os.environ.get("A3D_STEM_POOL", "1") != "0"


def stem_pool(x: torch.Tensor, p: "PackedConv") -> Optional[torch.Tensor]:
    if not (STEM_POOL_FUSED and DEFAULT_PRECISION == 3 and p.stem and p.presplit and p.pin_precision != 2 and AUDIT is None and p.cols == 64):
        return None
    _req(x)
    B, H, W, _ = x.shape
    if B * H * W * 16 >= (1 << 31) or p.Kpad != 224 or p.w.shape[0] != 64:
        return None
    Ho, Wo = (H + 6 - 7) // 2 + 1, (W + 6 - 7) // 2 + 1
    Hp, Wp = (Ho - 1) // 2 + 1, (Wo - 1) // 2 + 1
    out = torch.empty((B, Hp, Wp, 64), device=x.device, dtype=torch.float32)
    d = _conv_desc(p, B, H, W, 4, 0, Ho, Wo)
    d.KH, d.KW, d.stride, d.pad, d.Cout = 7, 7, 2, 3, 64
    d.x, d.y, d.precision = x.data_ptr(), out.data_ptr(), 3
    d.tune = int(os.environ.get("A3D_STEM_ABL", "0"))
    d.in_amax = amax_of(x).data_ptr()
    d.w_scale, d.w_x3 = filter_scale(p), weight_planes(p, "w_h2")
    d.y_amax = _y_amax(out)

    def rec():
        fl = 2.0 * B * Ho * Wo * 64 * 147
        return "stem_pool_kernel", fl, f"{B}x{H}x{W}x4->64 k7 s2 + pool", fl, "f16x3", None

    _launch(_lib.lib().a3d_stem_conv_pool, C.byref(d), precision=3, rec=rec)
    return out


def maxpool3x3s2(x: torch.Tensor) -> torch.Tensor:
    _req(x)
    B, H, W, Cc = x.shape
    out = torch.empty((B, (H - 1) // 2 + 1, (W - 1) // 2 + 1, Cc), device=x.device, dtype=torch.float32)
    _lib.check(_lib.lib().a3d_maxpool3x3s2_nhwc(x.data_ptr(), out.data_ptr(), B, H, W, Cc, _stream()), "a3d_maxpool3x3s2_nhwc")
    keep_amax(out, x)
    return out


def subsample2(x: torch.Tensor) -> torch.Tensor:
    _req(x)
    B, H, W, Cc = x.shape
    out = torch.empty((B, (H - 1) // 2 + 1, (W - 1) // 2 + 1, Cc), device=x.device, dtype=torch.float32)
    _lib.check(_lib.lib().a3d_subsample2_nhwc(x.data_ptr(), out.data_ptr(), B, H, W, Cc, _stream()), "a3d_subsample2_nhwc")
    keep_amax(out, x)
    return out


def resize_bilinear(x: torch.Tensor, Ho: int, Wo: int) -> torch.Tensor:
    _req(x)
    B, H, W, Cc = x.shape
    out = torch.empty((B, Ho, Wo, Cc), device=x.device, dtype=torch.float32)
    _lib.check(_lib.lib().a3d_resize_bilinear_nhwc(x.data_ptr(), out.data_ptr(), B, H, W, Cc, Ho, Wo, _stream()),
               "a3d_resize_bilinear_nhwc")
    keep_amax(out, x)
    return out


def conv3x3_to1(x: torch.Tensor, w: torch.Tensor, bias: float) -> torch.Tensor:
    _req(x)
    _req(w)
    B, H, W, Cc = x.shape
    out = torch.empty((B, H, W), device=x.device, dtype=torch.float32)
    _lib.check(_lib.lib().a3d_conv3x3_to1_nhwc(x.data_ptr(), w.data_ptr(), float(bias), out.data_ptr(), B, H, W, Cc, _stream()),
               "a3d_conv3x3_to1_nhwc")
    return out


def group_workspace(n_groups: int, device) -> torch.Tensor:
    return torch.empty(_lib.lib().a3d_group_buffers_bytes(n_groups), device=device, dtype=torch.uint8)


def _selection_workspace(workspace, nbytes: int, device) -> torch.Tensor:
    if workspace is None:
        return torch.empty(nbytes, device=device, dtype=torch.uint8)
    if workspace.dtype != torch.uint8 or not workspace.is_contiguous() or workspace.device != torch.device(device):
        raise ValueError("workspace: a contiguous uint8 tensor on the launch's device is needed")
    if workspace.numel() < nbytes or workspace.data_ptr() % 16:
        raise ValueError(f"workspace: {workspace.numel()} bytes at {workspace.data_ptr():#x}, {nbytes} bytes 16-byte aligned are needed")
    return workspace


def carve_group_workspace(ws: torch.Tensor, G: int) -> dict:
    cap = GROUP_CAP
    o = 0
    out = {}
    for name, width, dt in (("boxes", 16, torch.float32), ("scores", 4, torch.float32), ("pos", 4, torch.int32),
                            ("valid", 4, torch.int32), ("keep", 4, torch.int32)):
        nbytes = G * cap * width
        t = ws[o:o + nbytes].view(dt)
        out[name] = t.view(G, cap, 4) if name == "boxes" else t.view(G, cap)
        o += nbytes
    out["n"] = ws[o:o + G * 4].view(torch.int32)
    return out


def rpn_proposals(heads: Sequence[torch.Tensor], strides: Sequence[int], cell_anchors: torch.Tensor, img_hw, *,
                  pre_topk: int, post_topk: int, nms_thresh: float, min_size: float, weights, scale_clamp: float,
                  return_groups: bool = False, workspace: Optional[torch.Tensor] = None):
    L = len(heads)
    B = heads[0].shape[0]
    dev = heads[0].device
# ... 31 lines not shown
def box_detections(pred: torch.Tensor, prop_boxes: torch.Tensor, prop_count: torch.Tensor, img_hw, *, num_classes: int,
                   score_thresh: float, nms_thresh: float, topk: int, weights, scale_clamp: float,
                   return_groups: bool = False, workspace: Optional[torch.Tensor] = None):
    _req(pred)
    _req(prop_boxes)
    _req(prop_count, torch.int32)
    B, R, _ = prop_boxes.shape
    dev = pred.device
    d = _lib.BoxDetDesc()
    d.pred, d.prop_boxes, d.prop_count = pred.data_ptr(), prop_boxes.data_ptr(), prop_count.data_ptr()
    d.B, d.R, d.C, d.CH = B, R, int(num_classes), pred.shape[1]
    d.img_h, d.img_w = int(img_hw[0]), int(img_hw[1])
    d.score_thresh, d.nms_thresh, d.topk = float(score_thresh), float(nms_thresh), int(topk)
    for j in range(4):
        d.weights[j] = float(weights[j])
    d.scale_clamp = float(scale_clamp)
    ws = _selection_workspace(workspace, _lib.lib().a3d_group_buffers_bytes(B * num_classes), dev)
    boxes = torch.empty((B, topk, 4), device=dev, dtype=torch.float32)
    scores = torch.empty((B, topk), device=dev, dtype=torch.float32)
    classes = torch.empty((B, topk), device=dev, dtype=torch.int32)
    pos = torch.empty((B, topk), device=dev, dtype=torch.int32)
    count = torch.empty((B,), device=dev, dtype=torch.int32)
    d.workspace = ws.data_ptr()
    d.out_boxes, d.out_scores, d.out_classes, d.out_pos, d.out_count = (boxes.data_ptr(), scores.data_ptr(),
                                                                        classes.data_ptr(), pos.data_ptr(), count.data_ptr())
    _lib.check(_lib.lib().a3d_box_detections(C.byref(d), _stream()), "a3d_box_detections")
    if return_groups:
        return boxes, scores, classes, pos, count, carve_group_workspace(ws, B * num_classes)
    return boxes, scores, classes, pos, count


def group_nms(g_boxes: torch.Tensor, g_valid: torch.Tensor, g_n: torch.Tensor, thresh: float) -> torch.Tensor:
    _req(g_boxes)
    _req(g_valid, torch.int32)
    _req(g_n, torch.int32)
    G = g_boxes.shape[0]
    assert g_boxes.shape[1] == GROUP_CAP
    keep = torch.empty((G, GROUP_CAP), device=g_boxes.device, dtype=torch.int32)
    _lib.check(_lib.lib().a3d_group_nms(g_boxes.data_ptr(), g_valid.data_ptr(), g_n.data_ptr(), keep.data_ptr(), G,
                                        float(thresh), _stream()), "a3d_group_nms")
    return keep


ROI_SERIAL = False
ROI_SPATIAL_ORDER = True
ROI_ROLLING = os.environ.get("A3D_ROI_ROLLING", "1") != "0"


def roi_align_fpn(feats: Sequence[torch.Tensor], scales: Sequence[float], boxes: torch.Tensor,
                  count: Optional[torch.Tensor], P: int, sampling_ratio: int, aligned: bool, *,
                  row_offset: Optional[torch.Tensor] = None, rows: Optional[int] = None, want_level: bool = False,
                  zero: bool = False, presplit: bool = False):
    _req(boxes)
    B, R, _ = boxes.shape
    Cc = feats[0].shape[3]
    dev = boxes.device
    nrows = B * R if rows is None else rows
    presplit = bool(presplit) and DEFAULT_PRECISION == 3 and Cc == 256 and P * P * Cc * 4 <= 120 * 1024
    if presplit:
        out = (torch.zeros if zero else torch.empty)((nrows, 1, 1, P * P * Cc // 16, 2, 16), device=dev, dtype=torch.float16)
    else:
        out = (torch.zeros if zero else torch.empty)((nrows, P, P, Cc), device=dev, dtype=torch.float32)
    lvl = torch.full((nrows,), -1, device=dev, dtype=torch.int32) if want_level else None
    d = _lib.RoiAlignDesc()
    for l, f in enumerate(feats):
        _req(f)
        d.feat[l] = f.data_ptr()
        d.Hf[l], d.Wf[l] = f.shape[1], f.shape[2]
        d.scale[l] = float(scales[l])
    d.L, d.C = len(feats), Cc
    d.boxes, d.count, d.row_offset = boxes.data_ptr(), _p(count), _p(row_offset)
    d.B, d.R, d.P, d.sampling_ratio, d.aligned = B, R, int(P), int(sampling_ratio), int(bool(aligned))
    d.out, d.out_level = (None if presplit else out.data_ptr()), _p(lvl)
    if presplit:
        d.out_h2 = out.data_ptr()
    order = torch.empty((B * R,), device=dev, dtype=torch.int32) if (512 <= R <= 1024 and ROI_SPATIAL_ORDER) else None
    d.order_ws = _p(order)
    d.serial = 1 if ROI_SERIAL else (2 if (ROI_ROLLING and P == 7 and not presplit) else 0)
    ra = None
    if DEFAULT_PRECISION == 3:
        ra = amax_slot(nrows, dev)
        d.out_amax = ra.data_ptr()
        for l, f in enumerate(feats):
            d.level_amax[l] = amax_of(f).data_ptr()
        d.window_count = window_counter(dev).data_ptr()
    _lib.check(_lib.lib().a3d_roi_align_fpn(C.byref(d), _stream()), "a3d_roi_align_fpn")
    if ra is not None:
        out._a3d_amax = ra
    return (out, lvl) if want_level else out


_WINDOW_COUNTERS: dict = {}


def window_counter(device) -> torch.Tensor:
    device = torch.device(device)
    if device.index is None:
        device = torch.device("cuda", torch.cuda.current_device())
    t = _WINDOW_COUNTERS.get(device)
    if t is None:
        t = _WINDOW_COUNTERS[device] = torch.zeros(1, device=device, dtype=torch.int32)
        torch.cuda.current_stream(device).synchronize()
    return t


def roi_window_count(device="cuda") -> int:
    return int(window_counter(device).item())


def count_offsets(count: torch.Tensor, cap: int) -> torch.Tensor:
    _req(count, torch.int32)
    B = count.shape[0]
    off = torch.empty((B + 1,), device=count.device, dtype=torch.int32)
    _lib.check(_lib.lib().a3d_count_offsets(count.data_ptr(), off.data_ptr(), B, int(cap), _stream()), "a3d_count_offsets")
    return off


def linear_small(x: torch.Tensor, w: torch.Tensor, bias: Optional[torch.Tensor], norm_n: int = 0, sigmoid: bool = False,
                 m_dev: Optional[torch.Tensor] = None) -> torch.Tensor:
    _req(x)
    _req(w)
    M, K = x.shape
    N = w.shape[0]
    y = torch.empty((M, N), device=x.device, dtype=torch.float32)
    _lib.check(_lib.lib().a3d_linear_small(x.data_ptr(), w.data_ptr(), _p(bias), y.data_ptr(), M, _p(m_dev), K, N, int(norm_n),
                                           int(sigmoid), _stream()), "a3d_linear_small")
    return y


def paste_lsq(boxes, scores, count, row_offset, mask_prob, normals, depth, img_hw, *, post_score_thresh=0.1,
              mask_thresh=0.5, focal=571.623718, cx=319.5, cy=239.5, want_masks=True, clip_boxes=True):
    _req(boxes)
    _req(scores)
    B, R, _ = boxes.shape
    H, W = int(img_hw[0]), int(img_hw[1])
    dev = boxes.device
    MS = mask_prob.shape[-1]
    masks = torch.empty((B, R, H, W), device=dev, dtype=torch.uint8) if want_masks else None
    planes = torch.empty((B, R, 3), device=dev, dtype=torch.float32)
    area = torch.empty((B, R), device=dev, dtype=torch.int32)
    keep = torch.empty((B, R), device=dev, dtype=torch.int32)
    out_boxes = torch.empty((B, R, 4), device=dev, dtype=torch.float32)
    d = _lib.PasteDesc()
    d.boxes, d.scores, d.count, d.row_offset = boxes.data_ptr(), scores.data_ptr(), count.data_ptr(), row_offset.data_ptr()
    d.mask_prob, d.normals, d.depth = mask_prob.data_ptr(), _p(normals), _p(depth)
    d.B, d.R, d.MS, d.H, d.W = B, R, MS, H, W
    d.post_score_thresh, d.mask_thresh = float(post_score_thresh), float(mask_thresh)
    d.focal, d.cx, d.cy = float(focal), float(cx), float(cy)
    d.clip_boxes = int(bool(clip_boxes))
    d.masks, d.planes, d.area, d.keep, d.out_boxes = _p(masks), planes.data_ptr(), area.data_ptr(), keep.data_ptr(), out_boxes.data_ptr()
    _lib.check(_lib.lib().a3d_paste_lsq(C.byref(d), _stream()), "a3d_paste_lsq")
    return masks, planes, area, keep, out_boxes


def record_floats(MS: int = 28) -> int:
    return int(_lib.lib().a3d_record_floats(MS))


def detections_pack(boxes, scores, classes, count, row_offset, keep, planes, rot_axis, tran_axis, mask_prob, MS=28):
    B, R, _ = boxes.shape
    dev = boxes.device
    rec = record_floats(MS)
    records = torch.empty((B, R, rec), device=dev, dtype=torch.float32)
    rec_count = torch.empty((B,), device=dev, dtype=torch.int32)
    d = _lib.PackDesc()
    d.boxes, d.scores, d.classes, d.count = boxes.data_ptr(), scores.data_ptr(), classes.data_ptr(), count.data_ptr()
    d.row_offset, d.keep = row_offset.data_ptr(), keep.data_ptr()
# ... 6 lines not shown
```

include/a3d.h:

```cpp
#ifndef A3D_H
#define A3D_H
#include <stddef.h>
#include <stdint.h>
#ifdef __cplusplus
extern "C" {
#endif

#define A3D_OK 0
#define A3D_ERR_ARG (-1)
#define A3D_ERR_LAUNCH (-2)
#define A3D_ERR_UNSUPPORTED (-3)

#define A3D_ACT_NONE 0
#define A3D_ACT_RELU 1
#define A3D_ACT_LEAKY 2

int a3d_version(void);
size_t a3d_struct_size(int id);

int a3d_preprocess_u8hwc(const uint8_t *frames , float *out, int B, int H, int W,
                         const float mean[3], const float std[3], void *stream);
int a3d_preprocess_f32chw(const float *images , float *out, int B, int H, int W,
                          const float mean[3], const float std[3], void *stream);

int a3d_preprocess_resize_u8(const uint8_t *frames , float *out, uint8_t *out_u8, int B, int Hs, int Ws, int Hd, int Wd,
                             int swap_rb, const float mean[3], const float std[3], void *stream);

typedef struct a3d_conv_desc {
    const float *x;
    const float *x2;
    const float *w;
    const float *scale;
    const float *shift;
    const float *res;
    float *y;
    float *workspace;
    int B, H, W, Cin, Cin2;
    int Ho, Wo, Cout;
    int KH, KW, stride, pad;
    int Kpad;
    int ups;
    int act;
    int res_ups;
    int pixshuf;
    int stem;
    int splitk;
    const int *m_dev;
    int tune;
    int phase;
    const float *w_wino;
    const float *gate;
    int precision;
    const void *w_wino_x3;
    const float *w_wino_cm;
    const void *w_x3;
    const float *in_amax;
    const float *in_amax2;
    float *y_amax;
    float w_scale;
    float *wino_m;
    int io_bf16;
    const void *x_h2;
    const void *x2_h2;
    const float *dot_w;
    float *dot_y;
    int wino_t_off, wino_t_total;
    const void *w_bf16;
} a3d_conv_desc;

size_t a3d_conv_workspace_bytes(const a3d_conv_desc *d);
size_t a3d_wino_m_bytes(const a3d_conv_desc *d);
int a3d_conv2d_nhwc_f32(const a3d_conv_desc *d, void *stream);
int a3d_stem_conv_pool(const a3d_conv_desc *d, void *stream);
int a3d_tapsum9(const float *g, float bias, float *y, int B, int H, int W, void *stream);
int a3d_split_bf16x3(const float *src, void *dst, int outer, int rows, int cols, void *stream);
int a3d_split_bf16x3_chunk(const float *src, void *dst, int outer, int rows, int cols, int chunk, void *stream);
int a3d_split_f16x2_chunk(const float *src, void *dst, int outer, int rows, int cols, int chunk, float scale, void *stream);
int a3d_presplit_f16x2(const float *x, void *dst, const float *amax, const float *amax2, int B, size_t n, void *stream);
int a3d_absmax_rows(const float *x, float *out, int B, size_t n, void *stream);

int a3d_wino_input_transform(const a3d_conv_desc *d, void *stream);
int a3d_wino_gemm(const a3d_conv_desc *d, void *stream);
int a3d_wino_gemm_levels(const a3d_conv_desc *levels, int n, void *stream);
int a3d_conv_b2b(const a3d_conv_desc *d1, const a3d_conv_desc *d2, void *stream);
const char *a3d_last_conv_variant(void);

int a3d_maxpool3x3s2_nhwc(const float *x, float *y, int B, int H, int W, int C, void *stream);
int a3d_subsample2_nhwc(const float *x, float *y, int B, int H, int W, int C, void *stream);

int a3d_resize_bilinear_nhwc(const float *x, float *y, int B, int H, int W, int C, int Ho, int Wo, void *stream);

int a3d_conv3x3_to1_nhwc(const float *x, const float *w, float bias, float *y, int B, int H, int W, int C,
                         void *stream);

typedef struct a3d_rpn_desc {
    const float *head[5];
    int Hf[5], Wf[5], stride[5];
    float cell_anchors[5][3][4];
    int B, L, A, CH;
    int img_h, img_w;
    int pre_topk, post_topk;
    float nms_thresh, min_size;
    float weights[4];
    float scale_clamp;
    void *workspace;
    float *out_boxes;
    float *out_scores;
    int *out_level;
    int *out_pos;
    int *out_count;
} a3d_rpn_desc;

size_t a3d_group_buffers_bytes(int n_groups);
size_t a3d_rpn_workspace_bytes(int B, int L, int pre_topk);
int a3d_rpn_proposals(const a3d_rpn_desc *d, void *stream);

typedef struct a3d_boxdet_desc {
    const float *pred;
    const float *prop_boxes;
    const int *prop_count;
    int B, R, C, CH;
    int img_h, img_w;
    float score_thresh, nms_thresh;
    int topk;
    float weights[4];
    float scale_clamp;
    void *workspace;
    float *out_boxes;
    float *out_scores;
    int *out_classes;
    int *out_pos;
    int *out_count;
} a3d_boxdet_desc;

int a3d_box_detections(const a3d_boxdet_desc *d, void *stream);

int a3d_group_nms(const float *g_boxes, const int *g_valid, const int *g_n, int *g_keep, int n_groups, float thresh,
                  void *stream);

typedef struct a3d_roialign_desc {
    const float *feat[4];
    int Hf[4], Wf[4];
    float scale[4];
    int L, C;
// ... 528 lines not shown
```

Before: 1573 frames/s.

## Spread per-image amax atomics across strided sub-slots for Winograd convs

Adds a block form for the per-image absolute-max record. Each image gets n sub-slots spaced by stride floats, so Winograd 3x3 convs write their atomicMax to a sub-slot picked by block and wave index instead of all hitting one address. Consumers reduce over the sub-slots when they read the input scale. This is meant to cut atomic contention on the amax reduction in the bottleneck conv2 layers. Readers pay a small extra reduction, and several paths (b2b, presplit, ROI align, multi-level) now reject the block form.

After: 1584 frames/s, median of 6. About the same (+0.7%).

```diff
diff --git a/articulation3d_amd/_lib.py b/articulation3d_amd/_lib.py
--- a/articulation3d_amd/_lib.py
+++ b/articulation3d_amd/_lib.py
@@ -34,8 +34,10 @@
         ("in_amax2", fptr),
         ("y_amax", fptr),
         ("w_scale", C.c_float),
+        ("y_amax_n", C.c_ubyte), ("y_amax_stride", C.c_ubyte), ("in_amax_n", C.c_ubyte), ("in_amax_stride", C.c_ubyte),
         ("wino_m", fptr),
         ("io_bf16", C.c_int),
+        ("in_amax2_n", C.c_ubyte), ("in_amax2_stride", C.c_ubyte),
         ("x_h2", fptr),
         ("x2_h2", fptr),
         ("dot_w", fptr),
diff --git a/articulation3d_amd/csrc/conv_common.h b/articulation3d_amd/csrc/conv_common.h
--- a/articulation3d_amd/csrc/conv_common.h
+++ b/articulation3d_amd/csrc/conv_common.h
@@ -74,9 +74,12 @@
     return ldexpf(1.f, min(14 - ilogbf(amax), 126));
 }
 __device__ __forceinline__ float a3d_in_scale(const a3d_conv_desc &d, const int b) {
-    float a = d.in_amax[b];
-    if (d.in_amax2) a = fmaxf(a, d.in_amax2[b]);
+    float a = a3d_amax_get(d.in_amax, b, d.in_amax_n, d.in_amax_stride);
+    if (d.in_amax2) a = fmaxf(a, a3d_amax_get(d.in_amax2, b, d.in_amax2_n, d.in_amax2_stride));
     return a3d_pow2_scale(a);
+}
+inline bool a3d_amax_form_ok(const a3d_conv_desc *d) {
+    return (!d->y_amax_n || d->y_amax_stride >= 1) && (!d->in_amax_n || d->in_amax_stride >= 1) && (!d->in_amax2_n || d->in_amax2_stride >= 1);
 }
 void a3d_note_variant(const char *fmt, ...) __attribute__((format(printf, 1, 2)));
 
diff --git a/articulation3d_amd/csrc/conv_gemm.hip b/articulation3d_amd/csrc/conv_gemm.hip
--- a/articulation3d_amd/csrc/conv_gemm.hip
+++ b/articulation3d_amd/csrc/conv_gemm.hip
@@ -44,16 +44,21 @@
     const int rc = conv_check(d);
     if (rc != A3D_OK) return rc;
     hipStream_t s = (hipStream_t)stream;
+    if (!a3d_amax_form_ok(d)) return A3D_ERR_ARG;
     a3d_begin();
     if (d->precision == 1) return a3d_conv_launch_bf16(d, s);
     if (d->precision == 2) {
         if ((d->tune == 0 || d->tune == 8 || d->tune == 24 || d->tune == 25) && d->workspace && d->w_wino && d->w_wino_x3 && ((d->Cin + d->Cin2) & 31) == 0 && a3d_wino_eligible(d)) return a3d_conv_launch_wino(d, s);
         return a3d_conv_launch_bf16x3(d, s);
     }
-    if (d->precision == 3 && d->x_h2) return a3d_conv_launch_bf16x3_wide(d, s);
+    if (d->precision == 3 && d->x_h2) {
+        if (d->y_amax_n || d->in_amax_n || d->in_amax2_n) return A3D_ERR_ARG;
+        return a3d_conv_launch_bf16x3_wide(d, s);
+    }
     if (d->precision == 3) {
         if ((d->tune == 0 || d->tune == 23 || d->tune == 24) && d->workspace && d->w_wino && d->w_wino_x3 && ((d->Cin + d->Cin2) & 31) == 0 && a3d_wino_eligible(d))
             return a3d_conv_launch_wino(d, s);
+        if (d->y_amax_n) return A3D_ERR_ARG;
         return a3d_conv_launch_bf16x3(d, s);
     }
     if (d->precision != 0) return A3D_ERR_ARG;
diff --git a/articulation3d_amd/csrc/conv_prims.h b/articulation3d_amd/csrc/conv_prims.h
--- a/articulation3d_amd/csrc/conv_prims.h
+++ b/articulation3d_amd/csrc/conv_prims.h
@@ -50,7 +50,31 @@
     return *reinterpret_cast<const f32x4 *>(T + row * 32 + ((quad ^ (row & 7)) << 2));
 }
 
-__device__ __forceinline__ void a3d_note_amax(float *y_amax, const int b, float v, const bool valid) {
+__device__ __forceinline__ float a3d_amax_get(const float *amax, const int b, const int n, const int stride) {
+    if (n == 0) return amax[b];
+    const float *q = amax + (size_t)b * n * stride;
+    float m = q[0];
+    for (int k = 1; k < n; ++k) m = fmaxf(m, q[(size_t)k * stride]);
+    return m;
+}
+__device__ __forceinline__ void a3d_note_amax_block(float *y_amax, const int b, const float v, const bool valid, const int n, const int stride) {
+    const unsigned sub = (blockIdx.x + blockIdx.y + (threadIdx.x >> 6)) % (unsigned)n;
+    unsigned long long live = __ballot(valid);
+    while (live) {
+        const int b0 = __shfl(b, __ffsll((long long)live) - 1, 64);
+        const bool mine = valid && b == b0;
+        float m = mine ? v : 0.f;
+#pragma unroll
+        for (int off = 32; off > 0; off >>= 1) m = fmaxf(m, __shfl_xor(m, off, 64));
+        if ((threadIdx.x & 63) == 0 && m > 0.f) atomicMax(reinterpret_cast<int *>(y_amax + ((size_t)b0 * n + sub) * stride), __float_as_int(m));
+        live &= ~__ballot(mine);
+    }
+}
+__device__ __forceinline__ void a3d_note_amax(float *y_amax, const int b, float v, const bool valid, const int n = 0, const int stride = 0) {
+    if (n) {
+        a3d_note_amax_block(y_amax, b, v, valid, n, stride);
+        return;
+    }
     if (!valid) v = 0.f;
     const unsigned long long live = __ballot(valid);
     if (!live) return;
diff --git a/articulation3d_amd/csrc/conv_stem_pool.hip b/articulation3d_amd/csrc/conv_stem_pool.hip
--- a/articulation3d_amd/csrc/conv_stem_pool.hip
+++ b/articulation3d_amd/csrc/conv_stem_pool.hip
@@ -242,7 +242,7 @@
 }
 
 extern "C" int a3d_stem_conv_pool(const a3d_conv_desc *d, void *stream) {
-    if (!d || !d->x || !d->w_x3 || !d->y || !d->in_amax || !(d->w_scale > 0.f)) return A3D_ERR_ARG;
+    if (!d || !d->x || !d->w_x3 || !d->y || !d->in_amax || !(d->w_scale > 0.f) || d->y_amax_n || !a3d_amax_form_ok(d)) return A3D_ERR_ARG;
     if (!d->stem || d->precision != 3 || d->Cout != 64 || d->KH != 7 || d->KW != 7 || d->stride != 2 || d->pad != 3 || d->Kpad != 224) return A3D_ERR_UNSUPPORTED;
     if (d->Ho != (d->H + 6 - 7) / 2 + 1 || d->Wo != (d->W + 6 - 7) / 2 + 1 || d->x2 || d->res || d->gate || d->ups || d->phase || d->pixshuf || d->splitk != 1 || d->m_dev)
         return A3D_ERR_UNSUPPORTED;
diff --git a/articulation3d_amd/csrc/conv_wino.hip b/articulation3d_amd/csrc/conv_wino.hip
--- a/articulation3d_amd/csrc/conv_wino.hip
+++ b/articulation3d_amd/csrc/conv_wino.hip
@@ -59,7 +59,8 @@
 typedef unsigned int wi_u32x4 __attribute__((ext_vector_type(4)));
 __global__ __launch_bounds__(256) void wino_input_h2_kernel(const float *__restrict__ x, const float *__restrict__ x2, unsigned char *__restrict__ Vs,
                                                             const float *__restrict__ in_amax, const float *__restrict__ in_amax2, int B, int H, int W,
-                                                            int Cin, int Cin2, int ups, int Ty, int Tx, int t_off, int t_total) {
+                                                            int Cin, int Cin2, int ups, int Ty, int Tx, int t_off, int t_total, int in_n, int in_stride,
+                                                            int in2_n, int in2_stride) {
     const int C = Cin + Cin2;
     const int Hl = ups ? 2 * H : H, Wl = ups ? 2 * W : W;
     const size_t T = (size_t)B * Ty * Tx;
@@ -79,8 +80,8 @@
         const bool second = c >= Cin;
         const float *src = second ? x2 : x;
         const int cs = second ? Cin2 : Cin, cc = second ? c - Cin : c;
-        float am = in_amax[b];
-        if (in_amax2) am = fmaxf(am, in_amax2[b]);
+        float am = a3d_amax_get(in_amax, b, in_n, in_stride);
+        if (in_amax2) am = fmaxf(am, a3d_amax_get(in_amax2, b, in2_n, in2_stride));
         const float sv = 0.25f * a3d_pow2_scale(am);
         f32x4 d[4][4];
 #pragma unroll
@@ -133,6 +134,7 @@
     const __bf16 *U3;
     float *y_amax;
     const float *in_amax, *in_amax2;
+    int y_n, y_stride, in_n, in_stride, in2_n, in2_stride;
     float w_scale;
     float *M;
     int abl;
@@ -164,8 +166,8 @@
 }
 
 __device__ __forceinline__ float wino_v_scale(const WinoArgs &a, const int b) {
-    float m = a.in_amax[b];
-    if (a.in_amax2) m = fmaxf(m, a.in_amax2[b]);
+    float m = a3d_amax_get(a.in_amax, b, a.in_n, a.in_stride);
+    if (a.in_amax2) m = fmaxf(m, a3d_amax_get(a.in_amax2, b, a.in2_n, a.in2_stride));
     return 0.25f * a3d_pow2_scale(m);
 }
 
@@ -1085,8 +1087,8 @@
             wino_level_of(a.lv, min(tb + pr, a.T - 1), l, tl);
             const int b = tl / (wino_level_sel(a.lv.Ty, l) * wino_level_sel(a.lv.Tx, l));
             if (tb + pr < a.T) {
-                float m = wino_level_sel(a.lv.in_amax, l)[b];
-                if (a.in_amax2) m = fmaxf(m, a.in_amax2[b]);
+                float m = a3d_amax_get(wino_level_sel(a.lv.in_amax, l), b, a.in_n, a.in_stride);
+                if (a.in_amax2) m = fmaxf(m, a3d_amax_get(a.in_amax2, b, a.in2_n, a.in2_stride));
                 unx = 1.f / (0.25f * a3d_pow2_scale(m));
             }
         }
@@ -1162,6 +1164,18 @@
             }
         }
     }
+    if (a.y_n) {
+        if (a.y_amax && tb < a.T) {
+            const int b_hi = min(tb + 31, a.T - 1) / tyx;
+            for (int bi = tb / tyx; bi <= b_hi; ++bi) {
+                float v = 0.f;
+#pragma unroll
+                for (int j = 0; j < 4; ++j) v = jb[j] == bi ? fmaxf(v, vmax[j]) : v;
+                a3d_note_amax(a.y_amax, bi, v, true, a.y_n, a.y_stride);
+            }
+        }
+        return;
+    }
     if constexpr (ML) {
         int l0, tl0, l1, tl1;
         wino_level_of(a.lv, min(tb, a.T - 1), l0, tl0);
@@ -1243,7 +1257,7 @@
             *reinterpret_cast<f32x4 *>(a.y + ooff) = v;
         }
     }
-    if (a.y_amax) a3d_note_amax(a.y_amax, bimg, vmax, ok);
+    if (a.y_amax) a3d_note_amax(a.y_amax, bimg, vmax, ok, a.y_n, a.y_stride);
 }
 __global__ __launch_bounds__(256) void split_bf16x3_kernel(const float *__restrict__ src, __bf16 *__restrict__ dst, int rows, int cols, int chunk, size_t total) {
     const size_t i = ((size_t)blockIdx.x * 256 + threadIdx.x) * 4;
@@ -1335,11 +1349,12 @@
     size_t blocks = (total + 255) / 256;
     if (blocks > 16384) blocks = 16384;
     if (d->precision == 3) {
-        if ((C & 31) || !d->in_amax) return A3D_ERR_ARG;
+        if ((C & 31) || !d->in_amax || !a3d_amax_form_ok(d)) return A3D_ERR_ARG;
         if (d->wino_t_total && (d->wino_t_off < 0 || (size_t)d->wino_t_off + T > (size_t)d->wino_t_total)) return A3D_ERR_ARG;
         if ((size_t)(d->wino_t_total ? d->wino_t_total : T) * C * 4 >= ((size_t)1 << 32)) return A3D_ERR_UNSUPPORTED;
         hipLaunchKernelGGL(wino_input_h2_kernel, dim3((int)blocks), dim3(256), 0, s, d->x, d->x2, reinterpret_cast<unsigned char *>(d->workspace), d->in_amax,
-                           d->in_amax2, d->B, d->H, d->W, d->Cin, d->Cin2, d->ups, Ty, Tx, d->wino_t_total ? d->wino_t_off : 0, d->wino_t_total ? d->wino_t_total : (int)T);
+                           d->in_amax2, d->B, d->H, d->W, d->Cin, d->Cin2, d->ups, Ty, Tx, d->wino_t_total ? d->wino_t_off : 0, d->wino_t_total ? d->wino_t_total : (int)T,
+                           d->in_amax_n, d->in_amax_stride, d->in_amax2_n, d->in_amax2_stride);
         return A3D_OK;
     }
     hipLaunchKernelGGL(wino_input_kernel, dim3((int)blocks), dim3(256), 0, s, d->x, d->x2, d->workspace, d->B, d->H, d->W,
@@ -1372,6 +1387,10 @@
     a.y_amax = d->y_amax;
     a.in_amax = d->in_amax;
     a.in_amax2 = d->in_amax2;
+    if (!a3d_amax_form_ok(d) || (d->precision != 3 && (d->y_amax_n || d->in_amax_n || d->in_amax2_n))) return A3D_ERR_ARG;
+    a.y_n = d->y_amax_n, a.y_stride = d->y_amax_stride;
+    a.in_n = d->in_amax_n, a.in_stride = d->in_amax_stride;
+    a.in2_n = d->in_amax2_n, a.in2_stride = d->in_amax2_stride;
     a.w_scale = d->w_scale;
     a.M = nullptr;
     a.abl = (int)a3d_dev_knob("A3D_WINO_ABL", 0);
@@ -1511,6 +1530,7 @@
     a.y_amax = nullptr;
     a.in_amax = nullptr;
     a.in_amax2 = nullptr;
+    a.y_n = a.y_stride = a.in_n = a.in_stride = a.in2_n = a.in2_stride = 0;
     a.w_scale = d0->w_scale;
     a.M = nullptr;
     a.abl = 0;
@@ -1528,7 +1548,8 @@
         if (k < n) {
             if (d->precision != 3 || !a3d_wino_eligible(d) || d->workspace != d0->workspace || d->w_wino_x3 != d0->w_wino_x3 || d->Cout != d0->Cout ||
                 d->Cin + d->Cin2 != C || d->Cin2 || d->x2 || d->ups || d->gate || d->act != d0->act || d->scale != d0->scale || d->shift != d0->shift ||
-                d->w_scale != d0->w_scale || d->wino_t_total != d0->wino_t_total || (size_t)d->wino_t_off != t || !d->in_amax || !d->y)
+                d->w_scale != d0->w_scale || d->wino_t_total != d0->wino_t_total || (size_t)d->wino_t_off != t || !d->in_amax || !d->y ||
+                d->y_amax_n || d->in_amax_n || d->in_amax2_n)
                 return A3D_ERR_ARG;
         }
         const int Ty = (d->H + 1) / 2, Tx = (d->W + 1) / 2;
diff --git a/articulation3d_amd/csrc/conv_xs_b2b.hip b/articulation3d_amd/csrc/conv_xs_b2b.hip
--- a/articulation3d_amd/csrc/conv_xs_b2b.hip
+++ b/articulation3d_amd/csrc/conv_xs_b2b.hip
@@ -297,6 +297,7 @@
 
 extern "C" int a3d_conv_b2b(const a3d_conv_desc *d1, const a3d_conv_desc *d2, void *stream) {
     if (!d1 || !d2 || !d1->x || !d1->y || !d2->y) return A3D_ERR_ARG;
+    if (d1->y_amax_n || d2->y_amax_n || d2->in_amax_n || !a3d_amax_form_ok(d1)) return A3D_ERR_ARG;
     const a3d_conv_desc *d = d1;
     if (d->precision != 3 || !d->w_x3 || !d->in_amax || d->in_amax2 || !(d->w_scale > 0.f) || !d->res) return A3D_ERR_UNSUPPORTED;
     if (d->KH != 1 || d->KW != 1 || d->stride != 1 || d->pad != 0 || d->Kpad != d->Cin) return A3D_ERR_UNSUPPORTED;
diff --git a/articulation3d_amd/modeling/backbone.py b/articulation3d_amd/modeling/backbone.py
--- a/articulation3d_amd/modeling/backbone.py
+++ b/articulation3d_amd/modeling/backbone.py
@@ -41,6 +41,7 @@
                             norm=FrozenBatchNorm2d(bottleneck_channels), act=ACT_RELU)
         self.conv2 = Conv2d(bottleneck_channels, bottleneck_channels, 3, stride=1, padding=1, bias=False,
                             norm=FrozenBatchNorm2d(bottleneck_channels), act=ACT_RELU)
+        self.conv2.amax_block = True
         self.conv3 = Conv2d(bottleneck_channels, out_channels, 1, bias=False, norm=FrozenBatchNorm2d(out_channels),
                             act=ACT_RELU)
         for layer in (self.conv1, self.conv2, self.conv3, self.shortcut):
diff --git a/articulation3d_amd/modeling/layers.py b/articulation3d_amd/modeling/layers.py
--- a/articulation3d_amd/modeling/layers.py
+++ b/articulation3d_amd/modeling/layers.py
@@ -51,6 +51,7 @@
     pin_precision = None
     b2b_second = False
     _a3d_name = ""
+    amax_block = False
 
     def __init__(self):
         super().__init__()
@@ -104,6 +105,7 @@
         if pin is None and self.b2b_second and ops.B2B_FUSED:
             pin = 2
         self._pack_cache.pin_precision, self._pack_cache.name = pin, self._a3d_name
+        self._pack_cache.amax_block = self.amax_block
         return self._pack_cache
 
     def _pack(self):
diff --git a/articulation3d_amd/modeling/mask_head.py b/articulation3d_amd/modeling/mask_head.py
--- a/articulation3d_amd/modeling/mask_head.py
+++ b/articulation3d_amd/modeling/mask_head.py
@@ -32,6 +32,7 @@
         self.conv_norm_relus = []
         for k in range(m.NUM_CONV):
             conv = Conv2d(cin if k == 0 else dim, dim, 3, padding=1, act=ACT_RELU)
+            conv.amax_block = ops.AMAX_BLOCK_ROWS
             c2_msra_fill(conv.weight, conv.bias)
             self.add_module(f"mask_fcn{k + 1}", conv)
             self.conv_norm_relus.append(conv)
diff --git a/articulation3d_amd/modeling/meta_arch.py b/articulation3d_amd/modeling/meta_arch.py
--- a/articulation3d_amd/modeling/meta_arch.py
+++ b/articulation3d_amd/modeling/meta_arch.py
@@ -83,7 +83,7 @@
                           resize_to=(480, 640)) -> BatchedOutput:
         assert not self.training
         if frames.is_cuda and ops.DEFAULT_PRECISION == 3:
-            ops.amax_reserve(frames.shape[0] * (512 + 8 * int(self.proposal_generator.post_nms_topk[False])), frames.device)
+            ops.amax_reserve(frames.shape[0] * (512 + 1024 + 8 * int(self.proposal_generator.post_nms_topk[False])), frames.device)
         if source_rgb:
             assert frames.dtype == torch.uint8 and self.input_format == "BGR"
             B = frames.shape[0]
diff --git a/articulation3d_amd/modeling/roi_heads/axis_head.py b/articulation3d_amd/modeling/roi_heads/axis_head.py
--- a/articulation3d_amd/modeling/roi_heads/axis_head.py
+++ b/articulation3d_amd/modeling/roi_heads/axis_head.py
@@ -23,6 +23,7 @@
         for k in range(h.NUM_CONV):
             for t, lst in (("R", self.conv_norm_relus_R), ("T", self.conv_norm_relus_T)):
                 conv = Conv2d(self._output_size[0], h.CONV_DIM, 3, padding=1, act=ACT_RELU)
+                conv.amax_block = ops.AMAX_BLOCK_ROWS
                 self.add_module(f"axis_{t}_conv{k + 1}", conv)
                 lst.append(conv)
             self._output_size = (h.CONV_DIM, self._output_size[1], self._output_size[2])
diff --git a/articulation3d_amd/modeling/roi_heads/plane_head.py b/articulation3d_amd/modeling/roi_heads/plane_head.py
--- a/articulation3d_amd/modeling/roi_heads/plane_head.py
+++ b/articulation3d_amd/modeling/roi_heads/plane_head.py
@@ -27,6 +27,7 @@
         self.conv_norm_relus = []
         for k in range(h.NUM_CONV):
             conv = Conv2d(self._output_size[0], h.CONV_DIM, 3, padding=1, act=ACT_RELU)
+            conv.amax_block = ops.AMAX_BLOCK_ROWS
             self.add_module(f"plane_conv{k + 1}", conv)
             self.conv_norm_relus.append(conv)
             self._output_size = (h.CONV_DIM, self._output_size[1], self._output_size[2])
diff --git a/articulation3d_amd/ops.py b/articulation3d_amd/ops.py
--- a/articulation3d_amd/ops.py
+++ b/articulation3d_amd/ops.py
@@ -70,6 +70,7 @@
     w_b16: Optional[torch.Tensor] = None
     pin_precision: Optional[int] = None
     name: str = ""
+    amax_block: object = False
 
     @property
     def out_channels(self) -> int:
@@ -229,6 +230,8 @@
 
 WINO_PLANE_SPLIT = os.environ.get("A3D_WINO_PLANE_SPLIT", "1") != "0"
 _AMAX_CHUNK = 1 << 18
+AMAX_BLOCK_ROWS = tuple(int(v) for v in os.environ.get("A3D_AMAX_BLOCK_ROWS", "1,1").split(","))
+AMAX_BLOCK = tuple(int(v) for v in os.environ.get("A3D_AMAX_BLOCK", "4,16").split(",")) if os.environ.get("A3D_AMAX_BLOCK", "") != "0" else None
 AMAX_MISSES: Optional[list] = None
 _amax_arena: dict = {}
 
@@ -254,9 +257,41 @@
     return t
 
 
+def _block_form(p: "PackedConv"):
+    if not p.amax_block or AMAX_BLOCK is None:
+        return None
+    return AMAX_BLOCK if p.amax_block is True else tuple(p.amax_block)
+
+
+def amax_block_slot(B: int, device, form) -> torch.Tensor:
+    n, stride = form
+    return amax_slot(B * n * stride, device).view(B, n, stride)
+
+
+def _amax_form(a: torch.Tensor) -> Tuple[int, int]:
+    return (0, 0) if a.dim() == 1 else (int(a.shape[1]), int(a.shape[2]))
+
+
+def _packed_amax_of(x: torch.Tensor, what: str) -> torch.Tensor:
+    a = amax_of(x)
+    if a.dim() != 1:
+        raise RuntimeError(f"{what} reads packed [B] maxima only: its input was recorded in the block form (PackedConv.amax_block)")
+    return a
+
+
+def _set_in_amax(d, x: torch.Tensor, x2: Optional[torch.Tensor] = None) -> None:
+    a = amax_of(x)
+    d.in_amax = a.data_ptr()
+    d.in_amax_n, d.in_amax_stride = _amax_form(a)
+    if x2 is not None:
+        a2 = amax_of(x2)
+        d.in_amax2 = a2.data_ptr()
+        d.in_amax2_n, d.in_amax2_stride = _amax_form(a2)
+
+
 def amax_of(x: torch.Tensor) -> torch.Tensor:
     a = getattr(x, "_a3d_amax", None)
-    if a is not None and a.numel() == x.shape[0] and a.device == x.device:
+    if a is not None and a.shape[0] == x.shape[0] and a.device == x.device:
         return a
     if AMAX_MISSES is not None:
         AMAX_MISSES.append(tuple(x.shape))
@@ -326,7 +361,7 @@
 
 def _y_amax(out: torch.Tensor) -> int:
     ya = getattr(out, "_a3d_amax", None)
-    if ya is None or ya.numel() != out.shape[0]:
+    if ya is None or ya.dim() != 1 or ya.shape[0] != out.shape[0]:
         ya = out._a3d_amax = amax_slot(out.shape[0], out.device)
     return ya.data_ptr()
 
@@ -419,7 +454,7 @@
         d = descs[k]
         d.x, d.y, d.precision = _p(x), _p(out), 3
         d.w_wino, d.w_wino_x3, d.w_scale = p.w_wino.data_ptr(), w_h2, u_scale
-        d.in_amax = amax_of(x).data_ptr()
+        d.in_amax = _packed_amax_of(x, "conv2d_levels").data_ptr()
         d.y_amax = _y_amax(out)
         d.workspace = ws.data_ptr()
         d.wino_t_off, d.wino_t_total = off, total
@@ -484,7 +519,7 @@
         md = None if m_dev is None else (m_dev.reshape(1) - s).clamp(0, e - s).to(torch.int32)
         o = out[s:e]
         ya = getattr(out, "_a3d_amax", None)
-        if ya is not None and ya.numel() == B:
+        if ya is not None and ya.shape[0] == B:
             o._a3d_amax = ya[s:e]
         _conv2d_launch(xb, p, x2=x2b, res=rb, out=o, gate=gb, m_dev=md, **kw)
         recorded.append(getattr(o, "_a3d_amax", None))
@@ -565,7 +600,7 @@
 def presplit_f16x2(x: torch.Tensor, x2: Optional[torch.Tensor] = None):
     _req(x)
     B, n = x.shape[0], x.numel() // x.shape[0]
-    ax, ax2 = amax_of(x), (None if x2 is None else amax_of(_req(x2)))
+    ax, ax2 = _packed_amax_of(x, "presplit_f16x2"), (None if x2 is None else _packed_amax_of(_req(x2), "presplit_f16x2"))
     outs = []
     for t in ((x,) if x2 is None else (x, x2)):
         nt = t.numel() // B
@@ -621,7 +656,7 @@
 
     def __init__(self, t, s, e):
         a = getattr(t, "_a3d_amax", None)
-        self._a3d_amax = None if a is None or a.numel() != t.shape[0] else a[s:e]
+        self._a3d_amax = None if a is None or a.shape[0] != t.shape[0] else a[s:e]
         self.shape = (e - s,)
 
 
@@ -675,7 +710,7 @@
     if (LAUNCH_PLANS and CONV_TIMING is None and x2 is None and m_dev is None and out is None and gate is None and dot is None and not ups and splitk == 1
             and tune == 0 and wino is None and precision is None and act is None and not (p.phase or p.pixshuf or p.stem) and p.presplit
             and (_WINO_SHARE is None or x.data_ptr() not in _WINO_SHARE)):
-        plan_key = (DEFAULT_PRECISION, WINO_TUNE, p.pin_precision, x.shape, None if res is None else tuple(res.shape), bool(res_ups),
+        plan_key = (DEFAULT_PRECISION, WINO_TUNE, p.pin_precision, _block_form(p), x.shape, None if res is None else tuple(res.shape), bool(res_ups),
                     WINO_PLANE_SPLIT, BF16_SPLITK_AUTO, BF16_SPLITK, x.device, p.w.data_ptr())
         plans = p.__dict__.get("_plans")
         plan = plans.get(plan_key) if plans else None
@@ -688,9 +723,9 @@
                 _check_res(res, oshape[0], d.Ho, d.Wo, d.Cout, res_ups)
                 d.res = res.data_ptr()
             if need_in:
-                d.in_amax = amax_of(x).data_ptr()
+                _set_in_amax(d, x)
             if need_y:
-                ya = out._a3d_amax = amax_slot(oshape[0], x.device)
+                ya = out._a3d_amax = amax_block_slot(oshape[0], x.device, (d.y_amax_n, d.y_amax_stride)) if need_y == "block" else amax_slot(oshape[0], x.device)
                 d.y_amax = ya.data_ptr()
             if ws_n:
                 ws = torch.empty(ws_n, device=x.device, dtype=torch.float32)
@@ -741,12 +776,15 @@
         splitk = _bf16_splitk(B * Ho * Wo, p.cols, p.Kpad)
         d.splitk = splitk
     if precision == 3:
-        d.in_amax = amax_of(x).data_ptr()
-        if x2 is not None:
-            d.in_amax2 = amax_of(x2).data_ptr()
+        _set_in_amax(d, x, x2)
         d.w_scale = filter_scale(p)
     if precision in (2, 3) and (DEFAULT_PRECISION == 3 or precision == 3) and not p.pixshuf:
-        d.y_amax = _y_amax(out)
+        form = _block_form(p)
+        if use_wino and precision == 3 and tune in (0, 23, 24) and form and (Cin + Cin2) % 32 == 0 and getattr(out, "_a3d_amax", None) is None:
+            ya = out._a3d_amax = amax_block_slot(B, x.device, form)
+            d.y_amax, (d.y_amax_n, d.y_amax_stride) = ya.data_ptr(), form
+        else:
+            d.y_amax = _y_amax(out)
     if use_wino:
         d.w_wino = p.w_wino.data_ptr()
         if p.w_wino_cm is not None and precision == 0 and tune == 0:
@@ -820,7 +858,7 @@
     if plan_key is not None:
         if p.__dict__.get("_plans") is None or len(p._plans) > 64:
             p._plans = {}
-        p._plans[plan_key] = (bytes(d), tuple(out.shape), bool(d.in_amax), bool(d.y_amax), nbytes // 4 if ws is not None else 0,
+        p._plans[plan_key] = (bytes(d), tuple(out.shape), bool(d.in_amax), "block" if d.y_amax_n else bool(d.y_amax), nbytes // 4 if ws is not None else 0,
                               mbytes // 4 if d.wino_m else 0, precision)
     return out
 
@@ -852,7 +890,7 @@
     d1.x, d1.res, d1.y, d1.y_amax = x.data_ptr(), res.data_ptr(), y.data_ptr(), _y_amax(y)
     d2.x, d2.y, d2.y_amax = y.data_ptr(), z.data_ptr(), _y_amax(z)
     d1.precision, d2.precision = 3, 2
-    d1.in_amax = amax_of(x).data_ptr()
+    _set_in_amax(d1, x)
     d1.w_scale = filter_scale(p1)
     d1.w_x3, d2.w_x3 = weight_planes(p1, "w_h2"), weight_planes(p2, "w_x3")
 
@@ -1078,7 +1116,7 @@
     d.KH, d.KW, d.stride, d.pad, d.Cout = 7, 7, 2, 3, 64
     d.x, d.y, d.precision = x.data_ptr(), out.data_ptr(), 3
     d.tune = int(os.environ.get("A3D_STEM_ABL", "0"))
-    d.in_amax = amax_of(x).data_ptr()
+    _set_in_amax(d, x)
     d.w_scale, d.w_x3 = filter_scale(p), weight_planes(p, "w_h2")
     d.y_amax = _y_amax(out)
 
@@ -1276,7 +1314,7 @@
         ra = amax_slot(nrows, dev)
         d.out_amax = ra.data_ptr()
         for l, f in enumerate(feats):
-            d.level_amax[l] = amax_of(f).data_ptr()
+            d.level_amax[l] = _packed_amax_of(f, "roi_align_fpn").data_ptr()
         d.window_count = window_counter(dev).data_ptr()
     _lib.check(_lib.lib().a3d_roi_align_fpn(C.byref(d), _stream()), "a3d_roi_align_fpn")
     if ra is not None:
diff --git a/include/a3d.h b/include/a3d.h
--- a/include/a3d.h
+++ b/include/a3d.h
@@ -58,8 +58,10 @@
     const float *in_amax2;
     float *y_amax;
     float w_scale;
+    unsigned char y_amax_n, y_amax_stride, in_amax_n, in_amax_stride;
     float *wino_m;
     int io_bf16;
+    unsigned char in_amax2_n, in_amax2_stride;
     const void *x_h2;
     const void *x2_h2;
     const float *dot_w;
```
